# haampie/Homogenization.jl

Hardware: AMD Instinct MI355X
Metric: fine-DOF updates/sec per V-cycle (3D Tet64) (higher is better)
Workload: dtype f64; 1 GPU; 3D Tet64 checkerboard, 32^3 unit cubes x 6 tets, refinements=5 (BASELINE config 3); cells=196608, nf=6545, levels=6, smoothing_steps=3, smoothing_steps_coarse=2, coarse_solver=device CG, Chebyshev(4)-of-Jacobi preconditioner, rtol 1e-13, spare_vector_bytes=10294394880, lazy_top_form=2

## Files before the change

homogenization.jl_amd/csrc/hmg_context.cpp:

```cpp
#include "../../include/hmg.h"
#include "hmg_objects.hpp"

#include <algorithm>

namespace hmg {

std::recursive_mutex &lifetime_mutex()
{
    static std::recursive_mutex m;
    return m;
}

std::atomic<int64_t> &device_allocs()
{
    static std::atomic<int64_t> n{0};
    return n;
}

namespace {

void vec_pool_trim(hmg_ctx *c)
{
    LifetimeLock lock(lifetime_mutex());
    if (c->vec_pool.empty()) return;
    (void)hipStreamSynchronize(c->stream);
    for (auto &b : c->vec_pool) (void)hipFree(b.second);
    c->vec_pool.clear();
}

std::vector<hmg_ctx *> &live_contexts()
{
    static std::vector<hmg_ctx *> v;
    return v;
}

void release_pooled_memory()
{
    LifetimeLock lock(lifetime_mutex());
    for (hmg_ctx *c : live_contexts()) vec_pool_trim(c);
}

}

hipError_t device_malloc(void **p, size_t bytes)
{
    *p = nullptr;
    hipError_t e = hipMalloc(p, bytes);
    if (e != hipSuccess) {
        (void)hipGetLastError();
        release_pooled_memory();
        e = hipMalloc(p, bytes);
    }
    if (e == hipSuccess) device_allocs() += 1;
    return e;
}

double *vec_alloc(hmg_ctx *c, size_t bytes)
{
    LifetimeLock lock(lifetime_mutex());
    void *p = nullptr;
    for (size_t i = 0; i < c->vec_pool.size(); ++i)
        if (c->vec_pool[i].first == bytes) {
            p = c->vec_pool[i].second;
            c->vec_pool[i] = c->vec_pool.back();
            c->vec_pool.pop_back();
            break;
        }
    const bool pooled = p != nullptr;
    if (!pooled) {
        hipError_t e = device_malloc(&p, bytes);
        if (e != hipSuccess)
            throw std::runtime_error(std::string("hipMalloc of a level vector (") + std::to_string(bytes >> 20) +
                                     " MiB) failed: " + hipGetErrorString(e));
    }
    hipError_t e = hipMemsetAsync(p, 0, bytes, c->stream);
    if (e != hipSuccess) {
        (void)hipFree(p);
        throw std::runtime_error(std::string("HIP error: ") + hipGetErrorString(e));
    }
    return (double *)p;
}

void vec_release(hmg_ctx *c, void *p, size_t bytes)
{
    LifetimeLock lock(lifetime_mutex());
    if (c->vec_pool_on && bytes > 0) {
        c->vec_pool.emplace_back(bytes, p);
        return;
    }
    (void)hipStreamSynchronize(c->stream);
    (void)hipFree(p);
}

namespace {

void ensure_reduce_scratch(hmg_ctx *c, int64_t nentries)
{
    const int64_t need_blocks = nentries / 512 + 2;
    if (need_blocks <= 2048 || need_blocks <= c->L.rpart_cap) return;
    HIPCHK(hipStreamSynchronize(c->stream));
    c->rpart.alloc((size_t)need_blocks);
    c->L.rpart = c->rpart.p;
    c->L.rpart_cap = need_blocks;
}

void ctx_unref(hmg_ctx *ctx)
{
    LifetimeLock lock(lifetime_mutex());
    if (!ctx || --ctx->refs > 0) return;
    auto &lc = live_contexts();
    lc.erase(std::remove(lc.begin(), lc.end(), ctx), lc.end());
    (void)hipSetDevice(ctx->device);
    (void)hipStreamSynchronize(ctx->stream);
    for (auto &ev : ctx->timer.pool) {
        (void)hipEventDestroy(ev.first);
        (void)hipEventDestroy(ev.second);
    }
    vec_pool_trim(ctx);
    comm_drop(ctx);
    if (ctx->own_stream) (void)hipStreamDestroy(ctx->stream);
    delete ctx;
}

}

void grid_unref(hmg_grid *grid)
{
    LifetimeLock lock(lifetime_mutex());
    if (!grid || --grid->refs > 0) return;
    hmg_ctx *c = grid->ctx;
    if (c) {
        (void)hipSetDevice(c->device);
        (void)hipStreamSynchronize(c->stream);
    }
    probe_unlist(grid);
    release_top_spare(grid);
    release_weight_cache(grid);
    release_smoother_diag(grid);
    if (grid->probe && grid->probe->h) (void)hipHostFree(grid->probe->h);
    if (grid->probe && grid->probe->ev) (void)hipEventDestroy(grid->probe->ev);
    delete grid;
    ctx_unref(c);
}

double read_scalar(hmg_ctx *c, int slot)
{
    double h = 0.0;
    HIPCHK(hipMemcpyAsync(&h, c->L.scal + slot, sizeof(double), hipMemcpyDeviceToHost, c->stream));
    HIPCHK(hipStreamSynchronize(c->stream));
    judge_probes(c);
    return h;
}

}

extern "C" {

const char *hmg_last_error(void) { return last_error().c_str(); }
int hmg_version(void) { return 1; }

static int ctx_create(int device, void *stream, bool use_given, hmg_ctx **out)
{
    HMG_TRY
    need(out != nullptr, "null out pointer");
    int ndev = 0;
    hipError_t e = hipGetDeviceCount(&ndev);
    if (e != hipSuccess || ndev == 0)
        throw std::runtime_error("no HIP device available: libhmg_hip needs an MI355X (gfx950); there is no CPU fallback");
    need(device >= 0 && device < ndev, "device index out of range");
    HIPCHK(hipSetDevice(device));
    std::unique_ptr<hmg_ctx> c(new hmg_ctx);
    c->device = device;
    if (use_given) {
        c->stream = (hipStream_t)stream;
    } else {
        HIPCHK(hipStreamCreateWithFlags(&c->stream, hipStreamNonBlocking));
        c->own_stream = true;
    }
    hipDeviceProp_t prop;
    HIPCHK(hipGetDeviceProperties(&prop, device));
    c->partials.alloc(4096);
    c->scal.alloc(S_COUNT);
    HIPCHK(hipMemsetAsync(c->scal.p, 0, S_COUNT * sizeof(double), c->stream));
    c->L.stream = c->stream;
    c->L.partials = c->partials.p;
    c->L.rpart = nullptr;
    c->L.rpart_cap = 0;
    c->L.scal = c->scal.p;
    c->L.num_cu = prop.multiProcessorCount > 0 ? prop.multiProcessorCount : 256;
    c->L.apply_threads = 0;
    c->L.apply_mass_only = 0;
    c->L.cell_order = 1;
    c->L.weight_cache = 1;
    c->L.apply_wave = 1;
    c->L.wave_grid = 16 * (int64_t)c->L.num_cu;
    c->L.n_wave_launches = &c->wave_launches;
    c->L.apply_slab2 = 1;
    c->L.n_slab2_launches = &c->slab2_launches;
    c->L.n_rows_launches = &c->rows_launches;
    c->L.slab2_grid = 0;
    c->L.slab2_force = 0;
    c->L.restrict_slab2 = 1;
    c->L.apply_pack = 1;
    c->L.apply_small = 1;
    c->L.n_small_launches = &c->small_launches;
    c->L.n_wc_launches = &c->wc_launches;
    c->L.apply_wg512 = 1;
    {
        LifetimeLock lock(lifetime_mutex());
        live_contexts().push_back(c.get());
    }
    *out = c.release();
    HMG_END
}

int hmg_ctx_create(int device, void *stream, hmg_ctx **out) { return ctx_create(device, stream, stream != nullptr, out); }

int hmg_ctx_create_on_stream(int device, void *stream, hmg_ctx **out) { return ctx_create(device, stream, true, out); }

int hmg_ctx_destroy(hmg_ctx *ctx)
{
    HMG_TRY
    ctx_unref(ctx);
    HMG_END
}

int hmg_ctx_sync(hmg_ctx *ctx)
{
    HMG_TRY
    need(ctx != nullptr, "null ctx");
    HIPCHK(hipStreamSynchronize(ctx->stream));
    judge_probes(ctx);
    HMG_END
}

int64_t hmg_ctx_counter(hmg_ctx *ctx, const char *name)
{
    if (!ctx || !name) return -1;
    const std::string n(name);
    if (n == "wave_launches") return ctx->wave_launches;
    if (n == "slab2_launches") return ctx->slab2_launches;
    if (n == "rows_launches") return ctx->rows_launches;
    if (n == "small_launches") return ctx->small_launches;
    if (n == "weight_cache_launches") return ctx->wc_launches;
    if (n == "comm_calls") return ctx->comm_calls;
    if (n == "device_allocs") return device_allocs().load();
    if (n == "spare_bytes") return ctx->spare_bytes;
    if (n == "weight_cache_classes") return ctx->wc_classes;
    if (n == "weight_cache_bytes") return ctx->wc_bytes;
    if (n == "weight_cache_refusals") return ctx->wc_refusals;
    if (n == "fcg_bytes") return ctx->fcg_bytes;
    if (n == "smoother_diag_bytes") return ctx->smoother_diag_bytes;
    if (n == "smoother_diag_builds") return ctx->smoother_diag_builds;
    if (n == "lazy_top_form") return ctx->last_top_form;
    if (n == "lazy_pre_form") return ctx->last_pre_form;
    if (n == "coarse_x_folds") return ctx->coarse_x_folds;
    if (n == "cell_moments_kernel_ns") return ctx->moments_kernel_ns;
    if (n == "cell_moments_download_ns") return ctx->moments_download_ns;
    if (n == "comm_nranks") return ctx->comm ? ctx->comm_nranks : 0;
    return -1;
}

int hmg_ctx_release_memory(hmg_ctx *ctx)
{
    HMG_TRY
    need(ctx != nullptr, "null ctx");
    vec_pool_trim(ctx);
    HMG_END
}

int hmg_ctx_set_option(hmg_ctx *ctx, const char *name, int64_t value)
{
    HMG_TRY
    need(ctx && name, "null argument");
    std::string n(name);
    static const std::pair<const char *, bool hmg_ctx::*> flags[] = {
        {"coarse_probe", &hmg_ctx::coarse_probe}, {"fuse_cg", &hmg_ctx::fuse_cg_default}, {"fold_x", &hmg_ctx::fold_x},
        {"swap_rp", &hmg_ctx::swap_rp}, {"fold_prolong", &hmg_ctx::fold_prolong}, {"zero_entry", &hmg_ctx::zero_entry},
        {"fold_restrict", &hmg_ctx::fold_restrict}, {"lazy_dead", &hmg_ctx::lazy_dead}, {"lazy_pre", &hmg_ctx::lazy_pre}, {"fold_coarse_x", &hmg_ctx::fold_coarse_x}, {"fold_faces", &hmg_ctx::fold_faces},
        {"lean_post", &hmg_ctx::lean_post}, {"lazy_post", &hmg_ctx::lazy_post}, {"prolong_in_image", &hmg_ctx::prolong_in_image},
        {"comm_rehearsal", &hmg_ctx::comm_rehearsal}};
    for (const auto &f : flags)
        if (n == f.first) {
            ctx->*f.second = value != 0;
            return 0;
        }
    if (n == "apply_threads")
        ctx->L.apply_threads = (int)value;
    else if (n == "apply_wg512")
        ctx->L.apply_wg512 = value != 0;
    else if (n == "apply_pack")
        ctx->L.apply_pack = value != 0;
    else if (n == "apply_small")
        ctx->L.apply_small = value != 0;
    else if (n == "weight_cache")
        ctx->L.weight_cache = value != 0;
    else if (n == "weight_cache_classes")
        ctx->wc_max_classes = std::max<int64_t>(0, value);
    else if (n == "apply_slab2")
        ctx->L.apply_slab2 = value != 0;
    else if (n == "restrict_slab2")
        ctx->L.restrict_slab2 = value != 0;
    else if (n == "slab2_force")
        ctx->L.slab2_force = value != 0;
    else if (n == "slab2_grid")
        ctx->L.slab2_grid = std::max<int64_t>(0, value);
    else if (n == "apply_wave")
        ctx->L.apply_wave = value != 0;
    else if (n == "wave_grid")
        ctx->L.wave_grid = std::max<int64_t>(1, value) * (int64_t)ctx->L.num_cu;
    else if (n == "wave_grid_total")
        ctx->L.wave_grid = std::max<int64_t>(1, value);
    else if (n == "cell_order")
        ctx->L.cell_order = value != 0;
    else if (n == "coarse_poly")
        ctx->coarse_poly = std::max<int>(1, std::min<int>(16, (int)value));
    else if (n == "coarse_maxit")
        ctx->coarse_maxit = (int)value;
    else if (n == "coarse_check")
        ctx->coarse_check = std::max<int>(1, (int)value);
    else if (n == "lazy_top")
        ctx->lazy_top = (int)value;
    else if (n == "overlap_min_doubles")
        ctx->overlap_min_doubles = value;
    else if (n == "vec_pool") {
        ctx->vec_pool_on = value != 0;
        if (!ctx->vec_pool_on) vec_pool_trim(ctx);
    }
    else if (n == "time_apply") {
        ctx->timer.on = value > 0;
        ctx->timer.min_level = (int)value;
        ctx->timer.used = 0;
        ctx->timer.ev_level.clear();
        ctx->timer.ev_bytes.clear();
    }
    else
        throw std::runtime_error("unknown option: " + n);
    HMG_END
}

int hmg_ctx_set_option_f64(hmg_ctx *ctx, const char *name, double value)
{
    HMG_TRY
    need(ctx && name, "null argument");
    std::string n(name);
    if (n == "coarse_rtol")
        ctx->coarse_rtol = value;
    else if (n == "coarse_poly_ratio")
        ctx->coarse_poly_ratio = value;
    else
        throw std::runtime_error("unknown option: " + n);
    HMG_END
}

void *hmg_ctx_scalar_bank(hmg_ctx *ctx) { return ctx ? (void *)ctx->L.scal : nullptr; }

int hmg_ctx_set_scalar_bank(hmg_ctx *ctx, void *device_doubles16)
{
    HMG_TRY
    need(ctx != nullptr, "null argument");
    HIPCHK(hipStreamSynchronize(ctx->stream));
    double *to = device_doubles16 ? (double *)device_doubles16 : ctx->scal.p;
    if (to != ctx->L.scal) HIPCHK(hipMemcpy(to, ctx->L.scal, S_COUNT * sizeof(double), hipMemcpyDeviceToDevice));
    ctx->L.scal = to;
    HMG_END
}

static int apply_timing(hmg_ctx *ctx, bool every, int level, int64_t *launches, double *total_ms, double *total_bytes)
{
    HMG_TRY
    need(ctx && launches && total_ms && total_bytes, "null argument");
    HIPCHK(hipStreamSynchronize(ctx->stream));
    const ApplyTimer &tm = ctx->timer;
    double ms = 0.0, by = 0.0;
    int64_t n = 0;
    for (size_t i = 0; i < tm.used; ++i) {
        if (!every && tm.ev_level[i] != level) continue;
        float t = 0.f;
        HIPCHK(hipEventElapsedTime(&t, tm.pool[i].first, tm.pool[i].second));
        ms += t;
        by += tm.ev_bytes[i];
        n += 1;
    }
    *launches = n;
    *total_ms = ms;
    *total_bytes = by;
    HMG_END
}

int hmg_ctx_apply_timing(hmg_ctx *ctx, int64_t *launches, double *total_ms, double *total_bytes)
{
    return apply_timing(ctx, true, 0, launches, total_ms, total_bytes);
}

int hmg_ctx_apply_timing_level(hmg_ctx *ctx, int level, int64_t *launches, double *total_ms, double *total_bytes)
{
    return apply_timing(ctx, false, level, launches, total_ms, total_bytes);
}

void *hmg_ctx_stream(hmg_ctx *ctx) { return ctx ? (void *)ctx->stream : nullptr; }

int hmg_grid_destroy(hmg_grid *grid)
{
    HMG_TRY
    grid_unref(grid);
    HMG_END
}

int hmg_vec_create(hmg_grid *g, int level, hmg_vec **out)
{
    HMG_TRY
    need(g && out, "null argument");
    const LevelDev &lv = lev(g, level);
    HIPCHK(hipSetDevice(g->ctx->device));
    std::unique_ptr<hmg_vec> v(new hmg_vec);
    v->g = g;
    v->level = level;
    v->own = true;
    v->alloc_cells = g->md.ncells;
    size_t bytes = sizeof(double) * (size_t)lv.ld * (size_t)g->md.ncells;
    ensure_reduce_scratch(g->ctx, (int64_t)lv.ld * g->md.ncells);
    v->d = vec_alloc(g->ctx, bytes);
    v->bytes = bytes;
    if (wants_top_spare(g, level)) (void)reserve_top_spare(g, false);
    {
        LifetimeLock lock(lifetime_mutex());
        g->refs += 1;
    }
    *out = v.release();
    HMG_END
}

int hmg_vec_wrap(hmg_grid *g, int level, void *device_ptr, hmg_vec **out)
{
    HMG_TRY
    need(g && out && device_ptr, "null argument");
    ensure_reduce_scratch(g->ctx, (int64_t)lev(g, level).ld * g->md.ncells);
    std::unique_ptr<hmg_vec> v(new hmg_vec);
    v->g = g;
    v->level = level;
    v->own = false;
    v->alloc_cells = g->md.ncells;
    v->d = (double *)device_ptr;
    if (wants_top_spare(g, level)) (void)reserve_top_spare(g, false);
    {
        LifetimeLock lock(lifetime_mutex());
        g->refs += 1;
    }
    *out = v.release();
    HMG_END
}

int hmg_vec_destroy(hmg_vec *v)
{
    HMG_TRY
    if (v) {
        if (v->own && v->d) vec_release(v->g->ctx, v->d, v->bytes);
        hmg_grid *g = v->g;
        delete v;
        grid_unref(g);
    }
    HMG_END
}

void *hmg_vec_device_ptr(hmg_vec *v) { return v ? (void *)v->d : nullptr; }

}
```

homogenization.jl_amd/csrc/hmg_device.hpp:

```cpp
#pragma once
#include <hip/hip_runtime.h>

#include <cstdint>

namespace hmg {

constexpr int TABLE_PAD = 3 * 1024;

__host__ __device__ inline int rows_slot(int m, int i, int j, int nei, int off_int, int &cls)
{
    if (j == 0) {
        cls = i == 0 ? 4 : i == m ? 5 : 1;
        return i == 0 ? 0 : i == m ? 1 : 3 + i - 1;
    }
    if (i == 0) {
        cls = j == m ? 6 : 2;
        return j == m ? 2 : 3 + nei + j - 1;
    }
    if (i + j == m) {
        cls = 3;
        return 3 + 2 * nei + j - 1;
    }
    cls = 0;
    return off_int + (j - 1) * (m - 1) - (((j - 1) * j) >> 1) + i - 1;
}

struct LevelDev {
    int dim, level, m;
    int nf, ld;
    int ncorner, nedge, nface;
    int nei, nfi, nint;
    int off_edge, off_face, off_int;
    int ncls, ndir, nterm;
    int lds_g0, lds_g1;
    int nf_coarse;
    const uint64_t *meta;
    const uint16_t *lpos;
    const uint16_t *sweep_slot;
    int nsweep;
    const uint32_t *pos32;
    const uint32_t *pos32w;
    const uint32_t *sweep32;
    const uint32_t *blk_word;
    const uint16_t *blk_slot;
    int nblk, blk_R;
    const double *ctab;
    const int32_t *hier2slot;
    const int32_t *par_a, *par_b;
    const uint32_t *par32;
    const uint64_t *par64;
    const uint16_t *clpos;
    const uint32_t *rs_word;
    const double *rs_w;
    const uint16_t *rs_lp;
    const int32_t *rptr, *ridx;
    const double *dphi;
    const uint32_t *wave_tab;
    const uint32_t *wave_lpos;
    const uint32_t *wave_par;
    const uint32_t *wave_cl;
    const uint32_t *wave_rs;
    const double *wcache;
};

constexpr int WM = 16, WNF = 969, WNFI = 105, WNEI = 15, WNCORNER = 4, WNBLK = 152, WNFC = 165, WR = 4;
constexpr int WOFF_EDGE = 4, WOFF_FACE = 94, WNEC = 94;
constexpr int WNQ = 16;
constexpr int WVZ = 168;
constexpr int WAVE_TAB_ROWS = 15;
constexpr int WAVE_ROW = 16;
constexpr int WAVE_WSTRIDE = 15 * WAVE_ROW;

struct SlabTables {
    const int *head;
    const uint32_t *ld_word;
    const uint32_t *cp_word;
    const uint16_t *cp_slot;
    int nslab, lds_nodes;
    int max_surf;
    int max_int;
};

struct MeshDev {
    int dim;
    int64_t ncells, nnodes;
    const int32_t *cells;
    const int32_t *face_pairs;
    int64_t nfacepairs;
    const int32_t *face_partner;
    const int32_t *edge_ptr, *edge_ent;
    int64_t nsharededges;
    const int32_t *node_ptr, *node_ent;
    int64_t nsharednodes;
    const int32_t *node_first;
    const uint16_t *dmask, *dupmask;
    const double *coef;
    int64_t ncut_edge_groups, ncut_node_groups;
    int64_t ncut_face_pairs;
    const int32_t *cells_cut, *cells_inner;
    const int32_t *cell_perm;
    int64_t ncells_cut, ncells_inner;
    const uint8_t *mult;
    const int32_t *cell_class;
    int nclasses;
    double wc_lambda;
    double *blockpart;
    SlabTables slab;
};

struct ApplyArgs {
    double alpha, lambda;
    const double *x;
    const double *x2;
    double *xout;
    double *xacc;
    int a_num, a_den;
    const double *x3;
    int c_num, c_den;
    const double *x4;
    int d_num, d_den;
    const double *xcoarse;
    int64_t ldc;
    const double *xc_p, *xc_r;
    const double *src;
    double *out;
    double *rcoarse;
    int64_t ldrc;
    const double *scal;
    int s_num, s_den;
    double *blockpart;
    const uint8_t *mult;
    int flags;
    int64_t ncells_prefix;
    int64_t out_ld;
    const int32_t *cell_list;
    int64_t ncell_list;
    int64_t nwork;
    const int32_t *cell_class;
};

struct CoarseDev {
    int64_t n;
    const int32_t *rowptr, *colidx;
    const double *val, *diag;
    const int32_t *interior;
};

enum { S_RS = 0, S_PAP = 1, S_RS2 = 2, S_TMP = 3, S_C0 = 4, S_C1 = 5, S_C2 = 6, S_C3 = 7, S_PAP2 = 8, S_DONE = 9, S_ITER = 10,
       S_CRR = 11, S_HOST = 12, S_COUNT = 16,
       S_RS3 = S_C1, S_PAP3 = S_TMP };

struct Launch {
    hipStream_t stream;
    double *partials;
    double *rpart;
    int64_t rpart_cap;
    double *scal;
    int num_cu;
    int apply_threads;
    int apply_mass_only;
    int apply_wg512;
    int cell_order;
    int weight_cache;
    int apply_pack;
    int apply_small;
    int64_t *n_small_launches;
    int64_t *n_wc_launches;
    int apply_wave;
    int64_t wave_grid;
    int64_t *n_wave_launches;
    int apply_slab2;
    int64_t *n_slab2_launches;
    int64_t slab2_grid;
    int restrict_slab2;
    int slab2_force;
    int64_t *n_rows_launches;
};

void launch_apply(const Launch &L, const LevelDev &lv, const MeshDev &mesh, double alpha, double lambda,
                  const double *x, const double *src, double *out, int use_mask);
size_t apply_lds_bytes(const LevelDev &lv);
bool apply_restricts(const Launch &L, const LevelDev &lv);
bool apply_folds_coarse_x(const Launch &L, const LevelDev &lv);
bool apply_defers3(const Launch &L, const LevelDev &lv);
void launch_apply_fused_kernel(const Launch &L, const LevelDev &lv, const MeshDev &mesh, ApplyArgs a);
void launch_apply_fused_reduce(const Launch &L, const MeshDev &mesh, int slot_pap, int slot_rr);
void launch_apply_args(const Launch &L, const LevelDev &lv, const MeshDev &mesh, ApplyArgs a);
bool apply_wave_ok(const Launch &L, const LevelDev &lv, const MeshDev &mesh, const ApplyArgs &a, bool fused);
void launch_apply_wave(const Launch &L, const LevelDev &lv, const MeshDev &mesh, const ApplyArgs &a, bool fused);
bool apply_slab2_ok(const Launch &L, const LevelDev &lv, const MeshDev &mesh, const ApplyArgs &a);
void launch_apply_slab2(const Launch &L, const LevelDev &lv, const MeshDev &mesh, const ApplyArgs &a, bool fused);
void launch_apply_rows(const Launch &L, const LevelDev &lv, const MeshDev &mesh, const ApplyArgs &a, bool fused, bool wd);
void launch_prolong_add_wide(const Launch &L, const LevelDev &fine, const LevelDev &coarse, int64_t ncells, const double *xc,
                             double *xf);
int64_t launch_norm2_unique_wide(const Launch &L, const LevelDev &lv, const MeshDev &mesh, const double *x);
bool apply_small_ok(const Launch &L, const LevelDev &lv, const MeshDev &mesh, const ApplyArgs &a, bool fused);
void launch_apply_small(const Launch &L, const LevelDev &lv, const MeshDev &mesh, const ApplyArgs &a, bool fused);
void launch_weight_cache(const Launch &L, const LevelDev &lv, const double *coef_rep, int nclasses, double lambda, double *wcache);

void launch_interface_sum(const Launch &L, const LevelDev &lv, const MeshDev &mesh, double *x, int which = 0,
                          bool faces = true);
void launch_mask(const Launch &L, const LevelDev &lv, const MeshDev &mesh, double *x, int which );
void launch_restrict_slab(const Launch &L, const LevelDev &fine_rtab, const MeshDev &mesh, const SlabTables &st, int ldc,
                          const double *rf, double *bc);
void launch_restrict(const Launch &L, const LevelDev &fine, const LevelDev &coarse, int64_t ncells,
                     const double *rf, double *bc);
void launch_prolong_add(const Launch &L, const LevelDev &fine, const LevelDev &coarse, int64_t ncells,
                        const double *xc, double *xf);

void launch_fill(const Launch &L, double *x, int64_t n, double v);
void launch_copy(const Launch &L, double *dst, const double *src, int64_t n);
void launch_axpy(const Launch &L, double a, const double *x, double *y, int64_t n);
void launch_xpby(const Launch &L, const double *r, double b, double *p, int64_t n);
void launch_dot(const Launch &L, const double *x, const double *y, int64_t n, int slot);
void launch_norm2_unique(const Launch &L, const LevelDev &lv, const MeshDev &mesh, const double *x, int slot);
void launch_copy_dot(const Launch &L, double *p, const double *r, int64_t n, int slot);
void launch_cg_update(const Launch &L, double *x, double *r, const double *p, const double *q, int64_t n,
                      int s_num, int s_den, int s_out);
void launch_cg_rupdate(const Launch &L, const double *r, double *rout, const double *q, int64_t n, int s_num, int s_den,
                       int s_out);
void launch_cg_rupdate_faces(const Launch &L, const LevelDev &lv, const MeshDev &mesh, const double *r, double *rout,
                             const double *q, int64_t n, int s_num, int s_den, int s_out);
void launch_cg_rupdate_faces_x(const Launch &L, const LevelDev &lv, const MeshDev &mesh, const double *r, double *rout,
                               const double *q, int64_t n, int s_num, int s_den, int s_out, double *x, const double *p, int a_num,
                               int a_den, int b_num, int b_den, const double *p0, int z_num, int z_den);
void launch_cg_xp_update(const Launch &L, double *x, double *p, const double *r, int64_t n, int a_num, int a_den,
                         int s_num, int s_den, int with_p);
void launch_cg_x2_update(const Launch &L, double *x, const double *p, const double *r, int64_t n, int a_num, int a_den, int b_num,
                         int b_den, int c_num, int c_den);
void launch_cg_pupdate(const Launch &L, double *p, const double *r, int64_t n, int s_num, int s_den);

void launch_gather_base(const Launch &L, const MeshDev &mesh, int ld1, const double *v1, double *u);
void launch_scatter_base(const Launch &L, const MeshDev &mesh, int ld1, const double *u, double *v1);

void launch_gather_owned(const Launch &L, const MeshDev &mesh, const int32_t *nodes_g, const int32_t *owned, int ld1,
                         const double *v1, double *ug);
void launch_scatter_cells(const Launch &L, const int32_t *cell_nodes, int64_t ncells, int npc, int ld1, const double *u,
                          double *v1);

void launch_permute(const Launch &L, const LevelDev &lv, int64_t ncells, const double *src, double *dst,
                    int to_storage);
void launch_fill_random(const Launch &L, const LevelDev &lv, int64_t ncells, double *x, uint64_t seed,
                        int64_t cell_offset);

void launch_coarse_gather_rhs(const Launch &L, const CoarseDev &A, const double *u, double *b);
void launch_coarse_scatter_sol(const Launch &L, const CoarseDev &A, int64_t nnodes, const double *x, double *u);
void launch_coarse_init(const Launch &L, const CoarseDev &A, const double *b, double *x, double *r, double *z,
                        double *p, double zscale = 1.0, double *dcheb = nullptr);
void launch_coarse_cheb(const Launch &L, const CoarseDev &A, const double *r, const double *zin, double *zout, double *d, double c1,
                        double c2, int last);
void launch_coarse_rz_from_cheb(const Launch &L, const CoarseDev &A);
void launch_coarse_update(const Launch &L, const CoarseDev &A, double *x, double *r, double *z, const double *p,
                          const double *q, int slot_old, double zscale = 1.0, double *dcheb = nullptr);
void launch_coarse_residual_norm(const Launch &L, const CoarseDev &A);
void launch_coarse_direction(const Launch &L, const CoarseDev &A, double *p, double *q, const double *z, int slot_old, int slot_new,
                             double rtol2, int mode, int count_it, int rz_from_cheb = 0);

void launch_rhs_dphi(const Launch &L, const LevelDev &lv, int64_t ncells, const double *pvec, double *b);

void launch_integrate(const Launch &L, const LevelDev &lv, const MeshDev &mesh, int mode, int64_t nsub, const double *v,
                      const double *second, int slot);
void launch_integrate_load(const Launch &L, const LevelDev &lv, const MeshDev &mesh, int64_t nsub, const double *v,
                           const double *load, int slot);

struct CutPackArgs {
    int64_t n[3];
    const int64_t *pos[3];
    const int32_t *cell_lid[3];
    const uint8_t *first[3];
};
void launch_cut_pack(const Launch &L, const LevelDev &lv, const CutPackArgs &c, double *buf, double *x, int unpack);
void launch_seg_sum(const Launch &L, const int64_t *plan, int64_t ndoubles, double *buf, const double *stage);

}
```

homogenization.jl_amd/csrc/hmg_kernels.hip:

```cpp
#include "hmg_device.hpp"
#include "hmg_stencil.hpp"

#include <cstdio>
#include <stdexcept>
#include <string>

namespace hmg {

__global__ void __launch_bounds__(256) k_finalize(const double *__restrict__ partials, int n, double *scal, int slot)
{
    __shared__ double red[4];
    double v = 0.0;
    for (int i = threadIdx.x; i < n; i += 256) v += partials[i];
    double s = block_sum(v, red);
    if (threadIdx.x == 0) scal[slot] = s;
}

#ifdef HMG_PHASE_TIMING
#define HMG_STAMP(i)                                                                     \
    do {    \
        if (a.blockpart && !a.cell_list && tid == 0)                                     \
            a.blockpart[2 * (size_t)a.nwork + 8 * cell + (i)] = (double)wall_clock64(); \
    } while (0)
#define HMG_SLAB_T0() const long long _t0 = wall_clock64(); long long _tl = _t0; double _ph[5] = {0, 0, 0, 0, 0}
#define HMG_SLAB_PHASE(i)                              \
    do {                                               \
        const long long _n = wall_clock64();           \
        _ph[i] += (double)(_n - _tl);                  \
        _tl = _n;                                      \
    } while (0)
#define HMG_SLAB_STORE()                                                                      \
    do {                                                                                      \
        if (a.blockpart && tid == 0) {                                                        \
            double *_o = a.blockpart + 2 * (size_t)a.nwork + 8 * cell;                        \
            _o[0] = (double)_t0;                                                              \
            for (int _q = 0; _q < 5; ++_q) _o[1 + _q] = _ph[_q];                              \
            _o[6] = (double)wall_clock64();                                                   \
        }                                                                                     \
    } while (0)
#else
#define HMG_STAMP(i)
#define HMG_SLAB_T0()
#define HMG_SLAB_PHASE(i)
#define HMG_SLAB_STORE()
#endif

template <int DIM, int NT, int SPT, bool FUSED, int RB, bool WD = false, bool CG = false, bool RS = false, bool WC = false, int LF = 0>
__global__ void __launch_bounds__(NT, NT >= 640 ? 8 : RB && NT == 512 ? 6 : 1)
k_apply(LevelDev lv, const double *__restrict__ coef, const uint16_t *__restrict__ dmask, ApplyArgs a)
{
    constexpr int NDIR = DIM == 3 ? 15 : 7;
    constexpr int NTERM = DIM == 3 ? 7 : 4;
    constexpr int WS = RB ? WSZ_RB : WSZ;
    extern __shared__ double smem[];
    double *W = smem;
    double *xs = smem + WS + lv.lds_g0;
    const int tid = threadIdx.x;
    constexpr bool LOOP = NT == 64;
    int64_t blk = blockIdx.x;
    do {
    const int64_t cell = a.cell_list ? (int64_t)a.cell_list[blk] : blk;
    const int nf = lv.nf;
    HMG_STAMP(0);

    size_t wbase16 = 0;
    if constexpr (WC) wbase16 = (size_t)(2 * HMG_KP(int32_t, a.cell_class)[cell] + (a.alpha < 0.0 ? 1 : 0)) * WAVE_WSTRIDE;
    const double cv = RB && !WC ? coef[cell * 8 + (tid & 7)] : 0.0;
    if (!RB && (tid >= NT - 256 || NT <= 256)) {
        const int first = NT <= 256 ? tid : tid - (NT - 256);
        const int step = NT <= 256 ? NT : 256;
        if constexpr (WC) {
            for (int idx = first; idx < lv.ncls * NDIR; idx += step)
                W[idx] = lv.wcache[wbase16 + (size_t)((idx / NDIR) * WAVE_ROW + idx % NDIR)];
        } else {
        double s[NTERM];
        cell_scales<DIM>(coef + cell * 8, a.alpha, a.lambda, s, a.flags);
        for (int idx = first; idx < lv.ncls * NDIR; idx += step) {
            const double *c = lv.ctab + (size_t)idx * NTERM;
            double w = 0.0;
#pragma unroll
            for (int t = 0; t < NTERM; ++t) w += c[t] * s[t];
            W[idx] = w;
        }
        }
    }
    for (int q = tid; q < lv.lds_g0; q += NT) smem[WS + q] = 0.0;
    for (int q = tid; q < lv.lds_g1; q += NT) xs[nf + q] = 0.0;
    const int m = lv.m;
    constexpr int NW = NT / 64, WPF = NW / 4 > 0 ? NW / 4 : 1, NE = NW >= 6 ? 1 : 2;
    constexpr int FI = RB && NT == 512 ? 4 : 2;
    constexpr int NPASS = RB && NT == 512 ? 2 : 1;
    constexpr bool EARLY = RB && (NT <= 256 || WC);
    const int wave = tid >> 6, lane = tid & 63;
    const int face = wave / WPF, ft0 = (wave % WPF) * (FI * 64);
    int edge[NE], ebase[NE];
#pragma unroll
    for (int q = 0; q < NE; ++q) {
        edge[q] = NW - 1 - wave + q * NW;
        if (edge[q] >= lv.nedge) edge[q] = -1;
        ebase[q] = lv.off_edge + (edge[q] < 0 ? 0 : edge[q]) * lv.nei;
    }
    uint32_t fw[FI], ew[NE][1], cw = 0u;
#pragma unroll
    for (int q = 0; q < FI; ++q) fw[q] = 0u;
    uint32_t p0 = 0u, p1 = 0u;
    double wv = 0.0;
    double c7[NTERM];
    uint32_t q0 = 0u, q1 = 0u;
    int s0 = 0, s1 = 0;
    uint32_t mq[4] = {0, 0, 0, 0};
    uint32_t mqr[4] = {0, 0, 0, 0};
    uint32_t dm = 0u;
    const uint32_t *iw = RB ? lv.blk_word : lv.sweep32;
    const uint16_t *is = RB ? lv.blk_slot : lv.sweep_slot;
    double cwl = 0.0;
    auto issue_rows = [&]() {
        if constexpr (WC) {
            if (a.flags & 1) {
                const uint32_t w2 = HMG_KP(uint32_t, dmask)[cell >> 1];
                dm = (cell & 1) ? w2 >> 16 : w2 & 0xffffu;
            }
            if (RB) {
                int row = 0;
                if (lane < 15)
                    row = lane;
                else if (lane >= 16 && lane < 31)
                    row = (1 + face) * WAVE_ROW + lane - 16;
                else if (lane >= 32 && lane < 47 && edge[0] >= 0)
                    row = (1 + lv.nface + edge[0]) * WAVE_ROW + lane - 32;
                else if (NE > 1 && lane >= 48 && lane < 63 && edge[NE - 1] >= 0)
                    row = (1 + lv.nface + edge[NE - 1]) * WAVE_ROW + lane - 48;
                wv = lv.wcache[wbase16 + row];
                if (wave == NW - 1) {
                    const int cl = lane < 60 ? lane : 59;
                    cwl = lv.wcache[wbase16 + (1 + lv.nface + lv.nedge + cl / 15) * WAVE_ROW + cl % 15];
                }
            }
            if (FUSED && a.mult) {
#pragma unroll
                for (int q = 0; q < 4; ++q) mqr[q] = HMG_KP(uint32_t, a.mult)[cell * 4 + q];
            }
            return;
        }
        dm = (a.flags & 1) ? dmask[cell] : 0u;
        if (RB) {
            int row = 0;
            if (lane < 15)
                row = lane;
            else if (lane >= 16 && lane < 31)
                row = (1 + face) * NDIR + lane - 16;
            else if (lane >= 32 && lane < 47 && edge[0] >= 0)
                row = (1 + lv.nface + edge[0]) * NDIR + lane - 32;
            else if (NE > 1 && lane >= 48 && lane < 63 && edge[NE - 1] >= 0)
                row = (1 + lv.nface + edge[NE - 1]) * NDIR + lane - 48;
#pragma unroll
            for (int t = 0; t < NTERM; ++t) c7[t] = lv.ctab[(size_t)row * NTERM + t];
        }
        if (FUSED && a.mult) {
            const uint32_t *mp = reinterpret_cast<const uint32_t *>(a.mult + cell * 16);
#pragma unroll
            for (int q = 0; q < 4; ++q) mqr[q] = mp[q];
        }
    };
    auto issue_words = [&]() {
        if (RB) {
#pragma unroll
            for (int q = 0; q < FI; ++q) {
                const int ti = ft0 + q * 64 + lane;
                if (ti < lv.nfi) fw[q] = lv.pos32[lv.off_face + face * lv.nfi + ti];
            }
#pragma unroll
            for (int q = 0; q < NE; ++q) ew[q][0] = edge[q] >= 0 && lane < lv.nei ? lv.pos32[ebase[q] + lane] : 0u;
            if (wave == NW - 1 && lane < lv.ncorner) cw = lv.pos32[lane];
        } else {
            p0 = lv.pos32[tid];
            p1 = lv.pos32[tid + NT];
        }
        q0 = iw[tid];
        q1 = RB && NPASS < 2 ? 0u : iw[tid + NT];
        s0 = (int)is[tid];
        s1 = RB && NPASS < 2 ? 0 : (int)is[tid + NT];
    };
    auto finish_tables = [&]() {
        if constexpr (WC) {
            if (RB && wave == NW - 1 && lane < 60) W[lane] = cwl;
            if (FUSED) {
#pragma unroll
                for (int q = 0; q < 4; ++q) mq[q] = a.mult ? mqr[q] : 0x01010101u;
            }
            return;
        }
        if (RB) {
            double sc7[NTERM];
#pragma unroll
            for (int t = 0; t < NTERM - 1; ++t) sc7[t] = (a.flags & 2) ? 0.0 : a.alpha * readlane_f64(cv, t);
            sc7[NTERM - 1] = a.alpha * a.lambda * ((a.flags & 16) ? 1.0 : readlane_f64(cv, NTERM - 1));
#pragma unroll
            for (int t = 0; t < NTERM; ++t) wv += c7[t] * sc7[t];
            if (wave == NW - 1) {
                const int cbase = (1 + lv.nface + lv.nedge) * NDIR;
                for (int idx = cbase + lane; idx < lv.ncls * NDIR; idx += 64) {
                    double w = 0.0;
#pragma unroll
                    for (int t = 0; t < NTERM; ++t) w += lv.ctab[(size_t)idx * NTERM + t] * sc7[t];
                    W[idx - cbase] = w;
                }
            }
        }
        if (FUSED) {
#pragma unroll
            for (int q = 0; q < 4; ++q) mq[q] = a.mult ? __builtin_amdgcn_readfirstlane(mqr[q]) : 0x01010101u;
        }
    };
    constexpr bool rows_late = WC && (LF == 2 || LF == 5);
    constexpr bool WEARLY = false;
    if (EARLY && !rows_late) issue_rows();
    if (WEARLY) issue_words();
    const double *xc = a.x + cell * lv.ld;
    double rr = 0.0, pap = 0.0;
    {
        const double *x2c = FUSED && a.x2 ? a.x2 + cell * lv.ld : nullptr;
        double *xoc = FUSED && a.xout ? a.xout + cell * lv.ld : nullptr;
        double *xac = FUSED && a.xacc ? a.xacc + cell * lv.ld : nullptr;
        const double *x3c = FUSED && a.x3 ? a.x3 + cell * lv.ld : nullptr;
        const double beta = x2c ? a.scal[a.s_num] / a.scal[a.s_den] : 0.0;
        const double ax = xac || x3c ? a.scal[a.a_num] / a.scal[a.a_den] : 0.0;
        const double c2 = x3c ? a.scal[a.c_num] / a.scal[a.c_den] : 0.0;
        constexpr bool X4 = FUSED && RS && LF == 4;
        const double *x4c = X4 && a.x4 ? a.x4 + cell * lv.ld : nullptr;
        const double dx4 = x4c ? a.scal[a.d_num] / a.scal[a.d_den] : 0.0;
        const double *ccol = FUSED && !RS && a.xcoarse ? a.xcoarse + cell * a.ldc : nullptr;
        constexpr bool cgather = FUSED && CG;
        double *cs = xs + nf + lv.lds_g1;
        double cval = 0.0;
        if (ccol && !cgather) {
            if (tid < lv.nf_coarse) cval = ccol[tid];
            for (int q = tid + NT; q < lv.nf_coarse; q += NT) cs[q] = ccol[q];
        }
        auto prolong = [&](double v, uint32_t w) {
            const uint32_t pa = w & 0xffffu, pb = w >> 16;
            if (pa == pb) return v + cs[pa];
            v += 0.5 * cs[pa];
            return v + 0.5 * cs[pb];
        };
        if (cgather && ccol) {
            constexpr int NC = 2;
            constexpr bool CX = cgather && LF == 5;
            const double *cpc = CX ? a.xc_p + cell * a.ldc : nullptr, *crc = CX ? a.xc_r + cell * a.ldc : nullptr;
            const double cxa = CX ? to_sgpr(a.scal[a.a_num] / a.scal[a.a_den]) : 0.0;
            const double cxb = CX ? to_sgpr(a.scal[a.s_num] / a.scal[a.s_den]) : 0.0;
            const double cxc = CX ? to_sgpr(a.scal[a.c_num] / a.scal[a.c_den]) : 0.0;
            double cv2[NC], cp2[CX ? NC : 1], cr2[CX ? NC : 1];
            int cl2[NC];
#pragma unroll
            for (int q = 0; q < NC; ++q) {
                const int c = tid + q * NT;
                if (c < lv.nf_coarse) {
                    cv2[q] = ccol[c];
                    if (CX) {
                        cp2[q] = cpc[c];
                        cr2[q] = crc[c];
                    }
                    cl2[q] = lv.clpos[c];
                }
            }
            if (CX) {
#pragma unroll
                for (int q = 0; q < NC; ++q)
                    if (tid + q * NT < lv.nf_coarse) cv2[q] = axpy1(cxc, axpy1(cxb, cp2[q], cr2[q]), axpy1(cxa, cp2[q], cv2[q]));
                __builtin_amdgcn_sched_barrier(0);
                if (EARLY && rows_late) issue_rows();
            }
            double xv[SPT];
            uint64_t pw[SPT];
#pragma unroll
            for (int q = 0; q < SPT; ++q) {
                const int t = tid + q * NT;
                if (t < nf) {
                    xv[q] = xc[t];
                    pw[q] = lv.par64[t];
                }
            }
            if (EARLY) finish_tables();
#pragma unroll
            for (int q = 0; q < NC; ++q)
                if (tid + q * NT < lv.nf_coarse) xs[cl2[q]] = cv2[q];
            __syncthreads();
#pragma unroll
            for (int q = 0; q < SPT; ++q) {
                const int t = tid + q * NT;
                if (t < nf) {
                    const uint32_t pa = (uint32_t)pw[q] & 0xffffu, pb = ((uint32_t)pw[q] >> 16) & 0xffffu;
                    double v = xv[q];
                    if (pa == pb)
                        v = v + lds_ld(xs + pa);
                    else {
                        v += 0.5 * lds_ld(xs + pa);
                        v = v + 0.5 * lds_ld(xs + pb);
                    }
                    xv[q] = v;
                }
            }
            __syncthreads();
#pragma unroll
            for (int q = 0; q < SPT; ++q) {
                const int t = tid + q * NT;
                if (t < nf) {
                    const double v = xv[q];
                    if (xoc) xoc[t] = v;
                    rr += v * v;
                    xs[(int)(pw[q] >> 32)] = v;
                }
            }
        }
        const bool light = LF == 1 || (LF == 0 && !RS && FUSED && NT >= 512 && !x2c && !xac && !x3c && !ccol);
        if (FUSED && light) {
            double xv[SPT];
            int lp[SPT];
#pragma unroll
            for (int q = 0; q < SPT; ++q) {
                const int t = tid + q * NT;
                if (t < nf) {
                    xv[q] = xc[t];
                    lp[q] = lv.lpos[t];
                }
            }
            if (EARLY) finish_tables();
#pragma unroll
            for (int q = 0; q < SPT; ++q) {
                const int t = tid + q * NT;
                if (t < nf) {
                    const double v = xv[q];
                    if (xoc) xoc[t] = v;
                    rr += v * v;
                    xs[lp[q]] = v;
                }
            }
        }
        const bool light2 = LF == 2 || (LF == 0 && !RS && FUSED && NT >= 512 && x2c && !xoc && !xac && !x3c && !ccol);
        if (FUSED && light2) {
            double xv[SPT], x2v[SPT];
            int lp[SPT];
#pragma unroll
            for (int q = 0; q < SPT; ++q) {
                const int t = tid + q * NT;
                if (t < nf) {
                    xv[q] = xc[t];
                    x2v[q] = x2c[t];
                    lp[q] = lv.lpos[t];
                }
            }
            if (EARLY && rows_late) issue_rows();
            if (EARLY) finish_tables();
#pragma unroll
            for (int q = 0; q < SPT; ++q) {
                const int t = tid + q * NT;
                if (t < nf) {
                    const double v = axpy1(beta, x2v[q], xv[q]);
                    if (LF == 2 && xoc) xoc[t] = v;
                    rr += v * v;
                    xs[lp[q]] = v;
                }
            }
        }
        constexpr int HB = X4 ? (SPT + 2) / 3 : FUSED ? (SPT + 1) / 2 : SPT;
        const bool xzero = FUSED && (RS || RB == 0) && (a.flags & 128);
        if (!light && !light2 && !(cgather && ccol)) {
#pragma unroll
        for (int q0 = 0; q0 < SPT; q0 += HB) {
            double xv[HB], x2v[HB], xav[HB], x4v[X4 ? HB : 1];
            int lp[HB];
            uint32_t pw[HB];
#pragma unroll
            for (int q = 0; q < HB; ++q) {
                const int t = tid + (q0 + q) * NT;
                if (q0 + q < SPT && t < nf) {
                    xv[q] = xzero ? 0.0 : xc[t];
                    if (X4) x4v[q] = x4c ? x4c[t] : 0.0;
                    x2v[q] = x2c ? x2c[t] : 0.0;
                    xav[q] = xac ? xac[t] : x3c ? x3c[t] : 0.0;
                    lp[q] = lv.lpos[t];
                    if (FUSED && !cgather) pw[q] = ccol ? lv.par32[t] : 0u;
                }
            }
            if (EARLY && q0 == 0) finish_tables();
            if (FUSED && q0 == 0 && ccol && !cgather) {
                if (tid < lv.nf_coarse) cs[tid] = cval;
                __syncthreads();
            }
#pragma unroll
            for (int q = 0; q < HB; ++q) {
                const int t = tid + (q0 + q) * NT;
                if (q0 + q < SPT && t < nf) {
                    double v = xv[q];
                    if (FUSED) {
                        if (!cgather && ccol) v = prolong(v, pw[q]);
                        if (xac) xac[t] = axpy1(ax, x2v[q], xav[q]);
                        if (x3c) {
                            if (X4 && x4c) v = axpy1(dx4, x4v[q], v);
                            const double t1 = axpy1(ax, x2v[q], v);
                            const double p2 = axpy1(beta, x2v[q], xav[q]);
                            v = axpy1(c2, p2, t1);
                        } else if (x2c)
                            v = axpy1(beta, x2v[q], v);
                        if (xoc) xoc[t] = v;
                        if (!RS) rr += v * v;
                    }
                    xs[lp[q]] = v;
                }
            }
        }
        }
        for (int t = tid + SPT * NT; t < nf; t += NT) {
            double v = xzero ? 0.0 : xc[t];
            if (FUSED) {
                const double pv = x2c ? x2c[t] : 0.0;
                if (!cgather && ccol) v = prolong(v, lv.par32[t]);
                if (xac) xac[t] = axpy1(ax, pv, xac[t]);
                if (x3c) {
                    if (X4 && x4c) v = axpy1(dx4, x4c[t], v);
                    const double t1 = axpy1(ax, pv, v);
                    const double p2 = axpy1(beta, pv, x3c[t]);
                    v = axpy1(c2, p2, t1);
                } else if (x2c)
                    v = axpy1(beta, pv, v);
                if (xoc) xoc[t] = v;
                rr += v * v;
            }
            xs[lv.lpos[t]] = v;
        }
    }

    HMG_STAMP(1);
    __builtin_amdgcn_sched_barrier(0);
    if (!WEARLY) issue_words();
    if (!EARLY) {
        issue_rows();
        finish_tables();
    }
    const double *sc = a.src ? a.src + cell * lv.ld : nullptr;
    double *oc = a.out ? a.out + cell * lv.ld : nullptr;
    const int nsurf = lv.off_int;
    const int nsw = RB ? lv.nblk : lv.nsweep;
    const bool wdot = WD && FUSED && (a.flags & 8);
    const double wself = (wdot && (a.flags & 256)) ? 0.0 : 1.0;
    HMG_STAMP(2);
    __syncthreads();
    HMG_STAMP(3);

    const int wbase = RB ? (1 + lv.nface + lv.nedge) * NDIR : 0;
    auto surface_node = [&](int t, uint32_t pw) -> double {
        const double sv = sc ? sc[t] : 0.0;
        int L, len, A, B, cls;
        decode32<DIM>(pw, m, L, len, A, B, cls);
        double ctr;
        double o = stencil_eval_c<DIM>(W + cls * NDIR - wbase, xs, L, len, A, B, ctr);
        if (!wdot) o = sv + o;
        if ((dm >> (cls - 1)) & 1u) o = 0.0;
        if (!FUSED || oc) oc[t] = o;
        if (FUSED && !RS) {
            const int e = cls - 1;
            const uint32_t word = e < 4 ? mq[0] : e < 8 ? mq[1] : e < 12 ? mq[2] : mq[3];
            const uint32_t mu = (word >> (8 * (e & 3))) & 0xffu;
            pap += (double)mu * ((wdot ? fma(wself, ctr, sv) : ctr) * o);
        }
        return o;
    };
    double kf[FI], ke[NE], kc = 0.0, ki[NPASS][RB ? RB : 1];
    if constexpr (RS && RB != 0 && DIM == 3) {
        double w0e[15];
#pragma unroll
        for (int d = 0; d < NDIR; ++d) w0e[d] = readlane_f64(wv, d);
        if (tid < nsw) interior_block_keep<RB ? RB : 1, FUSED>(w0e, xs, m, nf >> 1, q0, s0, sc, oc, ki[0]);
        if (NPASS > 1 && tid + NT < nsw) interior_block_keep<RB ? RB : 1, FUSED>(w0e, xs, m, nf >> 1, q1, s1, sc, oc, ki[NPASS - 1]);
    }
    if (RB) {
        if (DIM == 3) {
            const bool fdir = (dm >> face) & 1u;
            const double fmult = (double)((mq[0] >> (8 * (face & 3))) & 0xffu);
            const int fbase = lv.off_face + face * lv.nfi;
            double nopre[FI];
#pragma unroll
            for (int q = 0; q < FI; ++q) nopre[q] = 0.0;
            if (face >= 4)
                ;
            else if (face == 0)
                face_items<0, FI, FUSED, FUSED && !RS>(wv, 16, xs, m, lv.nfi, fbase, ft0, fw, fdir, fmult, sc, oc, pap, lane, nopre, false, wdot, RS ? kf : nullptr, wself);
            else if (face == 1)
                face_items<1, FI, FUSED, FUSED && !RS>(wv, 16, xs, m, lv.nfi, fbase, ft0, fw, fdir, fmult, sc, oc, pap, lane, nopre, false, wdot, RS ? kf : nullptr, wself);
            else if (face == 2)
                face_items<2, FI, FUSED, FUSED && !RS>(wv, 16, xs, m, lv.nfi, fbase, ft0, fw, fdir, fmult, sc, oc, pap, lane, nopre, false, wdot, RS ? kf : nullptr, wself);
            else
                face_items<3, FI, FUSED, FUSED && !RS>(wv, 16, xs, m, lv.nfi, fbase, ft0, fw, fdir, fmult, sc, oc, pap, lane, nopre, false, wdot, RS ? kf : nullptr, wself);
#pragma unroll
            for (int q = 0; q < NE; ++q) {
                if (edge[q] < 0) continue;
                const int eb = lv.nface + edge[q];
                const bool edir = (dm >> eb) & 1u;
                const double emult = (double)(((eb < 4 ? mq[0] : eb < 8 ? mq[1] : mq[2]) >> (8 * (eb & 3))) & 0xffu);
                const double nop1[1] = {0.0};
                const int wl = 32 + 16 * q;
                switch (edge[q]) {
                case 0: class_items<edge_tap_mask(0), 1, FUSED, FUSED && !RS>(wv, wl, xs, m, lv.nei, ebase[q], 0, ew[q], edir, emult, sc, oc, pap, lane, nop1, false, wdot, RS ? &ke[q] : nullptr, wself); break;
                case 1: class_items<edge_tap_mask(1), 1, FUSED, FUSED && !RS>(wv, wl, xs, m, lv.nei, ebase[q], 0, ew[q], edir, emult, sc, oc, pap, lane, nop1, false, wdot, RS ? &ke[q] : nullptr, wself); break;
                case 2: class_items<edge_tap_mask(2), 1, FUSED, FUSED && !RS>(wv, wl, xs, m, lv.nei, ebase[q], 0, ew[q], edir, emult, sc, oc, pap, lane, nop1, false, wdot, RS ? &ke[q] : nullptr, wself); break;
                case 3: class_items<edge_tap_mask(3), 1, FUSED, FUSED && !RS>(wv, wl, xs, m, lv.nei, ebase[q], 0, ew[q], edir, emult, sc, oc, pap, lane, nop1, false, wdot, RS ? &ke[q] : nullptr, wself); break;
                case 4: class_items<edge_tap_mask(4), 1, FUSED, FUSED && !RS>(wv, wl, xs, m, lv.nei, ebase[q], 0, ew[q], edir, emult, sc, oc, pap, lane, nop1, false, wdot, RS ? &ke[q] : nullptr, wself); break;
                default: class_items<edge_tap_mask(5), 1, FUSED, FUSED && !RS>(wv, wl, xs, m, lv.nei, ebase[q], 0, ew[q], edir, emult, sc, oc, pap, lane, nop1, false, wdot, RS ? &ke[q] : nullptr, wself); break;
                }
            }
            if (wave == NW - 1 && lane < lv.ncorner) kc = surface_node(lane, cw);
        }
    } else {
        const int nit_surf = (nsurf + NT - 1) / NT;
        for (int it = 0; it < nit_surf; ++it) {
            const int t = tid + it * NT;
            const uint32_t pw = p0;
            p0 = p1;
            p1 = lv.pos32[t + 2 * NT];
            if (t < nsurf) surface_node(t, pw);
        }
    }
    HMG_STAMP(4);
    double w0[15];
#pragma unroll
    for (int d = 0; d < NDIR; ++d) w0[d] = RB ? readlane_f64(wv, d) : to_sgpr(W[d]);
    if (RB) {
        if constexpr (!RS) {
        if (DIM == 3 && tid < nsw) {
            if (sc)
                interior_block<RB ? RB : 1, FUSED, true>(w0, xs, m, nf >> 1, q0, s0, sc, oc, pap, wdot, wself);
            else
                interior_block<RB ? RB : 1, FUSED, false>(w0, xs, m, nf >> 1, q0, s0, sc, oc, pap);
        }
        if (DIM == 3 && NPASS > 1 && tid + NT < nsw) {
            if (sc)
                interior_block<RB ? RB : 1, FUSED, true>(w0, xs, m, nf >> 1, q1, s1, sc, oc, pap, wdot, wself);
            else
                interior_block<RB ? RB : 1, FUSED, false>(w0, xs, m, nf >> 1, q1, s1, sc, oc, pap);
        }
        }
    } else {
        const int nit_sweep = (nsw + NT - 1) / NT;
        for (int it = 0; it < nit_sweep; ++it) {
            const int u = tid + it * NT;
            const uint32_t pw = q0;
            const int t = s0;
            q0 = q1;
            s0 = s1;
            q1 = iw[u + 2 * NT];
            s1 = (int)is[u + 2 * NT];
            if (t != 0xffff) {
                const double sv = sc ? sc[t] : 0.0;
                int L, len, A, B, cls;
                decode32<DIM>(pw, m, L, len, A, B, cls);
                double ctr;
                double o = stencil_eval_v<DIM>(w0, xs + L, len, A, B, ctr);
                if (!wdot) o = sv + o;
                if (!FUSED || oc) oc[t] = o;
                if (FUSED) pap += (wdot ? fma(wself, ctr, sv) : ctr) * o;
            }
        }
    }
    HMG_STAMP(5);
    if constexpr (RS && RB != 0 && DIM == 3) {
        int fl[FI], el[NE], cl = 0;
        uint32_t b0 = 0u, b1 = 0u;
        if (face < 4) {
#pragma unroll
            for (int q = 0; q < FI; ++q) {
                const int ti = ft0 + q * 64 + lane;
                fl[q] = ti < lv.nfi ? (int)lv.lpos[lv.off_face + face * lv.nfi + ti] : 0;
            }
        }
#pragma unroll
        for (int q = 0; q < NE; ++q) el[q] = edge[q] >= 0 && lane < lv.nei ? (int)lv.lpos[ebase[q] + lane] : 0;
        if (wave == NW - 1 && lane < lv.ncorner) cl = (int)lv.lpos[lane];
        if (tid < nsw) b0 = lv.blk_word[tid];
        if (NPASS > 1 && tid + NT < nsw) b1 = lv.blk_word[tid + NT];
        __syncthreads();
        if (face < 4) {
#pragma unroll
            for (int q = 0; q < FI; ++q)
                if (ft0 + q * 64 + lane < lv.nfi) xs[fl[q]] = kf[q];
        }
#pragma unroll
        for (int q = 0; q < NE; ++q)
            if (edge[q] >= 0 && lane < lv.nei) xs[el[q]] = ke[q];
        if (wave == NW - 1 && lane < lv.ncorner) xs[cl] = kc;
        {
            int pos[RB ? RB : 1];
            if (tid < nsw) {
                block_positions<RB ? RB : 1>(m, b0, pos);
                const int nv = (int)(b0 >> 28);
#pragma unroll
                for (int r = 0; r < (RB ? RB : 1); ++r)
                    if (r < nv) xs[pos[r]] = ki[0][r];
            }
            if (NPASS > 1 && tid + NT < nsw) {
                block_positions<RB ? RB : 1>(m, b1, pos);
                const int nv = (int)(b1 >> 28);
#pragma unroll
                for (int r = 0; r < (RB ? RB : 1); ++r)
                    if (r < nv) xs[pos[r]] = ki[NPASS - 1][r];
            }
        }
        __syncthreads();
        double *rc = a.rcoarse + cell * a.ldrc;
        if (lv.rs_lp) {
            for (int c = tid; c < lv.nf_coarse; c += NT) {
                const int b = lv.rptr[c], n = lv.rptr[c + 1] - b;
                int lp[15];
#pragma unroll
                for (int q = 0; q < 15; ++q) lp[q] = lv.rs_lp[b + (q < n ? q : 0)];
                double tmp = 0.0;
                tmp += 1.0 * lds_ld(xs + lp[0]);
#pragma unroll
                for (int q = 1; q < 15; ++q)
                    if (q < n) tmp += 0.5 * lds_ld(xs + lp[q]);
                rc[c] = tmp;
            }
        } else
        for (int c = tid; c < lv.nf_coarse; c += NT) {
            int L, len, A, B, cls, k;
            decode32w(lv.rs_word[c], m, L, len, A, B, cls, k);
            const double *w = lv.rs_w + cls * NDIR;
            auto at = [&](int off) { return lds_ld(xs + max(L + off, 0)); };
            double acc = w[0] * lds_ld(xs + L);
            acc += w[1] * lds_ld(xs + L + 1);
            acc += w[2] * at(-1);
            acc += w[3] * lds_ld(xs + L + len - 1);
            acc += w[4] * at(-len);
            acc += w[5] * lds_ld(xs + L + len);
            acc += w[6] * at(-len - 1);
            acc += w[7] * lds_ld(xs + L + A - len);
            acc += w[8] * at(len + 1 - B);
            acc += w[9] * lds_ld(xs + L + A - 1);
            acc += w[10] * at(1 - B);
            acc += w[11] * lds_ld(xs + L + A);
            acc += w[12] * at(-B);
            acc += w[13] * lds_ld(xs + L + A + 1 - len);
            acc += w[14] * at(len - B);
            rc[c] = 0.0 + acc;
        }
    }
    if (FUSED && !RS) {
        __syncthreads();
        const double s_pap = block_sum(pap, smem);
        const double s_rr = block_sum(rr, smem);
        if (tid == 0) {
            a.blockpart[2 * cell] = s_pap;
            a.blockpart[2 * cell + 1] = s_rr;
        }
    }
    HMG_STAMP(6);
    if (LOOP) {
        blk += gridDim.x;
        if (blk >= a.nwork) break;
        __syncthreads();
    }
    } while (LOOP);
}

template <int DIM, int NT, bool FUSED, bool WD = false>
__global__ void __launch_bounds__(NT, 8)
k_apply_slab(LevelDev lv, const double *__restrict__ coef, const uint16_t *__restrict__ dmask, ApplyArgs a, SlabTables st)
{
    constexpr int NDIR = DIM == 3 ? 15 : 7;
    constexpr int NTERM = DIM == 3 ? 7 : 4;
    constexpr int HB = FUSED ? 3 : 4;
    constexpr int MV = 5;
    extern __shared__ double smem[];
    double *W = smem;
    double *img = smem + WSZ;
    const int tid = threadIdx.x;
    const int64_t cell = a.cell_list ? (int64_t)a.cell_list[blockIdx.x] : (int64_t)blockIdx.x;
    const int m = lv.m;

    if (a.flags & 4) {
        for (int idx = tid; idx < lv.ncls * NDIR; idx += NT) W[idx] = lv.ctab[(size_t)idx * NTERM + NTERM - 1];
    } else {
        double s[NTERM];
        cell_scales<DIM>(coef + cell * 8, a.alpha, a.lambda, s, a.flags);
        for (int idx = tid; idx < lv.ncls * NDIR; idx += NT) {
            const double *c = lv.ctab + (size_t)idx * NTERM;
            double w = 0.0;
#pragma unroll
            for (int t = 0; t < NTERM; ++t) w += c[t] * s[t];
            W[idx] = w;
        }
    }
    const double *xc = a.x + cell * lv.ld;
    const double *x2c = FUSED && a.x2 ? a.x2 + cell * lv.ld : nullptr;
    double *xoc = FUSED && a.xout ? a.xout + cell * lv.ld : nullptr;
    double *xac = FUSED && a.xacc ? a.xacc + cell * lv.ld : nullptr;
    const double *x3c = FUSED && a.x3 ? a.x3 + cell * lv.ld : nullptr;
    const double beta = to_sgpr(x2c ? a.scal[a.s_num] / a.scal[a.s_den] : 0.0);
    const double ax = to_sgpr(xac || x3c ? a.scal[a.a_num] / a.scal[a.a_den] : 0.0);
    const double c2 = to_sgpr(x3c ? a.scal[a.c_num] / a.scal[a.c_den] : 0.0);
    const uint32_t dm = (a.flags & 1) ? dmask[cell] : 0u;
    const double *sc = a.src ? a.src + cell * lv.ld : nullptr;
    double *oc = a.out ? a.out + cell * (a.out_ld ? a.out_ld : (int64_t)lv.ld) : nullptr;
    uint32_t mq[4] = {0, 0, 0, 0};
    if (FUSED) {
        const uint32_t *mp = reinterpret_cast<const uint32_t *>(a.mult + cell * 16);
#pragma unroll
        for (int q = 0; q < 4; ++q) mq[q] = a.mult ? __builtin_amdgcn_readfirstlane(mp[q]) : 0x01010101u;
    }
    const bool wdot = WD && FUSED && (a.flags & 8);
    const double wself = (wdot && (a.flags & 256)) ? 0.0 : 1.0;
    double rr = 0.0, pap = 0.0;
    auto plane_off = [&](int k) {
        if (k <= 0) return 0;
        if (k > m + 1) k = m + 1;
        const long long n1 = m + 1, n2 = m + 1 - k;
        return (int)((n1 * (n1 + 1) * (n1 + 2) - n2 * (n2 + 1) * (n2 + 2)) / 6);
    };
    HMG_SLAB_T0();
    __syncthreads();
    HMG_SLAB_PHASE(0);
    double w0[NDIR];
#pragma unroll
    for (int d = 0; d < NDIR; ++d) w0[d] = to_sgpr(W[d]);
    int lo_prev = 0;
    for (int sl = 0; sl < st.nslab; ++sl) {
        const int *hd = st.head + 8 * sl;
        const int k0 = hd[0], ld_off = hd[1], ld_cnt = hd[2], cp_off = hd[3], cp_cnt = hd[4], cp_surf = hd[5];
        const int lo = plane_off(k0 - 1);
        double *xs = img - lo;
        uint32_t wd0[HB];
#pragma unroll
        for (int q = 0; q < HB; ++q) wd0[q] = st.ld_word[ld_off + q * NT + tid];
        if (sl > 0) {
            __syncthreads();
            const int cnt = plane_off(k0 + 1) - lo, src = lo - lo_prev;
            if (cnt <= MV * NT) {
                double mv[MV];
#pragma unroll
                for (int c = 0; c < MV; ++c) {
                    const int q = c * NT + tid;
                    mv[c] = q < cnt ? img[src + q] : 0.0;
                }
                __syncthreads();
#pragma unroll
                for (int c = 0; c < MV; ++c) {
                    const int q = c * NT + tid;
                    if (q < cnt) img[q] = mv[c];
                }
            } else {
            const int nchunk = (cnt + NT - 1) / NT;
            for (int c = 0; c < nchunk; ++c) {
                const int q = c * NT + tid;
                const double v = q < cnt ? img[src + q] : 0.0;
                __syncthreads();
                if (q < cnt) img[q] = v;
            }
            }
        }
        for (int q = (sl > 0 ? plane_off(k0 + 1) - lo : 0) + tid; q < st.lds_nodes; q += NT) img[q] = 0.0;
        __syncthreads();
        HMG_SLAB_PHASE(1);
        for (int q0 = 0; q0 < ld_cnt; q0 += HB * NT) {
            uint32_t wd[HB];
            double xv[HB], x2v[HB], xav[HB];
#pragma unroll
            for (int q = 0; q < HB; ++q) {
                const int v = q0 + q * NT + tid;
                wd[q] = q0 == 0 ? wd0[q] : st.ld_word[ld_off + v];
            }
#pragma unroll
            for (int q = 0; q < HB; ++q) {
                const int v = q0 + q * NT + tid;
                if (v < ld_cnt) {
                    const int t = (int)(wd[q] >> 16);
                    xv[q] = xc[t];
                    x2v[q] = x2c ? x2c[t] : 0.0;
                    xav[q] = xac ? xac[t] : x3c ? x3c[t] : 0.0;
                }
            }
#pragma unroll
            for (int q = 0; q < HB; ++q) {
                const int v = q0 + q * NT + tid;
                if (v < ld_cnt) {
                    const int t = (int)(wd[q] >> 16);
                    double val = xv[q];
                    if (FUSED) {
                        if (xac) xac[t] = axpy1(ax, x2v[q], xav[q]);
                        if (x3c) {
                            const double t1 = axpy1(ax, x2v[q], val);
                            const double p2 = axpy1(beta, x2v[q], xav[q]);
                            val = axpy1(c2, p2, t1);
                        } else if (x2c)
                            val = axpy1(beta, x2v[q], val);
                        if (xoc) xoc[t] = val;
                        rr += val * val;
                    }
                    xs[wd[q] & 0xffffu] = val;
                }
            }
        }
        const int ib = cp_off + cp_surf;
        uint32_t p0 = st.cp_word[cp_off + tid], p1 = st.cp_word[cp_off + tid + NT];
        int s0 = (int)st.cp_slot[cp_off + tid], s1 = (int)st.cp_slot[cp_off + tid + NT];
        uint32_t q0 = st.cp_word[ib + tid], q1 = st.cp_word[ib + tid + NT];
        int t0 = (int)st.cp_slot[ib + tid], t1 = (int)st.cp_slot[ib + tid + NT];
        __syncthreads();
        HMG_SLAB_PHASE(2);
        const int nit_s = (cp_surf + NT - 1) / NT;
        for (int it = 0; it < nit_s; ++it) {
            const int v = it * NT + tid;
            const uint32_t pw = p0;
            const int t = s0;
            p0 = p1;
            s0 = s1;
            p1 = st.cp_word[cp_off + v + 2 * NT];
            s1 = (int)st.cp_slot[cp_off + v + 2 * NT];
            if (v < cp_surf) {
                const double sv = sc ? sc[t] : 0.0;
                int L, len, A, B, cls, k;
                decode32w(pw, m, L, len, A, B, cls, k);
                double ctr;
                double o = stencil_eval_c<DIM>(W + cls * NDIR, xs, L, len, A, B, ctr);
                if (!wdot) o = sv + o;
                if ((dm >> (cls - 1)) & 1u) o = 0.0;
                if (!FUSED || oc) oc[t] = o;
                if (FUSED) {
                    const int en = cls - 1;
                    const uint32_t word = en < 4 ? mq[0] : en < 8 ? mq[1] : en < 12 ? mq[2] : mq[3];
                    const uint32_t mu = (word >> (8 * (en & 3))) & 0xffu;
                    pap += (double)mu * ((wdot ? fma(wself, ctr, sv) : ctr) * o);
                }
            }
        }
        HMG_SLAB_PHASE(3);
        const int n_int = cp_cnt - cp_surf;
        const int nit_i = (n_int + NT - 1) / NT;
        for (int it = 0; it < nit_i; ++it) {
            const int v = it * NT + tid;
            const uint32_t pw = q0;
            const int t = t0;
            q0 = q1;
            t0 = t1;
            q1 = st.cp_word[ib + v + 2 * NT];
            t1 = (int)st.cp_slot[ib + v + 2 * NT];
            if (v < n_int) {
                const double sv = sc ? sc[t] : 0.0;
                int L, len, A, B;
                decode_lattice(pw, m, L, len, A, B);
                double ctr;
                double o = stencil_eval_v<DIM>(w0, xs + L, len, A, B, ctr);
                if (!wdot) o = sv + o;
                if (!FUSED || oc) oc[t] = o;
                if (FUSED) pap += (wdot ? fma(wself, ctr, sv) : ctr) * o;
            }
        }
        lo_prev = lo;
        HMG_SLAB_PHASE(4);
    }
    HMG_SLAB_STORE();
    if (FUSED) {
        __syncthreads();
        const double s_pap = block_sum(pap, smem);
        const double s_rr = block_sum(rr, smem);
        if (tid == 0) {
            a.blockpart[2 * cell] = s_pap;
            a.blockpart[2 * cell + 1] = s_rr;
        }
    }
}

__global__ void __launch_bounds__(256)
k_reduce_pairs(const double *__restrict__ blockpart, int64_t n, double *partials)
{
    __shared__ double red[4];
    double s0 = 0.0, s1 = 0.0;
    for (int64_t c = (int64_t)blockIdx.x * 256 + threadIdx.x; c < n; c += (int64_t)gridDim.x * 256) {
        s0 += blockpart[2 * c];
        s1 += blockpart[2 * c + 1];
    }
    const double r0 = block_sum(s0, red);
    const double r1 = block_sum(s1, red);
    if (threadIdx.x == 0) {
        partials[blockIdx.x] = r0;
        partials[2048 + blockIdx.x] = r1;
    }
}

__global__ void __launch_bounds__(256)
k_reduce_weighted(const double *__restrict__ blockpart, const double *__restrict__ coef, int jterm, int64_t n, double *partials)
{
    __shared__ double red[4];
    double s0 = 0.0;
    for (int64_t c = (int64_t)blockIdx.x * 256 + threadIdx.x; c < n; c += (int64_t)gridDim.x * 256)
        s0 += blockpart[2 * c] * coef[c * 8 + jterm];
    const double r0 = block_sum(s0, red);
    if (threadIdx.x == 0) partials[blockIdx.x] = r0;
}

size_t apply_lds_bytes(const LevelDev &lv)
{
    return sizeof(double) * (size_t)(WSZ + lv.lds_g0 + lv.nf + lv.lds_g1);
}

bool apply_restricts(const Launch &L, const LevelDev &lv)
{
    if (!(lv.dim == 3 && apply_lds_bytes(lv) <= 160 * 1024 && L.apply_threads == 0 && lv.rs_word &&
          lv.rs_w && lv.nf_coarse > 0 && lv.nei <= 64 && lv.nedge == 6 && lv.ncorner == 4))
        return false;
    if (lv.nf > 2048)
        return lv.blk_R == 6 && lv.nblk <= 960 && L.apply_wg512 && lv.nfi <= 512;
    return lv.nf > 192 && lv.nf <= 1024 && lv.blk_R == 4 && lv.nblk <= 192 && lv.nfi <= 128 && lv.rs_lp != nullptr;
}

bool apply_defers3(const Launch &L, const LevelDev &lv)
{
    return apply_restricts(L, lv) && lv.nf > 2048 && lv.nf <= 13 * 512;
}

bool apply_folds_coarse_x(const Launch &L, const LevelDev &lv)
{
    return lv.dim == 3 && apply_lds_bytes(lv) <= 160 * 1024 && L.apply_threads == 0 && L.apply_wg512 && lv.blk_R == 6 && lv.nblk <= 960 &&
           lv.nei <= 64 && lv.nedge == 6 && lv.ncorner == 4 && lv.nfi <= 512 && lv.par64 && lv.clpos && lv.nf > 2048 &&
           lv.nf <= 13 * 512 && lv.nf_coarse > 0 && lv.nf_coarse <= 2 * 512;
}

static size_t apply_lds_bytes_rb(const LevelDev &lv)
{
    return sizeof(double) * (size_t)(WSZ_RB + lv.lds_g0 + lv.nf + lv.lds_g1);
}

template <bool FUSED>
static void check_apply_bases(const ApplyArgs &a, const MeshDev &mesh)
{
    if (!a.x) throw std::runtime_error("operator apply: null input vector");
    if (!FUSED && !a.out) throw std::runtime_error("operator apply: a plain launch needs an output vector");
    if (a.rcoarse && a.ldrc <= 0) throw std::runtime_error("operator apply: epilogue restriction without the coarse column stride");
    if (FUSED && (!a.blockpart || !a.scal)) throw std::runtime_error("operator apply: fused launch without its reduction scratch");
    if (!mesh.coef) throw std::runtime_error("operator apply: no operator coefficients on the device (hmg_grid_set_operator)");
    if ((a.flags & 1) && !mesh.dmask) throw std::runtime_error("operator apply: constraint requested without a Dirichlet mask");
    if (a.xcoarse && !a.xout) throw std::runtime_error("operator apply: folded prolongation without xout");
    if ((a.flags & 128) && !(FUSED && a.x3 && a.x2 && a.xout && !a.xcoarse))
        throw std::runtime_error("operator apply: the zero-input form exists for the residual with two pending x-updates only");
}

static bool weight_cache_ok(const Launch &L, const LevelDev &lv, const MeshDev &mesh, const ApplyArgs &a)
{
    return L.weight_cache && lv.wcache && mesh.cell_class && lv.dim == 3 && lv.ncls == 15 && !(a.flags & (2 | 8 | 16)) &&
           (a.alpha == 1.0 || a.alpha == -1.0) && a.lambda == mesh.wc_lambda;
}

template <int DIM, int NT, int SPT, bool FUSED, int RB = 0, bool WD = false, bool CG = false, bool RS = false, bool WC = false, int LF = 0>
static void launch_apply_generic(const Launch &L, const LevelDev &lv, const MeshDev &mesh, const ApplyArgs &a, size_t lds)
{
    auto kern = k_apply<DIM, NT, SPT, FUSED, RB, WD, CG, RS, WC, LF>;
    if (a.rcoarse && !RS) throw std::runtime_error("operator apply: this instantiation cannot restrict in its epilogue");
    if (a.xc_p && !(CG && LF == 5)) throw std::runtime_error("operator apply: this instantiation cannot finish the coarse x");
    if (a.x4 && LF != 4) throw std::runtime_error("operator apply: this instantiation cannot carry a third pending x-update");
    if ((a.flags & 128) && !(FUSED && (RS || RB == 0)))
        throw std::runtime_error("operator apply: this instantiation cannot take a zero input that is not in memory");
    if (FUSED && a.xcoarse && !CG) lds += sizeof(double) * (size_t)lv.nf_coarse;
    if (lds > 48 * 1024)
        HMG_HIP_CHECK(hipFuncSetAttribute((const void *)kern, hipFuncAttributeMaxDynamicSharedMemorySize, (int)lds));
    const int64_t nblocks = a.cell_list ? a.ncell_list : a.ncells_prefix ? a.ncells_prefix : mesh.ncells;
    if (nblocks == 0) return;
    check_apply_bases<FUSED>(a, mesh);
    ApplyArgs b = a;
    b.nwork = nblocks;
    b.cell_class = WC ? mesh.cell_class : nullptr;
    if (WC && !weight_cache_ok(L, lv, mesh, a)) throw std::runtime_error("operator apply: class-weight cache not usable for this launch");
    if (L.cell_order && RB && !a.cell_list && !a.ncells_prefix && mesh.cell_perm) {
        b.cell_list = mesh.cell_perm;
        b.ncell_list = nblocks;
    }
    const int64_t grid = NT == 64 ? std::min<int64_t>(nblocks, 32 * (int64_t)L.num_cu) : nblocks;
    hipLaunchKernelGGL(kern, dim3((unsigned)grid), dim3(NT), lds, L.stream, lv, mesh.coef, mesh.dmask, b);
    check_launch();
    if (WC && L.n_wc_launches) *L.n_wc_launches += 1;
}

template <int DIM, bool FUSED, bool WD = false>
static void launch_apply_dim(const Launch &L, const LevelDev &lv, const MeshDev &mesh, const ApplyArgs &a)
{
    const size_t lds = apply_lds_bytes(lv);
    if (a.x4 && !(FUSED && DIM == 3 && !WD && a.x3 && a.x2 && a.xout && a.rcoarse && !a.xcoarse && !a.xacc && !(a.flags & 128) &&
                  apply_defers3(L, lv)))
        throw std::runtime_error("operator apply: a third pending x-update (x4) where no kernel carries it");
    if ((a.xc_p || a.xc_r) && !(FUSED && DIM == 3 && !WD && a.xc_p && a.xc_r && a.xcoarse && (a.flags & 64) && !a.x2 && !a.xacc && !a.x3 &&
                                !a.rcoarse && apply_folds_coarse_x(L, lv)))
        throw std::runtime_error("operator apply: pending coarse x-updates (xc_p, xc_r) where no kernel carries them");
    if constexpr (DIM == 3 && !WD) {
        if (apply_wave_ok(L, lv, mesh, a, FUSED)) {
            launch_apply_wave(L, lv, mesh, a, FUSED);
            return;
        }
        if (apply_small_ok(L, lv, mesh, a, FUSED)) {
            launch_apply_small(L, lv, mesh, a, FUSED);
            return;
        }
    }
    const bool force_slab2 = DIM == 3 && !WD && L.slab2_force && mesh.slab.head && mesh.slab.nslab >= 2 && lv.nf > 2048 &&
                             !a.xcoarse && !a.rcoarse && !(a.flags & (4 | 8));
    if (DIM == 2 && lds > 160 * 1024) {
        launch_apply_rows(L, lv, mesh, a, FUSED, WD);
        return;
    }
    if (lds > 160 * 1024 || force_slab2) {
        if (DIM != 3 || !mesh.slab.head) throw std::runtime_error("operator apply: cell does not fit the LDS");
        if constexpr (DIM == 3 && !WD) {
            if (apply_slab2_ok(L, lv, mesh, a)) {
                launch_apply_slab2(L, lv, mesh, a, FUSED);
                return;
            }
        }
        auto kern = k_apply_slab<3, 1024, FUSED, WD>;
        const size_t bytes = sizeof(double) * (size_t)(WSZ + mesh.slab.lds_nodes);
        HMG_HIP_CHECK(hipFuncSetAttribute((const void *)kern, hipFuncAttributeMaxDynamicSharedMemorySize, (int)bytes));
        const int64_t nblocks = a.cell_list ? a.ncell_list : a.ncells_prefix ? a.ncells_prefix : mesh.ncells;
        if (nblocks == 0) return;
        check_apply_bases<FUSED>(a, mesh);
        ApplyArgs b = a;
        b.nwork = nblocks;
        if (L.cell_order && !a.cell_list && !a.ncells_prefix && mesh.cell_perm) {
            b.cell_list = mesh.cell_perm;
            b.ncell_list = nblocks;
        }
        hipLaunchKernelGGL(kern, dim3((unsigned)nblocks), dim3(1024), bytes, L.stream, lv, mesh.coef, mesh.dmask, b,
                           mesh.slab);
        check_launch();
        return;
    }
    const int nf = lv.nf;
    int nt = WD ? 0 : L.apply_threads;
    if (nt == 0) nt = nf <= 192 ? 64 : nf <= 2048 ? 256 : 1024;
    if (nt <= 64) {
        if constexpr (DIM == 3 && !WD) {
            if (weight_cache_ok(L, lv, mesh, a)) {
                if (nf > 64)
                    launch_apply_generic<DIM, 64, 3, FUSED, 0, false, false, false, DIM == 3>(L, lv, mesh, a, lds);
                else
                    launch_apply_generic<DIM, 64, 1, FUSED, 0, false, false, false, DIM == 3>(L, lv, mesh, a, lds);
                return;
            }
        }
        if (nf > 64)
            launch_apply_generic<DIM, 64, 3, FUSED, 0, WD>(L, lv, mesh, a, lds);
        else
            launch_apply_generic<DIM, 64, 1, FUSED, 0, WD>(L, lv, mesh, a, lds);
    }
    else if (nt <= 192 && nf <= 192)
        launch_apply_generic<DIM, 192, 1, FUSED, 0, WD>(L, lv, mesh, a, lds);
    else if (nt <= 256 && nf <= 1024) {
        if (DIM == 3 && lv.blk_R == 4 && lv.nblk <= 192 && lv.nfi <= 128 && lv.nei <= 64 && lv.nedge == 6 && lv.ncorner == 4) {
            if constexpr (!WD) {
                if (FUSED && DIM == 3 && a.rcoarse && lv.rs_word && lv.rs_w && !a.xcoarse) {
                    launch_apply_generic<DIM, 256, 4, FUSED, DIM == 3 ? 4 : 0, false, false, FUSED && DIM == 3>(
                        L, lv, mesh, a, apply_lds_bytes_rb(lv));
                    return;
                }
            }
            launch_apply_generic<DIM, 256, 4, FUSED, DIM == 3 ? 4 : 0, WD>(L, lv, mesh, a, apply_lds_bytes_rb(lv));
        }
        else
            launch_apply_generic<DIM, 256, 4, FUSED, 0, WD>(L, lv, mesh, a, lds);
    }
    else if (nt <= 256)
        launch_apply_generic<DIM, 256, 8, FUSED, 0, WD>(L, lv, mesh, a, lds);
    else if (nt <= 640) {
        if constexpr (!WD) {
            if (nt <= 512) {
                if (DIM == 3 && lv.blk_R == 6 && lv.nblk <= 1024 && lv.nfi <= 512 && lv.nei <= 64 && lv.nedge == 6 &&
                    lv.ncorner == 4)
                    launch_apply_generic<DIM, 512, 13, FUSED, DIM == 3 ? 6 : 0>(L, lv, mesh, a, apply_lds_bytes_rb(lv));
                else
                    launch_apply_generic<DIM, 512, 13, FUSED>(L, lv, mesh, a, lds);
            } else
                launch_apply_generic<DIM, 640, 11, FUSED>(L, lv, mesh, a, lds);
        }
    } else if (DIM == 3 && lv.blk_R == 6 && lv.nblk <= 960 && lv.nei <= 64 && lv.nedge == 6 && lv.ncorner == 4) {
        if constexpr (!WD) {
            if (L.apply_wg512 && lv.nfi <= 512) {
                const bool cg = FUSED && DIM == 3 && a.xcoarse && (a.flags & 64) && lv.par64 && lv.clpos && !a.x2 && !a.xacc && !a.x3 &&
                                lv.nf <= 13 * 512 && lv.nf_coarse <= 2 * 512;
                const bool rs = !cg && FUSED && DIM == 3 && a.rcoarse && lv.rs_word && lv.rs_w && !a.xcoarse;
                constexpr int R6 = DIM == 3 ? 6 : 0;
                constexpr bool F3 = FUSED && DIM == 3;
                if (DIM == 3 && weight_cache_ok(L, lv, mesh, a)) {
                    if (cg && a.xc_p)
                        launch_apply_generic<DIM, 512, 13, FUSED, R6, false, F3, false, DIM == 3, F3 ? 5 : 0>(L, lv, mesh, a, apply_lds_bytes_rb(lv));
                    else if (cg)
                        launch_apply_generic<DIM, 512, 13, FUSED, R6, false, F3, false, DIM == 3>(L, lv, mesh, a, apply_lds_bytes_rb(lv));
                    else if (rs && a.x4)
                        launch_apply_generic<DIM, 512, 13, FUSED, R6, false, false, F3, DIM == 3, F3 ? 4 : 0>(L, lv, mesh, a, apply_lds_bytes_rb(lv));
                    else if (rs)
                        launch_apply_generic<DIM, 512, 13, FUSED, R6, false, false, F3, DIM == 3>(L, lv, mesh, a, apply_lds_bytes_rb(lv));
                    else if (FUSED && !a.x2 && !a.xacc && !a.x3 && !a.xcoarse && !a.rcoarse)
                        launch_apply_generic<DIM, 512, 13, FUSED, R6, false, false, false, DIM == 3, F3 ? 1 : 0>(L, lv, mesh, a, apply_lds_bytes_rb(lv));
                    else if (FUSED && a.x2 && (!a.xout || a.xout != a.x2) && !a.xacc && !a.x3 && !a.xcoarse && !a.rcoarse)
                        launch_apply_generic<DIM, 512, 13, FUSED, R6, false, false, false, DIM == 3, F3 ? 2 : 0>(L, lv, mesh, a, apply_lds_bytes_rb(lv));
                    else
                        launch_apply_generic<DIM, 512, 13, FUSED, R6, false, false, false, DIM == 3>(L, lv, mesh, a, apply_lds_bytes_rb(lv));
                    return;
                }
                if (cg && a.xc_p)
                    launch_apply_generic<DIM, 512, 13, FUSED, R6, false, F3, false, false, F3 ? 5 : 0>(L, lv, mesh, a, apply_lds_bytes_rb(lv));
                else if (cg)
                    launch_apply_generic<DIM, 512, 13, FUSED, R6, false, F3>(L, lv, mesh, a, apply_lds_bytes_rb(lv));
                else if (rs && a.x4)
                    launch_apply_generic<DIM, 512, 13, FUSED, R6, false, false, F3, false, F3 ? 4 : 0>(L, lv, mesh, a, apply_lds_bytes_rb(lv));
                else if (rs)
                    launch_apply_generic<DIM, 512, 13, FUSED, R6, false, false, F3>(L, lv, mesh, a, apply_lds_bytes_rb(lv));
                else
                    launch_apply_generic<DIM, 512, 13, FUSED, R6>(L, lv, mesh, a, apply_lds_bytes_rb(lv));
                return;
            }
        }
        launch_apply_generic<DIM, 1024, 7, FUSED, DIM == 3 ? 6 : 0, WD>(L, lv, mesh, a, apply_lds_bytes_rb(lv));
    }
    else
        launch_apply_generic<DIM, 1024, 7, FUSED, 0, WD>(L, lv, mesh, a, lds);
}

void launch_apply(const Launch &L, const LevelDev &lv, const MeshDev &mesh, double alpha, double lambda,
                  const double *x, const double *src, double *out, int use_mask)
{
    ApplyArgs a{};
    a.alpha = alpha;
    a.lambda = lambda;
    a.x = x;
    a.src = src;
    a.out = out;
    a.flags = (use_mask ? 1 : 0) | (L.apply_mass_only ? 2 : 0);
#ifdef HMG_PHASE_TIMING
    a.blockpart = mesh.blockpart;
#endif
    if (lv.dim == 3)
        launch_apply_dim<3, false>(L, lv, mesh, a);
    else
        launch_apply_dim<2, false>(L, lv, mesh, a);
}

void launch_apply_args(const Launch &L, const LevelDev &lv, const MeshDev &mesh, ApplyArgs a)
{
    a.flags = (a.flags & 1) | (L.apply_mass_only ? 2 : 0);
    if (lv.dim == 3)
        launch_apply_dim<3, false>(L, lv, mesh, a);
    else
        launch_apply_dim<2, false>(L, lv, mesh, a);
}

void launch_apply_fused_kernel(const Launch &L, const LevelDev &lv, const MeshDev &mesh, ApplyArgs a)
{
    a.scal = L.scal;
    if (!(a.flags & 32)) a.mult = mesh.mult;
    a.blockpart = mesh.blockpart;
    if (a.flags & 8) {
        if (lv.dim == 3)
            launch_apply_dim<3, true, true>(L, lv, mesh, a);
        else
            launch_apply_dim<2, true, true>(L, lv, mesh, a);
        return;
    }
    if (lv.dim == 3)
        launch_apply_dim<3, true>(L, lv, mesh, a);
    else
        launch_apply_dim<2, true>(L, lv, mesh, a);
}

void launch_apply_fused_reduce(const Launch &L, const MeshDev &mesh, int slot_pap, int slot_rr)
{
    hipLaunchKernelGGL(k_reduce_pairs, dim3(256), dim3(256), 0, L.stream, mesh.blockpart, mesh.ncells, L.partials);
    check_launch();
    hipLaunchKernelGGL(k_finalize, dim3(1), dim3(256), 0, L.stream, L.partials, 256, L.scal, slot_pap);
    if (slot_rr >= 0)
        hipLaunchKernelGGL(k_finalize, dim3(1), dim3(256), 0, L.stream, L.partials + 2048, 256, L.scal, slot_rr);
    check_launch();
}

__global__ void __launch_bounds__(256)
k_iface_faces(const int32_t *__restrict__ pairs, int64_t npairs, int nfi, int off_face, int ld, double *x)
{
    constexpr int U = 8;
    const int lane = threadIdx.x & 63;
    const int64_t nw = ((int64_t)gridDim.x * blockDim.x) >> 6;
    for (int64_t p = ((int64_t)blockIdx.x * blockDim.x + threadIdx.x) >> 6; p < npairs; p += nw) {
        const int32_t ca = pairs[3 * p], cb = pairs[3 * p + 1], lf = pairs[3 * p + 2];
        double *a = x + (int64_t)ca * ld + off_face + (lf & 15) * nfi;
        double *b = x + (int64_t)cb * ld + off_face + (lf >> 4) * nfi;
        for (int k0 = 0; k0 < nfi; k0 += U * 64) {
            double va[U], vb[U];
#pragma unroll
            for (int u = 0; u < U; ++u) {
                const int k = k0 + u * 64 + lane;
                if (k < nfi) {
                    va[u] = a[k];
                    vb[u] = b[k];
                }
            }
#pragma unroll
            for (int u = 0; u < U; ++u) {
                const int k = k0 + u * 64 + lane;
                if (k < nfi) {
                    const double s = va[u] + vb[u];
                    a[k] = s;
                    b[k] = s;
                }
            }
        }
    }
}

__global__ void __launch_bounds__(256)
k_iface_csr(const int32_t *__restrict__ eptr, const int32_t *__restrict__ eent, int64_t nedge, int nei, int off_edge,
            const int32_t *__restrict__ nptr, const int32_t *__restrict__ nent, int64_t nnode, int ld, double *x)
{
    constexpr int U = 8;
    const int64_t tedge = nedge * nei, total = tedge + nnode;
    for (int64_t idx = (int64_t)blockIdx.x * blockDim.x + threadIdx.x; idx < total;
         idx += (int64_t)gridDim.x * blockDim.x) {
        const bool is_edge = idx < tedge;
        const int64_t e = is_edge ? idx / nei : idx - tedge;
        const int k = is_edge ? (int)(idx - e * nei) : 0;
        const int per = is_edge ? nei : 1, off = is_edge ? off_edge : 0;
        const int32_t *ptr = is_edge ? eptr : nptr, *ent = is_edge ? eent : nent;
        const int b = ptr[e], end = ptr[e + 1];
        double s = 0.0;
        if (end - b <= U) {
            int32_t v[U];
            double xv[U];
#pragma unroll
            for (int u = 0; u < U; ++u) v[u] = b + u < end ? ent[b + u] : -1;
#pragma unroll
            for (int u = 0; u < U; ++u) xv[u] = v[u] >= 0 ? x[(int64_t)(v[u] >> 3) * ld + off + (v[u] & 7) * per + k] : 0.0;
#pragma unroll
            for (int u = 0; u < U; ++u)
                if (v[u] >= 0) s += xv[u];
#pragma unroll
            for (int u = 0; u < U; ++u)
                if (v[u] >= 0) x[(int64_t)(v[u] >> 3) * ld + off + (v[u] & 7) * per + k] = s;
            continue;
        }
        for (int q0 = b; q0 < end; q0 += U) {
            int32_t v[U];
            double xv[U];
#pragma unroll
            for (int u = 0; u < U; ++u) v[u] = q0 + u < end ? ent[q0 + u] : -1;
#pragma unroll
            for (int u = 0; u < U; ++u) xv[u] = v[u] >= 0 ? x[(int64_t)(v[u] >> 3) * ld + off + (v[u] & 7) * per + k] : 0.0;
#pragma unroll
            for (int u = 0; u < U; ++u)
                if (v[u] >= 0) s += xv[u];
        }
        for (int q0 = b; q0 < end; q0 += U) {
            int32_t v[U];
#pragma unroll
            for (int u = 0; u < U; ++u) v[u] = q0 + u < end ? ent[q0 + u] : -1;
#pragma unroll
            for (int u = 0; u < U; ++u)
                if (v[u] >= 0) x[(int64_t)(v[u] >> 3) * ld + off + (v[u] & 7) * per + k] = s;
        }
    }
}

void launch_interface_sum(const Launch &L, const LevelDev &lv, const MeshDev &mesh, double *x, int which, bool faces)
{
    const int cap = L.num_cu * 8;
    if (lv.dim == 3 && lv.nfi > 0 && mesh.nfacepairs > 0) {
        const int64_t ncut = mesh.ncut_face_pairs;
        const int64_t first = which == 2 ? ncut : 0;
        const int64_t last = which == 1 || !faces ? ncut : mesh.nfacepairs;
        const int64_t np = last - first;
        if (np > 0) {
            const int64_t blocks = (np + 3) / 4;
            hipLaunchKernelGGL(k_iface_faces, dim3((unsigned)blocks), dim3(256), 0, L.stream, mesh.face_pairs + 3 * first, np,
                               lv.nfi, lv.off_face, lv.ld, x);
            check_launch();
        }
    }
    auto range = [&](int64_t n, int64_t ncut, int64_t &first, int64_t &count) {
        first = which == 2 ? ncut : 0;
        count = which == 1 ? ncut : which == 2 ? n - ncut : n;
    };
    int64_t efirst, ecount, nfirst, ncount;
    range(mesh.nsharededges, mesh.ncut_edge_groups, efirst, ecount);
    range(mesh.nsharednodes, mesh.ncut_node_groups, nfirst, ncount);
    if (lv.nei == 0) ecount = 0;
    const int64_t total = ecount * lv.nei + ncount;
    if (total > 0) {
        int64_t blocks = (total + 255) / 256;
        if (blocks > cap * 4) blocks = cap * 4;
        hipLaunchKernelGGL(k_iface_csr, dim3((unsigned)blocks), dim3(256), 0, L.stream, mesh.edge_ptr + efirst,
                           mesh.edge_ent, ecount, lv.nei, lv.off_edge, mesh.node_ptr + nfirst, mesh.node_ent, ncount,
                           lv.ld, x);
        check_launch();
    }
}

__device__ __forceinline__ void entity_range(const LevelDev &lv, int bit, int &off, int &len)
{
    if (bit < lv.nface) {
        off = lv.off_face + bit * lv.nfi;
        len = lv.nfi;
    } else if (bit < lv.nface + lv.nedge) {
        off = lv.off_edge + (bit - lv.nface) * lv.nei;
        len = lv.nei;
    } else {
        off = bit - lv.nface - lv.nedge;
        len = 1;
    }
}

__global__ void __launch_bounds__(64) k_mask(LevelDev lv, int64_t ncells, const uint16_t *__restrict__ mask, double *x)
{
    const int64_t cell = blockIdx.x;
    if (cell >= ncells) return;
    uint32_t m = mask[cell];
    double *xc = x + cell * lv.ld;
    while (m) {
        const int bit = __ffs((int)m) - 1;
        m &= m - 1;
        int off, len;
        entity_range(lv, bit, off, len);
        for (int k = threadIdx.x; k < len; k += 64) xc[off + k] = 0.0;
    }
}

void launch_mask(const Launch &L, const LevelDev &lv, const MeshDev &mesh, double *x, int which)
{
    hipLaunchKernelGGL(k_mask, dim3((unsigned)mesh.ncells), dim3(64), 0, L.stream, lv, mesh.ncells,
                       which == 0 ? mesh.dmask : mesh.dupmask, x);
    check_launch();
}

template <int NT>
__global__ void __launch_bounds__(NT)
k_prolong_add(LevelDev fine, int nfc, int ldc, const double *__restrict__ xc, double *xf)
{
    extern __shared__ double smem[];
    const int64_t cell = blockIdx.x;
    const double *c = xc + cell * ldc;
    for (int t = threadIdx.x; t < nfc; t += NT) smem[t] = c[t];
    __syncthreads();
    double *f = xf + cell * fine.ld;
    for (int t = threadIdx.x; t < fine.nf; t += NT) {
        const int a = fine.par_a[t], b = fine.par_b[t];
        double y = f[t];
        if (a == b)
            y += 1.0 * smem[a];
        else {
            y += 0.5 * smem[a];
            y += 0.5 * smem[b];
        }
        f[t] = y;
    }
}

template <int NT, int SPT>
__global__ void __launch_bounds__(NT)
k_prolong_add_big(LevelDev fine, int nfc, int ldc, const double *__restrict__ xc, double *xf)
{
    extern __shared__ double smem[];
    const int64_t cell = blockIdx.x;
    const double *c = xc + cell * ldc;
    for (int t0 = threadIdx.x; t0 < nfc; t0 += NT * SPT) {
        double v[SPT];
#pragma unroll
        for (int q = 0; q < SPT; ++q) {
            const int t = t0 + q * NT;
            v[q] = t < nfc ? c[t] : 0.0;
        }
#pragma unroll
        for (int q = 0; q < SPT; ++q) {
            const int t = t0 + q * NT;
            if (t < nfc) smem[t] = v[q];
        }
    }
    __syncthreads();
    double *f = xf + cell * fine.ld;
    for (int t0 = threadIdx.x; t0 < fine.nf; t0 += NT * SPT) {
        double y[SPT];
        uint32_t w[SPT];
#pragma unroll
        for (int q = 0; q < SPT; ++q) {
            const int t = t0 + q * NT;
            if (t < fine.nf) {
                y[q] = f[t];
                w[q] = fine.par32[t];
            }
        }
#pragma unroll
        for (int q = 0; q < SPT; ++q) {
            const int t = t0 + q * NT;
            if (t < fine.nf) {
                const uint32_t a = w[q] & 0xffffu, b = w[q] >> 16;
                double r = y[q];
                if (a == b)
                    r += 1.0 * smem[a];
                else {
                    r += 0.5 * smem[a];
                    r += 0.5 * smem[b];
                }
                f[t] = r;
            }
        }
    }
}

template <int NT, bool USE_LDS>
__global__ void __launch_bounds__(NT)
k_restrict(LevelDev fine, int nfc, int ldc, const double *__restrict__ rf, double *bc)
{
    extern __shared__ double smem[];
    const int64_t cell = blockIdx.x;
    const double *f = rf + cell * fine.ld;
// ... 1122 lines not shown
```

homogenization.jl_amd/csrc/hmg_objects.hpp:

```cpp
#pragma once

#include "../../include/hmg.h"
#include "hmg_device.hpp"
#include "hmg_host.hpp"

#include <atomic>
#include <memory>
#include <mutex>
#include <stdexcept>
#include <string>
#include <vector>

struct ncclComm;

using namespace hmg;

#define HIPCHK(expr)                                                                            \
    do {                                                                                        \
        hipError_t _e = (expr);                                                                 \
        if (_e != hipSuccess)                                                                   \
            throw std::runtime_error(std::string("HIP error: ") + hipGetErrorString(_e) + " (" #expr ")"); \
    } while (0)

namespace hmg {

std::recursive_mutex &lifetime_mutex();
using LifetimeLock = std::lock_guard<std::recursive_mutex>;

std::atomic<int64_t> &device_allocs();

hipError_t device_malloc(void **p, size_t bytes);

struct DryUploads {
    static DryUploads *&current()
    {
        static thread_local DryUploads *c = nullptr;
        return c;
    }
    bool dry;
    uint64_t *hash;
    DryUploads *prev;
    DryUploads(bool dry_, uint64_t *hash_) : dry(dry_), hash(hash_), prev(current()) { current() = this; }
    ~DryUploads() { current() = prev; }
    DryUploads(const DryUploads &) = delete;
    DryUploads &operator=(const DryUploads &) = delete;
    static bool active() { return current() && current()->dry; }
    static void note(const void *data, size_t bytes)
    {
        uint64_t h = *current()->hash ^ (bytes * 0x9e3779b97f4a7c15ull);
        const unsigned char *b = (const unsigned char *)data;
        for (size_t i = 0; i < bytes; ++i) h = (h ^ b[i]) * 1099511628211ull;
        *current()->hash = h;
    }
};

template <class T>
struct DevBuf {
    T *p = nullptr;
    size_t n = 0;
    DevBuf() = default;
    DevBuf(const DevBuf &) = delete;
    DevBuf &operator=(const DevBuf &) = delete;
    ~DevBuf() { release(); }
    void release()
    {
        if (p) (void)hipFree(p);
        p = nullptr;
        n = 0;
    }
    void alloc(size_t count)
    {
        release();
        n = count;
        if (!count || DryUploads::active()) return;
        HIPCHK(device_malloc((void **)&p, count * sizeof(T)));
    }
    void upload(const std::vector<T> &h, hipStream_t s)
    {
        alloc(h.size());
        if (DryUploads::active()) {
            DryUploads::note(h.data(), h.size() * sizeof(T));
            return;
        }
        if (!h.empty()) {
            HIPCHK(hipMemcpyAsync(p, h.data(), h.size() * sizeof(T), hipMemcpyHostToDevice, s));
            HIPCHK(hipStreamSynchronize(s));
        }
    }
};

struct LevelBufs {
    DevBuf<uint64_t> meta;
    DevBuf<uint16_t> lpos, sweep_slot;
    DevBuf<int> slab_head, slab_rs_head;
    DevBuf<uint32_t> slab_ld_word, slab_cp_word, slab_rs_word;
    DevBuf<uint16_t> slab_cp_slot, slab_rs_slot;
    DevBuf<double> rtab;
    int nslab = 0, slab_lds_nodes = 0, slab_max_surf = 0, slab_rs_max_surf = 0, slab_max_int = 0, slab_rs_max_int = 0;
    DevBuf<uint32_t> pos32, pos32w, sweep32, par32, blk_word;
    DevBuf<uint64_t> par64;
    DevBuf<uint16_t> clpos;
    DevBuf<uint32_t> rs_word;
    DevBuf<double> rs_w;
    DevBuf<uint16_t> rs_lp;
    DevBuf<uint16_t> blk_slot;
    DevBuf<uint32_t> wave_tab, wave_lpos, wave_par, wave_cl, wave_rs;
    DevBuf<double> wcache;
    DevBuf<double> ctab;
    DevBuf<int32_t> hier2slot, par_a, par_b, rptr, ridx;
    DevBuf<double> dphi;
};

struct CutKind {
    int64_t nglobal = 0;
    int64_t nentries = 0;
    std::vector<int64_t> gid;
    std::vector<int32_t> seg;
    std::vector<int64_t> sidx;
    DevBuf<int32_t> cell_lid;
    DevBuf<uint8_t> first;
};

struct CutLevel {
    bool ready = false;
    DevBuf<int64_t> pos[3];
    int64_t ndoubles = 0;
    std::vector<int64_t> ops;
    int64_t nstage = 0;
    DevBuf<int64_t> plan;
};

struct ApplyTimer {
    bool on = false;
    int min_level = 0;
    std::vector<std::pair<hipEvent_t, hipEvent_t>> pool;
    std::vector<int> ev_level;
    std::vector<double> ev_bytes;
    size_t used = 0;
};

struct CoarseProbe {
    double *h = nullptr;
    hipEvent_t ev = nullptr;
    bool pending = false;
    int budget = 0;
    int generation = 0;
};

}

struct hmg_ctx {
    int refs = 1;
    ApplyTimer timer;
    bool fuse_cg_default = true;
    bool fold_x = true;
    bool swap_rp = true;
    bool fold_prolong = true;
    bool lazy_dead = true;
    bool lazy_pre = true;
    bool fold_faces = true;
    bool lean_post = true;
    bool lazy_post = true;
    bool fold_coarse_x = true;
    int lazy_top = 2;
    bool zero_entry = true;
    bool fold_restrict = true;
    bool prolong_in_image = true;
    int device = 0;
    hipStream_t stream = nullptr;
    bool own_stream = false;
    DevBuf<double> partials, scal, rpart;
    Launch L{};
    int coarse_maxit = 5000;
    int coarse_check = 25;
    bool coarse_probe = true;
    double coarse_rtol = 1e-13;
    int coarse_poly = 4;
    double coarse_poly_ratio = 20.0;
    ncclComm *comm = nullptr;
    int comm_nranks = 1, comm_rank = 0;
    hipStream_t comm_stream = nullptr;
    hipEvent_t ev_packed = nullptr, ev_summed = nullptr;
    int64_t comm_calls = 0, comm_doubles = 0;
    int64_t small_launches = 0;
    int64_t wc_launches = 0;
    int64_t wave_launches = 0;
    int64_t slab2_launches = 0;
    int64_t rows_launches = 0;
    int64_t wc_max_classes = 0;
    int64_t wc_classes = 0, wc_bytes = 0;
    int64_t wc_refusals = 0;
    int64_t spare_bytes = 0;
    int64_t fcg_bytes = 0;
    int64_t smoother_diag_bytes = 0;
    int64_t smoother_diag_builds = 0;
    int64_t moments_kernel_ns = 0, moments_download_ns = 0;
    int64_t coarse_x_folds = 0;
    int last_pre_form = 0;
    int last_top_form = 0;
    bool vec_pool_on = true;
    std::vector<std::pair<size_t, void *>> vec_pool;
    bool comm_rehearsal = false;
    int64_t overlap_min_doubles = 524288;
    std::vector<struct hmg_grid *> probe_grids;
};

struct hmg_grid {
    int refs = 1;
    hmg_ctx *ctx = nullptr;
    int dim = 0, nlevels = 0;
    std::vector<LevelTables> lt;
    std::vector<std::unique_ptr<LevelBufs>> lb;
    std::vector<LevelDev> ld;
    MeshTables mesh_full, mesh;
    bool shrunk = false;
    MeshDev md{};
    DevBuf<int32_t> d_cells, d_face_pairs, d_face_partner, d_edge_ptr, d_edge_ent, d_node_ptr, d_node_ent, d_node_first;
    DevBuf<uint16_t> d_dmask, d_dupmask;
    DevBuf<uint8_t> d_mult;
    DevBuf<double> d_blockpart;
    bool fuse_cg = true;
    DevBuf<double> d_coef;
    std::vector<double> sigma, coef;
    int sig_n = 0;
    DevBuf<int32_t> d_cell_class;
    DevBuf<double> d_coef_rep;
    int nclasses = 0;
    std::vector<int32_t> cell_class;
    int64_t wc_limit = 0;
    bool wc_trim = false;
    int64_t wc_counted_classes = 0, wc_counted_bytes = 0;
    double wc_lambda = 0.0;
    bool wc_ready = false;
    double lambda = 0.0;
    bool has_op = false;
    uint64_t op_epoch = 0;
    CoarseMatrix cm;
    CoarseDev cd{};
    bool coarse_ready = false;
    DevBuf<int32_t> c_rowptr, c_colidx, c_interior;
    DevBuf<double> c_val, c_diag, c_b, c_x, c_r, c_z, c_p, c_q, c_u, c_z2, c_d;
    DevBuf<double> top_spare;
    bool top_spare_refused = false;
    int smoother = 0;
    std::vector<std::unique_ptr<DevBuf<double>>> dinv;
    bool dinv_ready = false;
    std::vector<char> dinv_level_ready;
    bool dinv_build_counted = false;
    double c_lmax = 2.0;
    int coarse_last_it = 0;
    int coarse_budget = 0;
    int coarse_generation = 0;
    int64_t coarse_misses = 0;
    std::unique_ptr<CoarseProbe> probe{new CoarseProbe};
    std::unique_ptr<Partition> part;
    std::vector<double> sigma_global;
    std::vector<double> part_coords;
    std::vector<int64_t> part_cells;
    std::vector<int32_t> part_owner, part_cut_owner;
    bool part_halo = true;
    int64_t part_nnodes = 0, part_ncells = 0;
    DevBuf<int32_t> d_nodes_g, d_owned, d_cells_gnode;
    CutKind cut[3];
    int64_t cut_agreed[3] = {0, 0, 0};
    bool cut_agreed_ready = false;
    std::vector<std::unique_ptr<CutLevel>> cutlv;
    bool sharers = false;
    hmg_exchange_fn exchange = nullptr, scalar_sum = nullptr;
    hmg_exchange_fn ex_begin = nullptr;
    int (*ex_end)(void *) = nullptr;
    hmg_p2p_fn p2p = nullptr, p2p_begin = nullptr;
    double *stage = nullptr;
    int64_t stage_cap = 0;
    DevBuf<double> own_stage;
    bool overlap = true;
    DevBuf<int32_t> d_cells_cut, d_cells_inner, d_cell_perm;
    void *ex_user = nullptr;
    double *ex_buf = nullptr;
    int64_t ex_cap = 0;
    DevBuf<double> own_exbuf;

    uint64_t upload_hash = 1469598103934665603ull;

    const MeshTables &cur() const { return shrunk ? mesh : mesh_full; }
};

struct hmg_vec {
    hmg_grid *g = nullptr;
    int level = 0;
    double *d = nullptr;
    bool own = false;
    int64_t alloc_cells = 0;
    size_t bytes = 0;
};

namespace hmg {

inline int fail(const std::exception &e)
{
    last_error() = e.what();
    return 1;
}

#define HMG_TRY try {
#define HMG_END                      \
    }                                \
    catch (const std::exception &e)  \
    {                                \
        return fail(e);              \
    }                                \
    catch (...)                      \
    {                                \
        last_error() = "unknown error"; \
        return 1;                    \
    }                                \
    return 0;

inline void need(bool c, const char *msg)
{
    if (!c) throw std::runtime_error(msg);
}

inline const LevelDev &lev(const hmg_grid *g, int level)
{
    need(g != nullptr, "null grid");
    need(g->ctx != nullptr, "this grid was created without a device context (host tables only): no compute path exists on the CPU");
    need(level >= 1 && level <= g->nlevels, "level out of range");
    return g->ld[level - 1];
}

inline void check_vec(const hmg_grid *g, int level, const hmg_vec *v, const char *name)
{
    if (!v) throw std::runtime_error(std::string("null vector: ") + name);
    if (v->g != g) throw std::runtime_error(std::string("vector belongs to another grid: ") + name);
    if (v->level != level) throw std::runtime_error(std::string("vector has the wrong level: ") + name);
    if (v->alloc_cells < g->md.ncells) throw std::runtime_error(std::string("vector too small: ") + name);
}

inline int64_t vec_len(const hmg_vec *v) { return (int64_t)v->g->ld[v->level - 1].ld * v->g->md.ncells; }

inline bool has_exchange(const hmg_grid *g) { return g->exchange || g->ex_begin || g->p2p || g->p2p_begin; }

double *vec_alloc(hmg_ctx *c, size_t bytes);
void vec_release(hmg_ctx *c, void *p, size_t bytes);
void grid_unref(hmg_grid *grid);
double read_scalar(hmg_ctx *c, int slot);

void ensure_weight_cache(hmg_grid *g);
void release_weight_cache(hmg_grid *g);

void set_slab(hmg_grid *g, const LevelDev &lv);
void apply(hmg_grid *g, const LevelDev &lv, double alpha, const double *x, const double *src, double *out, int mask);
void restrict_level(hmg_grid *g, int level_fine, const double *rf, double *bc);
void interface_sum(hmg_grid *g, const LevelDev &lv, double *x, bool faces = true);
void scalar_sum(hmg_grid *g, int slot, int count);
bool reserve_top_spare(hmg_grid *g, bool must);
void release_top_spare(hmg_grid *g);
bool wants_top_spare(const hmg_grid *g, int level);
void ensure_smoother_diag(hmg_grid *g, int level, double *scratch);
void ensure_smoother_diag(hmg_grid *g, int top, hmg_vec **states);
void release_smoother_diag(hmg_grid *g);
void vcycle(hmg_grid *g, int k, int steps, int steps_coarse, hmg_vec **st, bool top = true, bool zero_guess = false);

void coarse_solve(hmg_grid *g, hmg_vec *b1, hmg_vec *x1);
void probe_unlist(hmg_grid *g);
void judge_probes(hmg_ctx *c);

void exchange_cut(hmg_grid *g, const LevelDev &lv, double *x);
void cut_pack(hmg_grid *g, const LevelDev &lv, double *x, int unpack);
void exchange_prepare(hmg_grid *g, const LevelDev &lv);
void exchange_run(hmg_grid *g, const LevelDev &lv, bool async);
void exchange_finish(hmg_grid *g, const LevelDev &lv, bool async);
void comm_drop(hmg_ctx *c);

}
```

homogenization.jl_amd/csrc/hmg_smooth.cpp:

```cpp
#include "../../include/hmg.h"
#include "hmg_objects.hpp"
#include "hmg_pcg.hpp"

#include <algorithm>
#include <cmath>

namespace hmg {

void set_slab(hmg_grid *g, const LevelDev &lv)
{
    const LevelBufs &B = *g->lb[lv.level - 1];
    g->md.slab.head = B.slab_head.p;
    g->md.slab.ld_word = B.slab_ld_word.p;
    g->md.slab.cp_word = B.slab_cp_word.p;
    g->md.slab.cp_slot = B.slab_cp_slot.p;
    g->md.slab.nslab = B.nslab;
    g->md.slab.lds_nodes = B.slab_lds_nodes;
    g->md.slab.max_surf = B.slab_max_surf;
    g->md.slab.max_int = B.slab_max_int;
}

namespace {

struct TimedRegion {
    hmg_ctx *c;
    bool timed;
    int level;
    double bytes;
    TimedRegion(hmg_grid *g, const LevelDev &lv, double bytes_) : c(g->ctx), level(lv.level), bytes(bytes_)
    {
        ApplyTimer &t = c->timer;
        timed = t.on && lv.level >= t.min_level;
        if (!timed) return;
        if (t.used == t.pool.size()) {
            hipEvent_t a, b;
            HIPCHK(hipEventCreate(&a));
            HIPCHK(hipEventCreate(&b));
            t.pool.emplace_back(a, b);
        }
        HIPCHK(hipEventRecord(t.pool[t.used].first, c->stream));
    }
    void stop()
    {
        if (!timed) return;
        ApplyTimer &t = c->timer;
        HIPCHK(hipEventRecord(t.pool[t.used].second, c->stream));
        t.used += 1;
        t.ev_level.push_back(level);
        t.ev_bytes.push_back(bytes);
        timed = false;
    }
};

}

void apply(hmg_grid *g, const LevelDev &lv, double alpha, const double *x, const double *src, double *out, int mask)
{
    TimedRegion tr(g, lv, 8.0 * (double)lv.nf * (double)g->md.ncells * (src ? 3.0 : 2.0));
    set_slab(g, lv);
    ensure_weight_cache(g);
    launch_apply(g->ctx->L, lv, g->md, alpha, g->lambda, x, src, out, mask);
    tr.stop();
}

void restrict_level(hmg_grid *g, int level_fine, const double *rf, double *bc)
{
    const LevelDev &fine = lev(g, level_fine), &coarse = lev(g, level_fine - 1);
    const LevelBufs &B = *g->lb[level_fine - 1];
    if (B.slab_rs_head.p) {
        LevelDev fr = fine;
        fr.ctab = B.rtab.p;
        SlabTables st{};
        st.head = B.slab_rs_head.p;
        st.ld_word = B.slab_ld_word.p;
        st.cp_word = B.slab_rs_word.p;
        st.cp_slot = B.slab_rs_slot.p;
        st.nslab = B.nslab;
        st.lds_nodes = B.slab_lds_nodes;
        st.max_surf = B.slab_rs_max_surf;
        st.max_int = B.slab_rs_max_int;
        launch_restrict_slab(g->ctx->L, fr, g->md, st, coarse.ld, rf, bc);
        return;
    }
    launch_restrict(g->ctx->L, fine, coarse, g->md.ncells, rf, bc);
}

void interface_sum(hmg_grid *g, const LevelDev &lv, double *x, bool faces)
{
    launch_interface_sum(g->ctx->L, lv, g->md, x, 0, faces);
    if (has_exchange(g)) exchange_cut(g, lv, x);
}

void scalar_sum(hmg_grid *g, int slot, int count)
{
    if (g->scalar_sum) {
        if (g->scalar_sum(g->ex_user, g->ctx->L.scal + slot, count) != 0)
            throw std::runtime_error("scalar_sum callback failed");
    }
}

namespace {

void agree_on_cut(hmg_grid *g)
{
    if (g->cut_agreed_ready) return;
    const Partition &P = *g->part;
    hmg_ctx *c = g->ctx;
    if (P.global_ids) {
        for (int k = 0; k < 3; ++k) g->cut_agreed[k] = g->cut[k].nglobal;
    } else if (!g->scalar_sum) {
        for (int k = 0; k < 3; ++k) g->cut_agreed[k] = -1;
    } else {
        double lead[3] = {0.0, 0.0, 0.0};
        for (const Partition::Segment &S : P.segs)
            if (!S.members.empty() && S.members.front() == P.rank)
                for (int k = 0; k < 3; ++k) lead[k] += (double)S.count[k];
        double *d = c->L.scal + S_HOST;
        HIPCHK(hipMemcpyAsync(d, lead, sizeof(lead), hipMemcpyHostToDevice, c->stream));
        scalar_sum(g, S_HOST, 3);
        HIPCHK(hipMemcpyAsync(lead, d, sizeof(lead), hipMemcpyDeviceToHost, c->stream));
        HIPCHK(hipStreamSynchronize(c->stream));
        for (int k = 0; k < 3; ++k) g->cut_agreed[k] = (int64_t)std::llround(lead[k]);
    }
    g->cut_agreed_ready = true;
}

void apply_then_sum(hmg_grid *g, const LevelDev &lv, ApplyArgs a, bool fused, int slot_pap, int slot_rr,
                    bool sum_out = true, bool faces = true)
{
    hmg_ctx *c = g->ctx;
    const Launch &L = c->L;
    set_slab(g, lv);
    ensure_weight_cache(g);
    const double streams = ((a.flags & 128) ? 0.0 : 1.0) + (a.out ? 1.0 : 0.0) + (a.src ? 1.0 : 0.0) + (a.x2 ? 1.0 : 0.0) + (a.xout ? 1.0 : 0.0) +
                           (a.xacc ? 2.0 : 0.0) + (a.x3 ? 1.0 : 0.0) + (a.x4 ? 1.0 : 0.0) + (a.xcoarse ? (double)lv.nf_coarse / (double)lv.nf : 0.0) +
                           (a.rcoarse ? (double)lv.nf_coarse / (double)lv.nf : 0.0) + (a.xc_p ? 2.0 * (double)lv.nf_coarse / (double)lv.nf : 0.0);
    TimedRegion tr(g, lv, 8.0 * (double)lv.nf * (double)g->md.ncells * streams);
    if (has_exchange(g) && g->part) agree_on_cut(g);
    const bool has_cut = has_exchange(g) && g->part && g->cut_agreed[0] >= 0 &&
                         g->cut_agreed[0] + g->cut_agreed[1] + g->cut_agreed[2] > 0;
    const int64_t global_cut = has_cut ? g->cut_agreed[0] * lv.nfi + g->cut_agreed[1] * lv.nei + g->cut_agreed[2] : 0;
    const bool overlap = has_cut && (g->sharers ? g->p2p_begin != nullptr : g->ex_begin != nullptr) && g->ex_end && g->overlap &&
                         global_cut >= std::max<int64_t>(1, c->overlap_min_doubles);
    auto launch = [&](const int32_t *list, int64_t n) {
        ApplyArgs b = a;
        b.cell_list = list;
        b.ncell_list = n;
        if (fused)
            launch_apply_fused_kernel(L, lv, g->md, b);
        else
            launch_apply_args(L, lv, g->md, b);
    };
    auto sums = [&]() {
        if (!fused || slot_pap < 0) return;
        launch_apply_fused_reduce(L, g->md, slot_pap, slot_rr);
        if (slot_rr >= 0 && (slot_rr == slot_pap + 1 || slot_rr + 1 == slot_pap))
            scalar_sum(g, std::min(slot_rr, slot_pap), 2);
        else {
            if (slot_rr >= 0) scalar_sum(g, slot_rr, 1);
            scalar_sum(g, slot_pap, 1);
        }
    };
    if (!a.out && a.rcoarse) {
        need(fused && !sum_out, "epilogue restriction belongs to the cell-local residual");
        launch(nullptr, 0);
        tr.stop();
        return;
    }
    if (!a.out) {
        need(fused, "apply without an output vector");
        launch(nullptr, 0);
        tr.stop();
        sums();
        return;
    }
    if (!sum_out) {
        launch(nullptr, 0);
        tr.stop();
        return;
    }
    if (!overlap) {
        launch(nullptr, 0);
        tr.stop();
        sums();
        interface_sum(g, lv, a.out, faces);
        return;
    }
    if (g->md.ncells_cut > 0) launch(g->md.cells_cut, g->md.ncells_cut);
    launch_interface_sum(L, lv, g->md, a.out, 1);
    exchange_prepare(g, lv);
    cut_pack(g, lv, a.out, 0);
    exchange_run(g, lv, true);
    if (g->md.ncells_inner > 0)
        launch(g->md.cells_inner, g->md.ncells_inner);
    tr.stop();
    launch_interface_sum(L, lv, g->md, a.out, 2, faces);
    sums();
    exchange_finish(g, lv, true);
    cut_pack(g, lv, a.out, 1);
}

enum class Role {
    Plain,
    Pre,
    PostTop,
    PostBelow,
};

enum class Tail {
    Full,
    ScratchP,
    Top2,
    Top3,
    DeadXp,
    DeadDefer,
    DeadDefer2,
    DeadDefer3,
    DeadX2,
};

struct SmoothForm {
    bool swap_rp = false;
    bool ride = false;
    Tail tail = Tail::Full;
    bool hand_up = false;
    bool x_zero = false;
};

struct DeferredX {
    int rs = -1;
    int pap = S_PAP;
    bool two_updates = false;
    int a_num = -1, a_den = -1, b_num = -1, b_den = -1;
    bool three_updates = false;
    int d_num = -1, d_den = -1;
    const double *p = nullptr, *r = nullptr;
};

SmoothForm smooth_form(const hmg_grid *g, int level, int steps, Role role)
{
    const LevelDev &lv = lev(g, level);
    const hmg_ctx *c = g->ctx;
    const bool lean = c->lean_post && (role == Role::PostTop || role == Role::PostBelow);
    const bool dead = role == Role::Pre || (lean && role == Role::PostBelow);
    SmoothForm f;
    if (!g->fuse_cg || g->smoother == 1) {
        f.tail = dead ? Tail::DeadXp : lean ? Tail::ScratchP : Tail::Full;
        return f;
    }
    const bool faces = c->fold_faces && lv.dim == 3 && lv.nfi > 0;
    f.swap_rp = role != Role::Plain && c->swap_rp && steps > 0;
    f.ride = faces;
    if (role == Role::Pre && c->fold_x) {
        f.tail = steps >= 2 && c->lazy_dead ? Tail::DeadDefer2 : Tail::DeadDefer;
        if (f.tail == Tail::DeadDefer2 && steps >= 3 && c->lazy_pre && faces && c->fold_restrict && apply_defers3(c->L, lv) &&
            g->top_spare.n >= (size_t)lv.ld * (size_t)g->md.ncells)
            f.tail = Tail::DeadDefer3;
    }
    else if (dead)
        f.tail = steps >= 2 && c->lazy_post ? Tail::DeadX2 : Tail::DeadXp;
    else if (lean && steps >= 2 && c->lazy_top > 0 && faces)
        f.tail = steps >= 3 && c->lazy_top > 1 && g->top_spare.n >= (size_t)lv.ld * (size_t)g->md.ncells ? Tail::Top3 : Tail::Top2;
    else if (lean)
        f.tail = Tail::ScratchP;
    return f;
}

}

bool reserve_top_spare(hmg_grid *g, bool must)
{
    hmg_ctx *c = g->ctx;
    const LevelDev &lv = g->ld[(size_t)g->nlevels - 1];
    const size_t n = (size_t)lv.ld * (size_t)g->mesh_full.ncells;
    if (g->top_spare.n >= n && n > 0) return true;
    if (g->top_spare_refused && !must) return false;
    HIPCHK(hipSetDevice(c->device));
    void *q = nullptr;
    if (device_malloc(&q, n * sizeof(double)) != hipSuccess) {
        (void)hipGetLastError();
        g->top_spare_refused = true;
        if (must)
            throw std::runtime_error("the spare direction vector of the finest level (" + std::to_string((n * sizeof(double)) >> 20) +
                                     " MiB, option lazy_top = 2) does not fit the device memory; V-cycles take the two-update form");
        return false;
    }
    c->spare_bytes -= (int64_t)(g->top_spare.n * sizeof(double));
    g->top_spare.release();
    g->top_spare.p = (double *)q;
    g->top_spare.n = n;
    g->top_spare_refused = false;
    c->spare_bytes += (int64_t)(n * sizeof(double));
    return true;
}

void release_top_spare(hmg_grid *g)
{
    if (g->ctx) {
        if (g->top_spare.p) (void)hipStreamSynchronize(g->ctx->stream);
        g->ctx->spare_bytes -= (int64_t)(g->top_spare.n * sizeof(double));
    }
    g->top_spare.release();
}

bool wants_top_spare(const hmg_grid *g, int level)
{
    return g->ctx && g->smoother == 0 && g->ctx->lazy_top > 1 && level == g->nlevels && g->dim == 3 && g->ld[(size_t)level - 1].nfi > 0;
}

void ensure_smoother_diag(hmg_grid *g, int level, double *scratch)
{
    if (g->smoother != 1 || level < 2) return;
    need(g->has_op, "operator not set");
    need(g->dinv.size() == (size_t)g->nlevels && level <= g->nlevels, "Jacobi-preconditioned smoother: the inverse diagonals were not reserved");
    if (!g->dinv_ready) {
        g->dinv_level_ready.assign((size_t)g->nlevels, 0);
        g->dinv_build_counted = false;
        g->dinv_ready = true;
    }
    if (g->dinv_level_ready[(size_t)level - 1]) return;
    const LevelDev &lv = lev(g, level);
    double *d = g->dinv[(size_t)level - 1]->p;
    need(scratch != nullptr && scratch != d, "Jacobi-preconditioned smoother: no scratch vector to form the diagonal with");
    for (int limb = diag_limbs() - 1; limb >= 0; --limb) {
        launch_operator_diag(g->ctx->L, lv, g->md, g->lambda, limb, scratch);
        interface_sum(g, lv, scratch);
        launch_diag_accum(g->ctx->L, lv, g->md, scratch, d, limb);
    }
    launch_dinv_finish(g->ctx->L, lv, g->md, d);
    g->dinv_level_ready[(size_t)level - 1] = 1;
    if (!g->dinv_build_counted) {
        g->ctx->smoother_diag_builds += 1;
        g->dinv_build_counted = true;
    }
}

void ensure_smoother_diag(hmg_grid *g, int top, hmg_vec **states)
{
    if (g->smoother != 1) return;
    for (int level = 2; level <= top; ++level) ensure_smoother_diag(g, level, states[5 * (level - 1) + 4]->d);
}

void release_smoother_diag(hmg_grid *g)
{
    int64_t bytes = 0;
    for (const auto &d : g->dinv)
        if (d) bytes += (int64_t)(d->n * sizeof(double));
    if (g->ctx) {
        if (bytes > 0) (void)hipStreamSynchronize(g->ctx->stream);
        g->ctx->smoother_diag_bytes -= bytes;
    }
    g->dinv.clear();
    g->dinv_level_ready.clear();
    g->dinv_ready = false;
}

namespace {

void first_residual(hmg_grid *g, int level, hmg_vec *x, hmg_vec *b, hmg_vec *r, const SmoothForm &f, const hmg_vec *xcoarse,
                    const DeferredX *cx)
{
    const LevelDev &lv = lev(g, level);
    const Launch &L = g->ctx->L;
    const int64_t n = vec_len(x);
    {
        ApplyArgs a{};
        a.alpha = -1.0;
        a.lambda = g->lambda;
        a.x = x->d;
        a.src = b->d;
        a.out = r->d;
        a.flags = 1;
        if (f.x_zero) {
            need(!xcoarse, "zero initial guess with a coarse-grid correction");
            launch_copy(L, r->d, b->d, n);
            launch_mask(L, lv, g->md, r->d, 0);
            interface_sum(g, lv, r->d);
        } else if (xcoarse) {
            a.xcoarse = xcoarse->d;
            a.ldc = lev(g, level - 1).ld;
            a.xout = x->d;
            if (g->ctx->prolong_in_image && apply_lds_bytes(lv) > 48 * 1024) a.flags |= 64;
            if (cx && cx->rs >= 0) {
                need(cx->two_updates && cx->p && cx->r && (a.flags & 64), "pending coarse x-updates where the residual cannot carry them");
                a.xc_p = cx->p;
                a.xc_r = cx->r;
                a.a_num = cx->a_num;
                a.a_den = cx->a_den;
                a.s_num = cx->b_num;
                a.s_den = cx->b_den;
                a.c_num = cx->rs;
                a.c_den = cx->pap;
                g->ctx->coarse_x_folds += 1;
            }
            apply_then_sum(g, lv, a, true, -1, -1);
        } else {
            apply_then_sum(g, lv, a, false, -1, -1);
        }
    }
}

void smooth_pcg(hmg_grid *g, int level, int steps, hmg_vec *x, hmg_vec *r, hmg_vec *p, hmg_vec *Ap, const SmoothForm &f)
{
    const LevelDev &lv = lev(g, level);
    const Launch &L = g->ctx->L;
    const int64_t n = vec_len(x);
    need(g->dinv_ready && g->dinv.size() == (size_t)g->nlevels && g->dinv_level_ready[(size_t)level - 1] && g->dinv[(size_t)level - 1] &&
             (g->dinv[(size_t)level - 1]->p || n == 0),
         "Jacobi-preconditioned smoother: no inverse diagonal for this level");
    need(f.tail == Tail::Full || f.tail == Tail::ScratchP || f.tail == Tail::DeadXp, "Jacobi-preconditioned smoother: unknown tail");
    const double *dinv = g->dinv[(size_t)level - 1]->p;
    int cur = S_RS, other = S_RS2;
    launch_pcg_start(L, p->d, r->d, dinv, n, cur);
    scalar_sum(g, cur, 1);
    for (int i = 0; i < steps; ++i) {
        if (g->fuse_cg) {
            ApplyArgs a{};
            a.alpha = 1.0;
            a.lambda = g->lambda;
            a.x = p->d;
            a.out = Ap->d;
            a.flags = 1;
            apply_then_sum(g, lv, a, true, S_PAP, -1);
        } else {
            apply(g, lv, 1.0, p->d, nullptr, Ap->d, 1);
            interface_sum(g, lv, Ap->d);
            launch_dot(L, p->d, Ap->d, n, S_PAP);
            scalar_sum(g, S_PAP, 1);
        }
        const bool last = i == steps - 1;
        if (last && f.tail != Tail::Full) {
            if (f.tail == Tail::ScratchP) {
                launch_pcg_rupdate(L, r->d, Ap->d, dinv, n, cur, S_PAP, other);
                scalar_sum(g, other, 1);
            }
            launch_cg_xp_update(L, x->d, p->d, r->d, n, cur, S_PAP, cur, other, 0);
            return;
        }
        launch_pcg_rupdate(L, r->d, Ap->d, dinv, n, cur, S_PAP, other);
        scalar_sum(g, other, 1);
        launch_pcg_xp(L, x->d, p->d, r->d, dinv, n, cur, S_PAP, other, cur);
        std::swap(cur, other);
    }
}

DeferredX smooth(hmg_grid *g, int level, int steps, hmg_vec *x, hmg_vec *b, hmg_vec *r, hmg_vec *p, hmg_vec *Ap,
                 const SmoothForm &f, const hmg_vec *xcoarse = nullptr, const DeferredX *cx = nullptr)
{
    const LevelDev &lv = lev(g, level);
    const Launch &L = g->ctx->L;
    const int64_t n = vec_len(x);
    first_residual(g, level, x, b, r, f, xcoarse, cx);
    if (g->smoother == 1) {
        smooth_pcg(g, level, steps, x, r, p, Ap, f);
        return {};
    }
    int cur = S_RS, other = S_RS2;
    if (!g->fuse_cg || steps <= 0) {
        launch_copy_dot(L, p->d, r->d, n, cur);
        scalar_sum(g, cur, 1);
        for (int i = 0; i < steps; ++i) {
            apply(g, lv, 1.0, p->d, nullptr, Ap->d, 1);
            interface_sum(g, lv, Ap->d);
            launch_dot(L, p->d, Ap->d, n, S_PAP);
            scalar_sum(g, S_PAP, 1);
            const bool last = i == steps - 1;
            if (last && f.tail == Tail::DeadXp) {
                launch_cg_xp_update(L, x->d, p->d, r->d, n, cur, S_PAP, cur, other, 0);
                return {};
            }
            launch_cg_update(L, x->d, r->d, p->d, Ap->d, n, cur, S_PAP, other);
            scalar_sum(g, other, 1);
            if (last && f.tail == Tail::ScratchP) return {};
            launch_cg_pupdate(L, p->d, r->d, n, other, cur);
            std::swap(cur, other);
        }
        return {};
    }
    auto args = [&](int i) {
        ApplyArgs a{};
        a.alpha = 1.0;
        a.lambda = g->lambda;
        a.x = r->d;
        a.x2 = i == 0 ? nullptr : p->d;
        a.xout = i == 0 && f.swap_rp ? nullptr : p->d;
        a.xacc = i == 0 ? nullptr : x->d;
        a.a_num = other;
        a.a_den = S_PAP;
        a.out = Ap->d;
        a.s_num = cur;
        a.s_den = other;
        a.flags = 1;
        return a;
    };
    auto exchange_rp = [&]() {
        std::swap(r->d, p->d);
        std::swap(r->own, p->own);
        std::swap(r->alloc_cells, p->alloc_cells);
        std::swap(r->bytes, p->bytes);
    };
    auto step = [&](int i, bool ride) {
        apply_then_sum(g, lv, args(i), true, S_PAP, i == 0 ? cur : -1, true, !ride);
        const double *r_in = r->d;
        if (i == 0 && f.swap_rp) {
            exchange_rp();
            r_in = p->d;
        }
        if (ride)
            launch_cg_rupdate_faces(L, lv, g->md, r_in, r->d, Ap->d, n, cur, S_PAP, other);
        else
            launch_cg_rupdate(L, r_in, r->d, Ap->d, n, cur, S_PAP, other);
        scalar_sum(g, other, 1);
        std::swap(cur, other);
    };
    const int last = steps - 1;
    for (int i = 0; i < last; ++i) {
        if ((f.tail == Tail::Top3 || f.tail == Tail::DeadDefer3) && i == last - 1) {
            ApplyArgs a = args(i);
            a.xout = g->top_spare.p;
            a.xacc = nullptr;
            apply_then_sum(g, lv, a, true, S_PAP2, -1, true, false);
            launch_cg_rupdate_faces(L, lv, g->md, r->d, r->d, Ap->d, n, cur, S_PAP2, S_RS3);
            scalar_sum(g, S_RS3, 1);
            continue;
        }
        step(i, f.ride);
    }
    if (f.tail == Tail::Top2 || f.tail == Tail::Top3) g->ctx->last_top_form = f.tail == Tail::Top3 ? 2 : 1;
    ApplyArgs a = args(last);
    switch (f.tail) {
    case Tail::Full:
    case Tail::ScratchP:
        step(last, f.ride && f.tail == Tail::ScratchP);
        launch_cg_xp_update(L, x->d, p->d, r->d, n, other, S_PAP, cur, other, f.tail == Tail::Full ? 1 : 0);
        return {};
    case Tail::DeadXp:
    case Tail::DeadDefer:
        a.out = nullptr;
        apply_then_sum(g, lv, a, true, S_PAP, last == 0 ? cur : -1, true, true);
        if (last == 0 && f.swap_rp) exchange_rp();
        if (f.tail == Tail::DeadDefer) return DeferredX{cur};
        launch_cg_xp_update(L, x->d, p->d, r->d, n, cur, S_PAP, cur, other, 0);
        return {};
    case Tail::DeadDefer2:
    case Tail::DeadX2:
        a.out = a.xout = a.xacc = nullptr;
        apply_then_sum(g, lv, a, true, S_PAP2, -1);
        if (f.tail == Tail::DeadX2 && f.hand_up) {
            DeferredX d{cur, S_PAP2, true, other, S_PAP, cur, other};
            d.p = p->d;
            d.r = r->d;
            return d;
        }
        if (f.tail == Tail::DeadX2) {
            launch_cg_x2_update(L, x->d, p->d, r->d, n, other, S_PAP, cur, other, cur, S_PAP2);
            return {};
        }
        return DeferredX{cur, S_PAP2, true, other, S_PAP, cur, other};
    case Tail::DeadDefer3:
        a.x2 = g->top_spare.p;
        a.out = a.xout = a.xacc = nullptr;
        a.s_num = S_RS3;
        a.s_den = cur;
        apply_then_sum(g, lv, a, true, S_PAP3, -1);
        {
            DeferredX d{S_RS3, S_PAP3, true, cur, S_PAP2, S_RS3, cur};
            d.three_updates = true;
            d.d_num = other;
            d.d_den = S_PAP;
            return d;
        }
    case Tail::Top2:
        a.xout = a.xacc = nullptr;
        apply_then_sum(g, lv, a, true, S_PAP2, -1, true, false);
        launch_cg_rupdate_faces_x(L, lv, g->md, r->d, r->d, Ap->d, n, cur, S_PAP2, other, x->d, p->d, other, S_PAP, cur, other,
                                  nullptr, 0, 0);
        scalar_sum(g, other, 1);
        return {};
    case Tail::Top3:
        a.x2 = g->top_spare.p;
        a.xout = a.xacc = nullptr;
        a.s_num = S_RS3;
        a.s_den = cur;
        apply_then_sum(g, lv, a, true, S_PAP3, -1, true, false);
        launch_cg_rupdate_faces_x(L, lv, g->md, r->d, r->d, Ap->d, n, S_RS3, S_PAP3, other, x->d, g->top_spare.p, cur, S_PAP2,
                                  S_RS3, cur, p->d, other, S_PAP);
        scalar_sum(g, other, 1);
        return {};
    }
    return {};
}

bool zero_entry_ok(const hmg_grid *g, int k, int steps)
{
    if (!g->ctx->zero_entry) return false;
    if (k == 1) return true;
    if (g->smoother == 1) return false;
    if (steps != 2 || smooth_form(g, k, steps, Role::Pre).tail != Tail::DeadDefer2) return false;
    const LevelDev &lv = g->ld[k - 1];
    if (lv.blk_R > 0) return g->ctx->fold_restrict && apply_restricts(g->ctx->L, lv);
    return true;
}

int vcycle_down(hmg_grid *g, int k, int steps, hmg_vec **st, bool inside = false, bool x_zero = false, int steps_next = -1)
{
    hmg_vec **cur = st + 5 * (k - 1);
    hmg_vec **nxt = st + 5 * (k - 2);
    const Launch &L = g->ctx->L;
    SmoothForm form = smooth_form(g, k, steps, Role::Pre);
    need(!x_zero || form.tail == Tail::DeadDefer2, "zero initial guess: the pre-smoother does not defer both x-updates");
    form.x_zero = x_zero;
    const DeferredX dx = smooth(g, k, steps, cur[0], cur[1], cur[2], cur[3], cur[4], form);
    const int deferred = dx.rs < 0 ? 0 : dx.three_updates ? 3 : dx.two_updates ? 2 : 1;
    const bool skip_fill = inside && steps_next >= 0 && zero_entry_ok(g, k - 1, steps_next);
    if (dx.rs >= 0) {
        ApplyArgs a{};
        a.alpha = -1.0;
        a.lambda = g->lambda;
        a.x = cur[0]->d;
        a.x2 = dx.three_updates ? g->top_spare.p : cur[3]->d;
        a.xout = cur[0]->d;
        if (dx.three_updates) {
            need(g->ctx->fold_restrict && apply_defers3(L, lev(g, k)), "three pending x-updates where the local residual cannot carry them");
            a.x4 = cur[3]->d;
            a.d_num = dx.d_num;
            a.d_den = dx.d_den;
        }
        if (dx.two_updates) {
            a.x3 = cur[2]->d;
            a.a_num = dx.a_num;
            a.a_den = dx.a_den;
            a.s_num = dx.b_num;
            a.s_den = dx.b_den;
            a.c_num = dx.rs;
            a.c_den = dx.pap;
        } else {
            a.s_num = dx.rs;
            a.s_den = dx.pap;
        }
        a.src = cur[1]->d;
        a.out = cur[2]->d;
        a.flags = 1 | (x_zero ? 128 : 0);
        if (g->ctx->fold_restrict && apply_restricts(L, lev(g, k))) {
            if (inside) a.out = nullptr;
            a.rcoarse = nxt[1]->d;
            a.ldrc = lev(g, k - 1).ld;
            apply_then_sum(g, lev(g, k), a, true, -1, -1, false);
            if (!skip_fill) launch_fill(L, nxt[0]->d, vec_len(nxt[0]), 0.0);
            return deferred;
        }
        apply_then_sum(g, lev(g, k), a, true, -1, -1, false);
    } else {
        apply(g, lev(g, k), -1.0, cur[0]->d, cur[1]->d, cur[2]->d, 1);
    }
    restrict_level(g, k, cur[2]->d, nxt[1]->d);
    if (!skip_fill) launch_fill(L, nxt[0]->d, vec_len(nxt[0]), 0.0);
    return deferred;
}

DeferredX vcycle_up(hmg_grid *g, int k, int steps, hmg_vec **st, Role role, const DeferredX *cx = nullptr, bool hand_up = false)
{
    hmg_vec **cur = st + 5 * (k - 1);
    hmg_vec **nxt = st + 5 * (k - 2);
    const Launch &L = g->ctx->L;
    const bool fold_p = g->ctx->fold_prolong && g->fuse_cg && apply_lds_bytes(lev(g, k)) <= 160 * 1024 &&
                        apply_lds_bytes(lev(g, k)) + sizeof(double) * (size_t)lev(g, k - 1).nf <= 80 * 1024;
    need(!(cx && cx->rs >= 0) || fold_p, "pending coarse x-updates without the folded prolongation");
    if (!fold_p) launch_prolong_add(L, lev(g, k), lev(g, k - 1), g->md.ncells, nxt[0]->d, cur[0]->d);
    SmoothForm form = smooth_form(g, k, steps, role);
    form.hand_up = hand_up && form.tail == Tail::DeadX2;
    return smooth(g, k, steps, cur[0], cur[1], cur[2], cur[3], cur[4], form, fold_p ? nxt[0] : nullptr, cx);
}

bool coarse_x_folds(const hmg_grid *g, int k, int steps_below)
{
    const hmg_ctx *c = g->ctx;
    if (k < 3 || g->smoother == 1 || !c->fold_coarse_x || !c->lazy_post || !c->fold_prolong || !c->lean_post || !g->fuse_cg || !c->prolong_in_image) return false;
    const LevelDev &lv = g->ld[(size_t)k - 1];
    if (!(apply_lds_bytes(lv) > 48 * 1024 && apply_lds_bytes(lv) <= 160 * 1024 &&
          apply_lds_bytes(lv) + sizeof(double) * (size_t)g->ld[(size_t)k - 2].nf <= 80 * 1024))
        return false;
    return apply_folds_coarse_x(c->L, lv) && smooth_form(g, k - 1, steps_below, Role::PostBelow).tail == Tail::DeadX2;
}

DeferredX vcycle_level(hmg_grid *g, int k, int steps, int steps_coarse, hmg_vec **st, bool top, bool zero_guess, bool hand_up)
{
    if (k == 1) {
        hmg_vec **cur = st;
        coarse_solve(g, cur[1], cur[0]);
        return {};
    }
    const bool x_zero = (zero_guess || !top) && zero_entry_ok(g, k, steps);
    if (top && zero_guess && !x_zero) launch_fill(g->ctx->L, st[5 * (k - 1)]->d, vec_len(st[5 * (k - 1)]), 0.0);
    const int deferred = vcycle_down(g, k, steps, st, true, x_zero, steps_coarse);
    if (top) g->ctx->last_pre_form = deferred;
    const DeferredX cx = vcycle_level(g, k - 1, steps_coarse, steps_coarse, st, false, false, coarse_x_folds(g, k, steps_coarse));
    if (top) g->ctx->last_top_form = 0;
    return vcycle_up(g, k, steps, st, top ? Role::PostTop : Role::PostBelow, &cx, hand_up);
}

}

void vcycle(hmg_grid *g, int k, int steps, int steps_coarse, hmg_vec **st, bool top, bool zero_guess)
{
    (void)vcycle_level(g, k, steps, steps_coarse, st, top, zero_guess, false);
}

}

extern "C" {

int hmg_grid_reserve_spare(hmg_grid *g, int enable)
{
    HMG_TRY
    need(g != nullptr, "null grid");
    need(g->ctx != nullptr, "this grid was created without a device context (host tables only)");
    if (enable) {
        (void)reserve_top_spare(g, true);
    } else {
        release_top_spare(g);
        g->top_spare_refused = true;
    }
    HMG_END
}

int hmg_grid_set_smoother(hmg_grid *g, int kind)
{
    HMG_TRY
    need(g != nullptr, "null grid");
    need(g->ctx != nullptr, "this grid was created without a device context (host tables only)");
    need(kind == 0 || kind == 1, "smoother kind must be 0 (CG) or 1 (Jacobi-preconditioned CG)");
    HIPCHK(hipSetDevice(g->ctx->device));
    if (kind == 1 && g->dinv.size() != (size_t)g->nlevels) {
        release_smoother_diag(g);
        std::vector<std::unique_ptr<DevBuf<double>>> bufs((size_t)g->nlevels);
        int64_t bytes = 0;
        for (int level = 2; level <= g->nlevels; ++level) {
            const size_t n = (size_t)g->ld[(size_t)level - 1].ld * (size_t)g->mesh_full.ncells;
            bufs[(size_t)level - 1].reset(new DevBuf<double>);
            try {
                bufs[(size_t)level - 1]->alloc(n);
            } catch (const std::exception &) {
                (void)hipGetLastError();
                throw std::runtime_error("hmg_grid_set_smoother: the inverse diagonal of level " + std::to_string(level) + " (" +
                                         std::to_string((n * sizeof(double)) >> 20) + " MiB) does not fit the device memory; the smoother is unchanged");
            }
            bytes += (int64_t)(n * sizeof(double));
        }
        g->dinv = std::move(bufs);
        g->ctx->smoother_diag_bytes += bytes;
    }
    if (kind == 0) {
        release_smoother_diag(g);
    }
    g->smoother = kind;
    g->dinv_ready = false;
    g->op_epoch += 1;
    HMG_END
}

int hmg_grid_smoother(const hmg_grid *g) { return g ? g->smoother : -1; }

int hmg_grid_smoother_diag(hmg_grid *g, int level, hmg_vec *out)
{
    HMG_TRY
    need(g != nullptr, "null grid");
    need(g->smoother == 1, "hmg_grid_smoother_diag: the grid's smoother has no diagonal (hmg_grid_set_smoother(grid, 1))");
    need(level >= 2 && level <= g->nlevels, "level out of range (2..nlevels: level 1 has no smoother)");
    check_vec(g, level, out, "out");
    ensure_smoother_diag(g, level, out->d);
    launch_copy(g->ctx->L, out->d, g->dinv[(size_t)level - 1]->p, vec_len(out));
    HMG_END
}

int hmg_smooth(hmg_grid *g, int level, int steps, hmg_vec *x, hmg_vec *b, hmg_vec *r, hmg_vec *p, hmg_vec *Ap)
{
    HMG_TRY
    need(g && g->has_op, "operator not set");
    check_vec(g, level, x, "x");
    check_vec(g, level, b, "b");
    check_vec(g, level, r, "r");
    check_vec(g, level, p, "p");
    check_vec(g, level, Ap, "Ap");
    ensure_smoother_diag(g, level, Ap->d);
    smooth(g, level, steps, x, b, r, p, Ap, smooth_form(g, level, steps, Role::Plain));
    HMG_END
}

int hmg_level_tune_placement(hmg_grid *g, int level, int steps, hmg_vec **states, int extra, int trials, double *ms_out)
{
    HMG_TRY
    need(g && g->has_op && states, "null argument or operator not set");
    need(level >= 2 && level <= g->nlevels, "level must be 2..nlevels (level 1 has no smoother)");
    need(steps >= 1, "steps must be positive");
    need(extra >= 0 && extra <= 8, "extra must be 0..8");
    need(trials >= 1 && trials <= 512, "trials must be 1..512");
    hmg_vec **state = states + 5 * (level - 1);
    hmg_vec **below = states + 5 * (level - 2);
    for (int q = 0; q < 5; ++q) {
        check_vec(g, level, state[q], "states[] (level)");
        check_vec(g, level - 1, below[q], "states[] (level - 1)");
        need(state[q]->own && state[q]->bytes == state[0]->bytes && state[q]->alloc_cells == state[0]->alloc_cells,
             "the five vectors of the level must be hmg_vec_create'd vectors");
        for (int p = 0; p < q; ++p) need(state[p] != state[q] && state[p]->d != state[q]->d, "the five vectors must be distinct");
    }
    hmg_ctx *c = g->ctx;
    HIPCHK(hipSetDevice(c->device));
    ensure_smoother_diag(g, level, state[4]->d);
    const size_t bytes = state[0]->bytes;
    const int64_t n = vec_len(state[0]);
    std::vector<double *> blk;
    for (int q = 0; q < 5; ++q) blk.push_back(state[q]->d);
    hipEvent_t e0 = nullptr, e1 = nullptr;
    std::vector<int> first = {0, 1, 2, 3, 4}, best = first;
    auto assign = [&](const std::vector<int> &a) {
        for (int q = 0; q < 5; ++q) state[q]->d = blk[(size_t)a[q]];
    };
    auto cleanup = [&](const std::vector<int> &keep) {
        assign(keep);
        (void)hipStreamSynchronize(c->stream);
        for (size_t i = 0; i < blk.size(); ++i)
            if (std::find(keep.begin(), keep.end(), (int)i) == keep.end()) (void)hipFree(blk[i]);
        if (e0) (void)hipEventDestroy(e0);
        if (e1) (void)hipEventDestroy(e1);
    };
    double t_first = 0.0, t_best = 0.0;
    try {
        std::string local_failure;
        try {
            for (int e = 0; e < extra; ++e) blk.push_back(vec_alloc(c, bytes));
            HIPCHK(hipEventCreate(&e0));
            HIPCHK(hipEventCreate(&e1));
        } catch (const std::exception &ex) {
            local_failure = ex.what();
        }
        if (has_exchange(g) && g->part && g->scalar_sum) {
            double failed = local_failure.empty() ? 0.0 : 1.0;
            double *d = c->L.scal + S_HOST;
            HIPCHK(hipMemcpyAsync(d, &failed, sizeof(double), hipMemcpyHostToDevice, c->stream));
            scalar_sum(g, S_HOST, 1);
            HIPCHK(hipMemcpyAsync(&failed, d, sizeof(double), hipMemcpyDeviceToHost, c->stream));
            HIPCHK(hipStreamSynchronize(c->stream));
            if (failed > 0.0 && local_failure.empty())
                local_failure = "placement tuning: another rank could not set it up (nothing was changed on this rank)";
        }
        if (!local_failure.empty()) throw std::runtime_error(local_failure);
        const int nb = (int)blk.size();
        auto run = [&](const std::vector<int> &a) {
            assign(a);
            launch_fill(c->L, state[0]->d, n, 0.5);
            launch_fill(c->L, state[1]->d, n, 1.0);
            HIPCHK(hipEventRecord(e0, c->stream));
            (void)vcycle_down(g, level, steps, states, true, false, 2);
            (void)vcycle_up(g, level, steps, states, Role::PostTop);
            HIPCHK(hipEventRecord(e1, c->stream));
            HIPCHK(hipEventSynchronize(e1));
            float ms = 0.f;
            HIPCHK(hipEventElapsedTime(&ms, e0, e1));
            return (double)ms;
        };
        (void)run(first);
        uint64_t rng = 0x9E3779B97F4A7C15ull;
        auto next = [&]() {
            rng ^= rng << 13;
            rng ^= rng >> 7;
            rng ^= rng << 17;
            return rng;
        };
        t_best = 1e300;
        for (int t = 0; t < trials; ++t) {
            std::vector<int> a(nb);
            for (int i = 0; i < nb; ++i) a[i] = i;
            if (t > 0)
                for (int i = 0; i < 5; ++i) std::swap(a[i], a[i + (int)(next() % (uint64_t)(nb - i))]);
            a.resize(5);
            const double ms = run(a);
            if (t == 0) t_first = ms;
            if (ms < t_best) {
                t_best = ms;
                best = a;
            }
        }
        {
            const double again_first = run(first), again_best = run(best);
            t_first = std::min(t_first, again_first);
            t_best = std::max(t_best, again_best);
            if (!(t_best < 0.995 * t_first)) {
                best = first;
                t_best = t_first;
            }
        }
    } catch (...) {
        cleanup(first);
        throw;
    }
    cleanup(best);
    for (int q = 0; q < 5; ++q) {
        HIPCHK(hipMemsetAsync(state[q]->d, 0, bytes, c->stream));
        HIPCHK(hipMemsetAsync(below[q]->d, 0, sizeof(double) * (size_t)vec_len(below[q]), c->stream));
    }
    if (ms_out) {
        ms_out[0] = t_first;
        ms_out[1] = t_best;
    }
    HMG_END
}

int hmg_vcycle(hmg_grid *g, int top_level, int steps, int steps_coarse, hmg_vec **states)
{
    HMG_TRY
    need(g && g->has_op && states, "null argument or operator not set");
    need(top_level >= 1 && top_level <= g->nlevels, "top_level out of range");
    for (int l = 1; l <= top_level; ++l)
        for (int q = 0; q < 5; ++q) check_vec(g, l, states[5 * (l - 1) + q], "states[]");
    ensure_smoother_diag(g, top_level, states);
    vcycle(g, top_level, steps, steps_coarse, states);
    HMG_END
}

static void check_two_levels(hmg_grid *g, int level, hmg_vec **states)
{
    need(g && g->has_op && states, "null argument or operator not set");
    need(level >= 2 && level <= g->nlevels, "level out of range (2..nlevels)");
    for (int l = level - 1; l <= level; ++l)
        for (int q = 0; q < 5; ++q) check_vec(g, l, states[5 * (l - 1) + q], "states[]");
}

int hmg_vcycle_down(hmg_grid *g, int level, int steps, hmg_vec **states)
{
    HMG_TRY
    check_two_levels(g, level, states);
    ensure_smoother_diag(g, level, states[5 * (level - 1) + 4]->d);
    g->ctx->last_pre_form = vcycle_down(g, level, steps, states);
    HMG_END
}

int hmg_vcycle_up(hmg_grid *g, int level, int steps, hmg_vec **states)
{
    HMG_TRY
    check_two_levels(g, level, states);
    ensure_smoother_diag(g, level, states[5 * (level - 1) + 4]->d);
    (void)vcycle_up(g, level, steps, states, Role::PostTop);
    HMG_END
}

}
```

homogenization.jl_amd/csrc/hmg_stencil.hpp:

```cpp
#pragma once
#include "hmg_device.hpp"

#include <cstdio>
#include <stdexcept>
#include <string>

namespace hmg {

#define HMG_HIP_CHECK(expr)                                                                     \
    do {                                                                                        \
        hipError_t _e = (expr);                                                                 \
        if (_e != hipSuccess)                                                                   \
            throw std::runtime_error(std::string("HIP error: ") + hipGetErrorString(_e) + " at " + \
                                     __FILE__ + ":" + std::to_string(__LINE__));                \
    } while (0)

static inline void check_launch() { HMG_HIP_CHECK(hipGetLastError()); }

constexpr int WSZ = 232;
constexpr int WSZ_RB = 64;

#define HMG_KP(T, p) ((const T __attribute__((address_space(4))) *)(uintptr_t)(p))

__device__ __forceinline__ double axpy1(double a, double x, double y) { return __builtin_fma(a, x, y); }

__device__ __forceinline__ void st_global(double *p, double v)
{
    asm volatile("global_store_dwordx2 %0, %1, off\n\ts_nop 1" : : "v"(p), "v"(v));
}

typedef double hmg_f64x2 __attribute__((ext_vector_type(2)));
__device__ __forceinline__ void st_global2(double *p, double lo, double hi)
{
    hmg_f64x2 v;
    v.x = lo;
    v.y = hi;
    asm volatile("global_store_dwordx4 %0, %1, off\n\ts_nop 1" : : "v"(p), "v"(v));
}

__device__ __forceinline__ double pair_swap_f64(double v)
{
    const int lo = __builtin_amdgcn_update_dpp(0, __double2loint(v), 0xB1, 0xf, 0xf, false);
    const int hi = __builtin_amdgcn_update_dpp(0, __double2hiint(v), 0xB1, 0xf, 0xf, false);
    return __hiloint2double(hi, lo);
}

__device__ __forceinline__ double wave_sum(double v)
{
#pragma unroll
    for (int o = 32; o > 0; o >>= 1) v += __shfl_down(v, o, 64);
    return v;
}

template <int CTRL, int ROW_MASK>
__device__ __forceinline__ double dpp_add(double v)
{
    const int lo = __builtin_amdgcn_update_dpp(0, __double2loint(v), CTRL, ROW_MASK, 0xf, false);
    const int hi = __builtin_amdgcn_update_dpp(0, __double2hiint(v), CTRL, ROW_MASK, 0xf, false);
    return v + __hiloint2double(hi, lo);
}
__device__ __forceinline__ double wave_sum63(double v)
{
    v = dpp_add<0x111, 0xf>(v);
    v = dpp_add<0x112, 0xf>(v);
    v = dpp_add<0x114, 0xf>(v);
    v = dpp_add<0x118, 0xf>(v);
    v = dpp_add<0x142, 0xa>(v);
    v = dpp_add<0x143, 0xc>(v);
    return v;
}

__device__ __forceinline__ double block_sum(double v, double *red)
{
    v = wave_sum63(v);
    const int lane = threadIdx.x & 63, w = threadIdx.x >> 6;
    if (lane == 63) red[w] = v;
    __syncthreads();
    double s = 0.0;
    if (threadIdx.x == 0) {
        const int nw = (blockDim.x + 63) >> 6;
        for (int i = 0; i < nw; ++i) s += red[i];
    }
    __syncthreads();
    return s;
}

__device__ __forceinline__ double sum_partials_all(const double *__restrict__ part, int nb, double *red, double *bc)
{
    double a = 0.0;
    for (int i = threadIdx.x; i < nb; i += blockDim.x) a += part[i];
    const double s = block_sum(a, red);
    if (threadIdx.x == 0) *bc = s;
    __syncthreads();
    return *bc;
}


template <int DIM>
__device__ __forceinline__ void cell_scales(const double *__restrict__ cc, double alpha, double lambda, double *s,
                                            int flags = 0)
{
    constexpr int NTERM = DIM == 3 ? 7 : 4;
#pragma unroll
    for (int t = 0; t < NTERM - 1; ++t) s[t] = (flags & 2) ? 0.0 : alpha * cc[t];
    s[NTERM - 1] = alpha * lambda * ((flags & 16) ? 1.0 : cc[NTERM - 1]);
}

typedef __attribute__((address_space(3))) double lds_f64;
__device__ __forceinline__ double lds_ld(const double *p)
{
    return *(const volatile lds_f64 *)(const lds_f64 *)p;
}

template <int DIM>
__device__ __forceinline__ double stencil_eval_v(const double *w, const double *p, int len, int A, int B, double &ctr)
{
    ctr = lds_ld(p);
    double acc = w[0] * ctr;
    acc += w[1] * lds_ld(p + 1);
    acc += w[2] * lds_ld(p - 1);
    acc += w[3] * lds_ld(p + len - 1);
    acc += w[4] * lds_ld(p - len);
    acc += w[5] * lds_ld(p + len);
    acc += w[6] * lds_ld(p - len - 1);
    if (DIM == 3) {
        const double *pu = p + A;
        const double *pd = p - B;
        acc += w[7] * lds_ld(pu - len);
        acc += w[8] * lds_ld(pd + len + 1);
        acc += w[9] * lds_ld(pu - 1);
        acc += w[10] * lds_ld(pd + 1);
        acc += w[11] * lds_ld(pu);
        acc += w[12] * lds_ld(pd);
        acc += w[13] * lds_ld(pu + 1 - len);
        acc += w[14] * lds_ld(pd + len);
    }
    return acc;
}

template <int DIM>
__device__ __forceinline__ double stencil_eval_c(const double *wr, const double *base, int L, int len, int A, int B,
                                                 double &ctr)
{
    auto at = [&](int off) { return lds_ld(base + max(L + off, 0)); };
    ctr = lds_ld(base + L);
    double acc = lds_ld(wr + 0) * ctr;
    acc += lds_ld(wr + 1) * lds_ld(base + L + 1);
    acc += lds_ld(wr + 2) * at(-1);
    acc += lds_ld(wr + 3) * lds_ld(base + L + len - 1);
    acc += lds_ld(wr + 4) * at(-len);
    acc += lds_ld(wr + 5) * lds_ld(base + L + len);
    acc += lds_ld(wr + 6) * at(-len - 1);
    if (DIM == 3) {
        acc += lds_ld(wr + 7) * lds_ld(base + L + A - len);
        acc += lds_ld(wr + 8) * at(len + 1 - B);
        acc += lds_ld(wr + 9) * lds_ld(base + L + A - 1);
        acc += lds_ld(wr + 10) * at(1 - B);
        acc += lds_ld(wr + 11) * lds_ld(base + L + A);
        acc += lds_ld(wr + 12) * at(-B);
        acc += lds_ld(wr + 13) * lds_ld(base + L + A + 1 - len);
        acc += lds_ld(wr + 14) * at(len - B);
    }
    return acc;
}

__device__ __forceinline__ double to_sgpr(double v)
{
    const unsigned lo = __builtin_amdgcn_readfirstlane(__double2loint(v));
    const unsigned hi = __builtin_amdgcn_readfirstlane(__double2hiint(v));
    return __hiloint2double((int)hi, (int)lo);
}

template <int DIM>
__device__ __forceinline__ void decode32(uint32_t w, int m, int &L, int &len, int &A, int &B, int &cls)
{
    L = (int)(w & 0xffffu);
    cls = (int)(w >> 28);
    if (DIM == 3) {
        const int j = (int)((w >> 16) & 63u), k = (int)((w >> 22) & 63u);
        len = m + 1 - j - k;
        const int n = m - k;
        const int Tk = (int)(__umul24((uint32_t)n + 1u, (uint32_t)n + 2u) >> 1);
        A = Tk - j;
        B = Tk + n + 2 - j;
    } else {
        const int j = (int)((w >> 16) & 255u);
        len = m + 1 - j;
        A = 0;
        B = 0;
    }
}

__device__ __forceinline__ void decode32w(uint32_t w, int m, int &L, int &len, int &A, int &B, int &cls, int &k)
{
    const int i = (int)(w & 127u), j = (int)((w >> 7) & 127u);
    k = (int)((w >> 14) & 127u);
    cls = (int)(w >> 21);
    len = m + 1 - j - k;
    const int n = m - k;
    const int Tk = ((n + 1) * (n + 2)) >> 1;
    A = Tk - j;
    B = Tk + n + 2 - j;
    const int full = (m + 1) * (m + 2) * (m + 3), rest = (n + 1) * (n + 2) * (n + 3);
    L = (full - rest) / 6 + j * (n + 1) - ((j * (j - 1)) >> 1) + i;
}

__device__ __forceinline__ void decode_lattice(uint32_t w, int m, int &L, int &len, int &A, int &B)
{
    L = (int)(w & 0xffffu);
    const int j = (int)((w >> 16) & 127u), k = (int)((w >> 23) & 127u);
    len = m + 1 - j - k;
    const int n = m - k;
    const int Tk = ((n + 1) * (n + 2)) >> 1;
    A = Tk - j;
    B = Tk + n + 2 - j;
}

__host__ __device__ constexpr uint32_t face_tap_mask(int f)
{
    return 0x7fffu & ~(f == 0   ? (1u << 8 | 1u << 10 | 1u << 12 | 1u << 14)
                       : f == 1 ? (1u << 4 | 1u << 6 | 1u << 7 | 1u << 13)
                       : f == 2 ? (1u << 2 | 1u << 3 | 1u << 9 | 1u << 14)
                                : (1u << 1 | 1u << 5 | 1u << 11 | 1u << 13));
}

__device__ __forceinline__ double readlane_f64(double v, int lane)
{
    const unsigned lo = __builtin_amdgcn_readlane(__double2loint(v), lane);
    const unsigned hi = __builtin_amdgcn_readlane(__double2hiint(v), lane);
    return __hiloint2double((int)hi, (int)lo);
}

template <uint32_t M, int NITEM, bool FUSED, bool PAP = FUSED>
__device__ __forceinline__ void class_items(double wv, int wlane0, const double *xs, int m, int nfi, int slot_base, int t0,
                                            const uint32_t (&fw)[NITEM], bool dirichlet, double mult, const double *sc,
                                            double *oc, double &pap, int lane, const double (&pre)[NITEM], bool use_pre,
                                            bool wdot = false, double *keep = nullptr, double wself = 1.0)
{
    double w[15];
#pragma unroll
    for (int d = 0; d < 15; ++d) w[d] = (M >> d) & 1u ? readlane_f64(wv, wlane0 + d) : 0.0;
#pragma unroll
    for (int q = 0; q < NITEM; ++q) {
        const int ti = t0 + q * 64 + lane;
        if (ti < nfi) {
            const int t = slot_base + ti;
            double o = 0.0;
            if (!dirichlet) {
                const double sv = use_pre ? pre[q] : sc ? sc[t] : 0.0;
                int L, len, A, B, cls;
                decode32<3>(fw[q], m, L, len, A, B, cls);
                const double *p = xs + L;
                const double ctr = lds_ld(p);
                double acc = w[0] * ctr;
                if ((M >> 1) & 1u) acc += w[1] * lds_ld(p + 1);
                if ((M >> 2) & 1u) acc += w[2] * lds_ld(p - 1);
                if ((M >> 3) & 1u) acc += w[3] * lds_ld(p + len - 1);
                if ((M >> 4) & 1u) acc += w[4] * lds_ld(p - len);
                if ((M >> 5) & 1u) acc += w[5] * lds_ld(p + len);
                if ((M >> 6) & 1u) acc += w[6] * lds_ld(p - len - 1);
                const double *pu = p + A, *pd = p - B;
                if ((M >> 7) & 1u) acc += w[7] * lds_ld(pu - len);
                if ((M >> 8) & 1u) acc += w[8] * lds_ld(pd + len + 1);
                if ((M >> 9) & 1u) acc += w[9] * lds_ld(pu - 1);
                if ((M >> 10) & 1u) acc += w[10] * lds_ld(pd + 1);
                if ((M >> 11) & 1u) acc += w[11] * lds_ld(pu);
                if ((M >> 12) & 1u) acc += w[12] * lds_ld(pd);
                if ((M >> 13) & 1u) acc += w[13] * lds_ld(pu + 1 - len);
                if ((M >> 14) & 1u) acc += w[14] * lds_ld(pd + len);
                o = wdot ? acc : sv + acc;
                if (PAP) pap += mult * ((wdot ? fma(wself, ctr, sv) : ctr) * o);
            }
            if (!FUSED || oc) oc[t] = o;
            if (keep) keep[q] = o;
        }
    }
}

template <int F, int NITEM, bool FUSED, bool PAP = FUSED>
__device__ __forceinline__ void face_items(double wv, int wlane0, const double *xs, int m, int nfi, int slot_base, int t0,
                                           const uint32_t (&fw)[NITEM], bool dirichlet, double mult, const double *sc,
                                           double *oc, double &pap, int lane, const double (&pre)[NITEM], bool use_pre,
                                           bool wdot = false, double *keep = nullptr, double wself = 1.0)
{
    class_items<face_tap_mask(F), NITEM, FUSED, PAP>(wv, wlane0, xs, m, nfi, slot_base, t0, fw, dirichlet, mult, sc, oc, pap, lane,
                                                     pre, use_pre, wdot, keep, wself);
}

__host__ __device__ constexpr uint32_t edge_tap_mask(int e)
{
    return face_tap_mask(e == 0 || e == 1 || e == 3 ? 0 : e == 2 || e == 4 ? 1 : 2) &
           face_tap_mask(e == 0 ? 1 : e == 1 || e == 2 ? 2 : 3);
}

template <int R>
__device__ __forceinline__ void block_slots(int m, uint32_t word, int slot0, int (&slot)[R])
{
    const int j = (int)((word >> 16) & 63u), n0 = m - (int)((word >> 22) & 63u);
    int sl = slot0, ds = (int)(__umul24((uint32_t)(n0 - 2), (uint32_t)(n0 - 1)) >> 1) - j + 1;
#pragma unroll
    for (int r = 0; r < R; ++r) {
        slot[r] = sl;
        sl += ds;
        ds -= n0 - 2 - r;
    }
}

template <int R, bool FUSED, bool WDOT = false, bool KEEP = false>
__device__ __forceinline__ void interior_block_core(const double (&w)[15], const double *xs, int m, int safe, uint32_t word,
                                                    int slot0, double *oc, double &pap, double (&acc)[R],
                                                    const double *wsv = nullptr, double wself = 1.0)
{
    const int L = (int)(word & 0xffffu), j = (int)((word >> 16) & 63u), k0 = (int)((word >> 22) & 63u);
    const int nv = (int)(word >> 28);
    const int n0 = m - k0;
    const int ds0 = (int)(__umul24((uint32_t)(n0 - 2), (uint32_t)(n0 - 1)) >> 1) - j + 1;
    double ctr[R];
    int len = n0 + 2 - j;
    int delta = (int)(__umul24((uint32_t)(n0 + 2), (uint32_t)(n0 + 3)) >> 1) - j;
    int q = L - delta;
    int slot = slot0, ds = ds0;
#pragma unroll
    for (int s = 0; s < R + 2; ++s) {
        const int qs = s <= nv + 1 ? q : safe;
        const double *a1 = xs + (qs - len - 1), *a2 = xs + (qs - 1), *a3 = xs + (qs + len - 1);
        double v0 = 0.0, v1 = 0.0, v2 = 0.0, v3, v4 = 0.0, v5 = 0.0, v6 = 0.0;
        if (s >= 1) {
            v0 = lds_ld(a1);
            v1 = lds_ld(a1 + 1);
            v2 = lds_ld(a2);
        }
        v3 = lds_ld(a2 + 1);
        if (s <= R) {
            v4 = lds_ld(a2 + 2);
            v5 = lds_ld(a3);
            v6 = lds_ld(a3 + 1);
        }
        if (s >= 2) {
            double t = acc[s - 2];
            t += w[7] * v0;
            t += w[13] * v1;
            t += w[9] * v2;
            t += w[11] * v3;
            if (KEEP) acc[s - 2] = t;
            if (s - 2 < nv) {
                if (!FUSED || oc) oc[slot] = t;
                if (FUSED && !KEEP) pap += (WDOT ? fma(wself, ctr[s - 2], wsv[s - 2]) : ctr[s - 2]) * t;
            }
            slot += ds;
            ds -= n0 - s;
        }
        if (s >= 1 && s <= R) {
            double t = acc[s - 1];
            if (!KEEP) ctr[s - 1] = v3;
            t += w[0] * v3;
            t += w[1] * v4;
            t += w[2] * v2;
            t += w[3] * v5;
            t += w[4] * v1;
            t += w[5] * v6;
            t += w[6] * v0;
            acc[s - 1] = t;
        }
        if (s < R) {
            double t = acc[s];
            t += w[12] * v3;
            t += w[10] * v4;
            t += w[14] * v5;
            t += w[8] * v6;
            acc[s] = t;
        }
        q += delta;
        delta -= n0 + 2 - s;
        len -= 1;
        __builtin_amdgcn_sched_barrier(0);
    }
}

template <int R>
__device__ __forceinline__ void block_positions(int m, uint32_t word, int (&pos)[R])
{
    const int L = (int)(word & 0xffffu), j = (int)((word >> 16) & 63u), n0 = m - (int)((word >> 22) & 63u);
    int delta = (int)(__umul24((uint32_t)(n0 + 2), (uint32_t)(n0 + 3)) >> 1) - j;
    int q = L - delta;
#pragma unroll
    for (int s = 0; s < R + 1; ++s) {
        if (s >= 1) pos[s - 1] = q;
        q += delta;
        delta -= n0 + 2 - s;
    }
}

template <int R, bool FUSED>
__device__ __forceinline__ void interior_block_keep(const double (&w)[15], const double *xs, int m, int safe, uint32_t word,
                                                    int slot0, const double *sc, double *oc, double (&res)[R])
{
    if (sc) {
        int slot[R];
        block_slots<R>(m, word, slot0, slot);
        const int nv = (int)(word >> 28);
#pragma unroll
        for (int r = 0; r < R; ++r) res[r] = r < nv ? sc[slot[r]] : 0.0;
    } else {
#pragma unroll
        for (int r = 0; r < R; ++r) res[r] = 0.0;
    }
    double pap = 0.0;
    interior_block_core<R, FUSED, false, true>(w, xs, m, safe, word, slot0, oc, pap, res);
}

template <int R, bool FUSED, bool SRC>
__device__ __forceinline__ void interior_block(const double (&w)[15], const double *xs, int m, int safe, uint32_t word,
                                               int slot0, const double *sc, double *oc, double &pap, bool wdot = false,
                                               double wself = 1.0)
{
    double acc[R];
    if (SRC) {
        int slot[R];
        block_slots<R>(m, word, slot0, slot);
        const int nv = (int)(word >> 28);
#pragma unroll
        for (int r = 0; r < R; ++r) acc[r] = r < nv ? sc[slot[r]] : 0.0;
        if (FUSED && wdot) {
            double wsv[R];
#pragma unroll
            for (int r = 0; r < R; ++r) {
                wsv[r] = acc[r];
                acc[r] = 0.0;
            }
            interior_block_core<R, FUSED, true>(w, xs, m, safe, word, slot0, oc, pap, acc, wsv, wself);
            return;
        }
    } else {
#pragma unroll
        for (int r = 0; r < R; ++r) acc[r] = 0.0;
    }
    interior_block_core<R, FUSED>(w, xs, m, safe, word, slot0, oc, pap, acc);
}


}
```

Before: 11.12 billion fine-DOF updates/s.

## Fold last post-smoothing CG r-update into a two-pass recomputed apply

For the top-level post-smoother's last CG step, the first apply now writes only surface (face/edge/corner) Ap values plus the pAp sum. A second apply pass recomputes the interior stencil from p and directly updates r = r - alpha*Ap, also applying the pending x-update. Surface entries get face-partner summation inline. This avoids writing and re-reading the full Ap vector and drops a separate r-update kernel, at the cost of recomputing the interior stencil and adding two new kernel instantiations.

```diff
diff --git a/homogenization.jl_amd/csrc/hmg_context.cpp b/homogenization.jl_amd/csrc/hmg_context.cpp
--- a/homogenization.jl_amd/csrc/hmg_context.cpp
+++ b/homogenization.jl_amd/csrc/hmg_context.cpp
@@ -254,6 +254,7 @@
     if (n == "smoother_diag_builds") return ctx->smoother_diag_builds;
     if (n == "lazy_top_form") return ctx->last_top_form;
     if (n == "lazy_pre_form") return ctx->last_pre_form;
+    if (n == "last_ap_form") return ctx->last_ap_form;
     if (n == "coarse_x_folds") return ctx->coarse_x_folds;
     if (n == "cell_moments_kernel_ns") return ctx->moments_kernel_ns;
     if (n == "cell_moments_download_ns") return ctx->moments_download_ns;
@@ -277,7 +278,7 @@
     static const std::pair<const char *, bool hmg_ctx::*> flags[] = {
         {"coarse_probe", &hmg_ctx::coarse_probe}, {"fuse_cg", &hmg_ctx::fuse_cg_default}, {"fold_x", &hmg_ctx::fold_x},
         {"swap_rp", &hmg_ctx::swap_rp}, {"fold_prolong", &hmg_ctx::fold_prolong}, {"zero_entry", &hmg_ctx::zero_entry},
-        {"fold_restrict", &hmg_ctx::fold_restrict}, {"lazy_dead", &hmg_ctx::lazy_dead}, {"lazy_pre", &hmg_ctx::lazy_pre}, {"fold_coarse_x", &hmg_ctx::fold_coarse_x}, {"fold_faces", &hmg_ctx::fold_faces},
+        {"fold_restrict", &hmg_ctx::fold_restrict}, {"lazy_dead", &hmg_ctx::lazy_dead}, {"lazy_pre", &hmg_ctx::lazy_pre}, {"fold_coarse_x", &hmg_ctx::fold_coarse_x}, {"fold_last_ap", &hmg_ctx::fold_last_ap}, {"fold_faces", &hmg_ctx::fold_faces},
         {"lean_post", &hmg_ctx::lean_post}, {"lazy_post", &hmg_ctx::lazy_post}, {"prolong_in_image", &hmg_ctx::prolong_in_image},
         {"comm_rehearsal", &hmg_ctx::comm_rehearsal}};
     for (const auto &f : flags)
diff --git a/homogenization.jl_amd/csrc/hmg_device.hpp b/homogenization.jl_amd/csrc/hmg_device.hpp
--- a/homogenization.jl_amd/csrc/hmg_device.hpp
+++ b/homogenization.jl_amd/csrc/hmg_device.hpp
@@ -137,6 +137,8 @@
     int64_t ncell_list;
     int64_t nwork;
     const int32_t *cell_class;
+    const double *rq;
+    const int32_t *fpart;
 };
 
 struct CoarseDev {
@@ -183,6 +185,7 @@
 bool apply_restricts(const Launch &L, const LevelDev &lv);
 bool apply_folds_coarse_x(const Launch &L, const LevelDev &lv);
 bool apply_defers3(const Launch &L, const LevelDev &lv);
+bool apply_folds_last_ap(const Launch &L, const LevelDev &lv);
 void launch_apply_fused_kernel(const Launch &L, const LevelDev &lv, const MeshDev &mesh, ApplyArgs a);
 void launch_apply_fused_reduce(const Launch &L, const MeshDev &mesh, int slot_pap, int slot_rr);
 void launch_apply_args(const Launch &L, const LevelDev &lv, const MeshDev &mesh, ApplyArgs a);
diff --git a/homogenization.jl_amd/csrc/hmg_kernels.hip b/homogenization.jl_amd/csrc/hmg_kernels.hip
--- a/homogenization.jl_amd/csrc/hmg_kernels.hip
+++ b/homogenization.jl_amd/csrc/hmg_kernels.hip
@@ -52,6 +52,8 @@
     constexpr int NDIR = DIM == 3 ? 15 : 7;
     constexpr int NTERM = DIM == 3 ? 7 : 4;
     constexpr int WS = RB ? WSZ_RB : WSZ;
+    constexpr bool SURF = FUSED && RB != 0 && DIM == 3 && LF == 6;
+    constexpr bool RUPD = FUSED && RB != 0 && DIM == 3 && LF == 7;
     extern __shared__ double smem[];
     double *W = smem;
     double *xs = smem + WS + lv.lds_g0;
@@ -163,7 +165,8 @@
         }
     };
     auto issue_words = [&]() {
-        if (RB) {
+        if (RB && RUPD) {
+        } else if (RB) {
 #pragma unroll
             for (int q = 0; q < FI; ++q) {
                 const int ti = ft0 + q * 64 + lane;
@@ -212,7 +215,7 @@
             for (int q = 0; q < 4; ++q) mq[q] = a.mult ? __builtin_amdgcn_readfirstlane(mqr[q]) : 0x01010101u;
         }
     };
-    constexpr bool rows_late = WC && (LF == 2 || LF == 5);
+    constexpr bool rows_late = WC && (LF == 2 || LF == 5 || LF == 6);
     constexpr bool WEARLY = false;
     if (EARLY && !rows_late) issue_rows();
     if (WEARLY) issue_words();
@@ -226,7 +229,7 @@
         const double beta = x2c ? a.scal[a.s_num] / a.scal[a.s_den] : 0.0;
         const double ax = xac || x3c ? a.scal[a.a_num] / a.scal[a.a_den] : 0.0;
         const double c2 = x3c ? a.scal[a.c_num] / a.scal[a.c_den] : 0.0;
-        constexpr bool X4 = FUSED && RS && LF == 4;
+        constexpr bool X4 = FUSED && ((RS && LF == 4) || RUPD);
         const double *x4c = X4 && a.x4 ? a.x4 + cell * lv.ld : nullptr;
         const double dx4 = x4c ? a.scal[a.d_num] / a.scal[a.d_den] : 0.0;
         const double *ccol = FUSED && !RS && a.xcoarse ? a.xcoarse + cell * a.ldc : nullptr;
@@ -337,7 +340,7 @@
                 }
             }
         }
-        const bool light2 = LF == 2 || (LF == 0 && !RS && FUSED && NT >= 512 && x2c && !xoc && !xac && !x3c && !ccol);
+        const bool light2 = LF == 2 || LF == 6 || (LF == 0 && !RS && FUSED && NT >= 512 && x2c && !xoc && !xac && !x3c && !ccol);
         if (FUSED && light2) {
             double xv[SPT], x2v[SPT];
             int lp[SPT];
@@ -401,10 +404,14 @@
                             const double t1 = axpy1(ax, x2v[q], v);
                             const double p2 = axpy1(beta, x2v[q], xav[q]);
                             v = axpy1(c2, p2, t1);
+                            if (RUPD) {
+                                if (xoc) xoc[t] = v;
+                                v = p2;
+                            }
                         } else if (x2c)
                             v = axpy1(beta, x2v[q], v);
-                        if (xoc) xoc[t] = v;
-                        if (!RS) rr += v * v;
+                        if (xoc && !RUPD) xoc[t] = v;
+                        if (!RS && !RUPD) rr += v * v;
                     }
                     xs[lp[q]] = v;
                 }
@@ -445,8 +452,56 @@
     const bool wdot = WD && FUSED && (a.flags & 8);
     const double wself = (wdot && (a.flags & 256)) ? 0.0 : 1.0;
     HMG_STAMP(2);
+    double us[FI], ur[FI], ues[NE], uer[NE], ucs = 0.0, ucr = 0.0;
+    const double nalpha = RUPD ? -(a.scal[a.c_num] / a.scal[a.c_den]) : 0.0;
+    if constexpr (RUPD) {
+        const double *qc = a.rq + cell * lv.ld;
+        if (face < 4) {
+            const int fb = lv.off_face + face * lv.nfi;
+            const int32_t fp = a.fpart[4 * cell + face];
+            const int64_t pc = fp >> 2;
+            const double *qp = fp >= 0 ? a.rq + pc * lv.ld + lv.off_face + (fp & 3) * lv.nfi : nullptr;
+#pragma unroll
+            for (int q = 0; q < FI; ++q) {
+                const int ti = ft0 + q * 64 + lane;
+                if (ti < lv.nfi) {
+                    const double own = qc[fb + ti];
+                    ur[q] = sc[fb + ti];
+                    if (qp) {
+                        const double other = qp[ti];
+                        us[q] = cell < pc ? own + other : other + own;
+                    } else
+                        us[q] = own;
+                }
+            }
+        }
+#pragma unroll
+        for (int q = 0; q < NE; ++q)
+            if (edge[q] >= 0 && lane < lv.nei) {
+                ues[q] = qc[ebase[q] + lane];
+                uer[q] = sc[ebase[q] + lane];
+            }
+        if (wave == NW - 1 && lane < lv.ncorner) {
+            ucs = qc[lane];
+            ucr = sc[lane];
+        }
+    }
     __syncthreads();
     HMG_STAMP(3);
+    if constexpr (RUPD) {
+        if (face < 4) {
+            const int fb = lv.off_face + face * lv.nfi;
+#pragma unroll
+            for (int q = 0; q < FI; ++q) {
+                const int ti = ft0 + q * 64 + lane;
+                if (ti < lv.nfi) oc[fb + ti] = axpy1(nalpha, us[q], ur[q]);
+            }
+        }
+#pragma unroll
+        for (int q = 0; q < NE; ++q)
+            if (edge[q] >= 0 && lane < lv.nei) oc[ebase[q] + lane] = axpy1(nalpha, ues[q], uer[q]);
+        if (wave == NW - 1 && lane < lv.ncorner) oc[lane] = axpy1(nalpha, ucs, ucr);
+    }
 
     const int wbase = RB ? (1 + lv.nface + lv.nedge) * NDIR : 0;
     auto surface_node = [&](int t, uint32_t pw) -> double {
@@ -474,7 +529,7 @@
         if (tid < nsw) interior_block_keep<RB ? RB : 1, FUSED>(w0e, xs, m, nf >> 1, q0, s0, sc, oc, ki[0]);
         if (NPASS > 1 && tid + NT < nsw) interior_block_keep<RB ? RB : 1, FUSED>(w0e, xs, m, nf >> 1, q1, s1, sc, oc, ki[NPASS - 1]);
     }
-    if (RB) {
+    if (RB && !RUPD) {
         if (DIM == 3) {
             const bool fdir = (dm >> face) & 1u;
             const double fmult = (double)((mq[0] >> (8 * (face & 3))) & 0xffu);
@@ -511,7 +566,7 @@
             }
             if (wave == NW - 1 && lane < lv.ncorner) kc = surface_node(lane, cw);
         }
-    } else {
+    } else if (!RB) {
         const int nit_surf = (nsurf + NT - 1) / NT;
         for (int it = 0; it < nit_surf; ++it) {
             const int t = tid + it * NT;
@@ -526,7 +581,13 @@
 #pragma unroll
     for (int d = 0; d < NDIR; ++d) w0[d] = RB ? readlane_f64(wv, d) : to_sgpr(W[d]);
     if (RB) {
-        if constexpr (!RS) {
+        if constexpr (RUPD) {
+            if (tid < nsw) interior_block_rupdate<RB ? RB : 1>(w0, xs, m, nf >> 1, q0, s0, sc, oc, nalpha);
+            if (NPASS > 1 && tid + NT < nsw) interior_block_rupdate<RB ? RB : 1>(w0, xs, m, nf >> 1, q1, s1, sc, oc, nalpha);
+        } else if constexpr (SURF) {
+            if (tid < nsw) interior_block<RB ? RB : 1, FUSED, false>(w0, xs, m, nf >> 1, q0, s0, nullptr, nullptr, pap);
+            if (NPASS > 1 && tid + NT < nsw) interior_block<RB ? RB : 1, FUSED, false>(w0, xs, m, nf >> 1, q1, s1, nullptr, nullptr, pap);
+        } else if constexpr (!RS) {
         if (DIM == 3 && tid < nsw) {
             if (sc)
                 interior_block<RB ? RB : 1, FUSED, true>(w0, xs, m, nf >> 1, q0, s0, sc, oc, pap, wdot, wself);
@@ -644,7 +705,7 @@
             rc[c] = 0.0 + acc;
         }
     }
-    if (FUSED && !RS) {
+    if (FUSED && !RS && !RUPD) {
         __syncthreads();
         const double s_pap = block_sum(pap, smem);
         const double s_rr = block_sum(rr, smem);
@@ -917,6 +978,11 @@
     return apply_restricts(L, lv) && lv.nf > 2048 && lv.nf <= 13 * 512;
 }
 
+bool apply_folds_last_ap(const Launch &L, const LevelDev &lv)
+{
+    return apply_defers3(L, lv) && lv.nface == 4 && lv.off_int == lv.off_face + 4 * lv.nfi && lv.off_int < lv.nf;
+}
+
 bool apply_folds_coarse_x(const Launch &L, const LevelDev &lv)
 {
     return lv.dim == 3 && apply_lds_bytes(lv) <= 160 * 1024 && L.apply_threads == 0 && L.apply_wg512 && lv.blk_R == 6 && lv.nblk <= 960 &&
@@ -955,7 +1021,11 @@
     auto kern = k_apply<DIM, NT, SPT, FUSED, RB, WD, CG, RS, WC, LF>;
     if (a.rcoarse && !RS) throw std::runtime_error("operator apply: this instantiation cannot restrict in its epilogue");
     if (a.xc_p && !(CG && LF == 5)) throw std::runtime_error("operator apply: this instantiation cannot finish the coarse x");
-    if (a.x4 && LF != 4) throw std::runtime_error("operator apply: this instantiation cannot carry a third pending x-update");
+    if (a.x4 && LF != 4 && LF != 7) throw std::runtime_error("operator apply: this instantiation cannot carry a third pending x-update");
+    if (((a.flags & 512) != 0) != (LF == 6)) throw std::runtime_error("operator apply: surface-only output (flags bit 9) and its instantiation do not match");
+    if ((a.rq != nullptr) != (LF == 7)) throw std::runtime_error("operator apply: the r-update form (rq) and its instantiation do not match");
+    if (LF == 7 && !(a.x2 && a.x3 && a.xout && a.src && a.out && mesh.face_partner))
+        throw std::runtime_error("operator apply: the r-update form needs x2, x3, xout, src, out and the face partner table");
     if ((a.flags & 128) && !(FUSED && (RS || RB == 0)))
         throw std::runtime_error("operator apply: this instantiation cannot take a zero input that is not in memory");
     if (FUSED && a.xcoarse && !CG) lds += sizeof(double) * (size_t)lv.nf_coarse;
@@ -967,6 +1037,7 @@
     ApplyArgs b = a;
     b.nwork = nblocks;
     b.cell_class = WC ? mesh.cell_class : nullptr;
+    b.fpart = LF == 7 ? mesh.face_partner : nullptr;
     if (WC && !weight_cache_ok(L, lv, mesh, a)) throw std::runtime_error("operator apply: class-weight cache not usable for this launch");
     if (L.cell_order && RB && !a.cell_list && !a.ncells_prefix && mesh.cell_perm) {
         b.cell_list = mesh.cell_perm;
@@ -982,7 +1053,13 @@
 static void launch_apply_dim(const Launch &L, const LevelDev &lv, const MeshDev &mesh, const ApplyArgs &a)
 {
     const size_t lds = apply_lds_bytes(lv);
-    if (a.x4 && !(FUSED && DIM == 3 && !WD && a.x3 && a.x2 && a.xout && a.rcoarse && !a.xcoarse && !a.xacc && !(a.flags & 128) &&
+    if (((a.flags & 512) || a.rq) &&
+        !(FUSED && DIM == 3 && !WD && a.out && !a.xcoarse && !a.rcoarse && !a.xacc && !a.xc_p && !a.xc_r && !(a.flags & (2 | 4 | 8 | 16 | 64 | 128 | 256)) &&
+          a.alpha == 1.0 && apply_folds_last_ap(L, lv) && !L.slab2_force &&
+          (a.rq ? !(a.flags & 512) && a.x2 && a.x3 && a.xout && a.src && !a.cell_list && !a.ncells_prefix
+                : a.x2 && !a.x3 && !a.x4 && !a.xout && !a.src)))
+        throw std::runtime_error("operator apply: the two-pass last step (flags bit 9 / rq) where no kernel carries it");
+    if (a.x4 && !a.rq && !(FUSED && DIM == 3 && !WD && a.x3 && a.x2 && a.xout && a.rcoarse && !a.xcoarse && !a.xacc && !(a.flags & 128) &&
                   apply_defers3(L, lv)))
         throw std::runtime_error("operator apply: a third pending x-update (x4) where no kernel carries it");
     if ((a.xc_p || a.xc_r) && !(FUSED && DIM == 3 && !WD && a.xc_p && a.xc_r && a.xcoarse && (a.flags & 64) && !a.x2 && !a.xacc && !a.x3 &&
@@ -1093,6 +1170,10 @@
                         launch_apply_generic<DIM, 512, 13, FUSED, R6, false, false, F3, DIM == 3, F3 ? 4 : 0>(L, lv, mesh, a, apply_lds_bytes_rb(lv));
                     else if (rs)
                         launch_apply_generic<DIM, 512, 13, FUSED, R6, false, false, F3, DIM == 3>(L, lv, mesh, a, apply_lds_bytes_rb(lv));
+                    else if (FUSED && a.rq)
+                        launch_apply_generic<DIM, 512, 13, FUSED, R6, false, false, false, DIM == 3, F3 ? 7 : 0>(L, lv, mesh, a, apply_lds_bytes_rb(lv));
+                    else if (FUSED && (a.flags & 512))
+                        launch_apply_generic<DIM, 512, 13, FUSED, R6, false, false, false, DIM == 3, F3 ? 6 : 0>(L, lv, mesh, a, apply_lds_bytes_rb(lv));
                     else if (FUSED && !a.x2 && !a.xacc && !a.x3 && !a.xcoarse && !a.rcoarse)
                         launch_apply_generic<DIM, 512, 13, FUSED, R6, false, false, false, DIM == 3, F3 ? 1 : 0>(L, lv, mesh, a, apply_lds_bytes_rb(lv));
                     else if (FUSED && a.x2 && (!a.xout || a.xout != a.x2) && !a.xacc && !a.x3 && !a.xcoarse && !a.rcoarse)
@@ -1109,6 +1190,10 @@
                     launch_apply_generic<DIM, 512, 13, FUSED, R6, false, false, F3, false, F3 ? 4 : 0>(L, lv, mesh, a, apply_lds_bytes_rb(lv));
                 else if (rs)
                     launch_apply_generic<DIM, 512, 13, FUSED, R6, false, false, F3>(L, lv, mesh, a, apply_lds_bytes_rb(lv));
+                else if (FUSED && a.rq)
+                    launch_apply_generic<DIM, 512, 13, FUSED, R6, false, false, false, false, F3 ? 7 : 0>(L, lv, mesh, a, apply_lds_bytes_rb(lv));
+                else if (FUSED && (a.flags & 512))
+                    launch_apply_generic<DIM, 512, 13, FUSED, R6, false, false, false, false, F3 ? 6 : 0>(L, lv, mesh, a, apply_lds_bytes_rb(lv));
                 else
                     launch_apply_generic<DIM, 512, 13, FUSED, R6>(L, lv, mesh, a, apply_lds_bytes_rb(lv));
                 return;
diff --git a/homogenization.jl_amd/csrc/hmg_objects.hpp b/homogenization.jl_amd/csrc/hmg_objects.hpp
--- a/homogenization.jl_amd/csrc/hmg_objects.hpp
+++ b/homogenization.jl_amd/csrc/hmg_objects.hpp
@@ -163,6 +163,7 @@
     bool lazy_post = true;
     bool fold_coarse_x = true;
     int lazy_top = 2;
+    bool fold_last_ap = true;
     bool zero_entry = true;
     bool fold_restrict = true;
     bool prolong_in_image = true;
@@ -197,6 +198,7 @@
     int64_t moments_kernel_ns = 0, moments_download_ns = 0;
     int64_t coarse_x_folds = 0;
     int last_pre_form = 0;
+    int last_ap_form = 0;
     int last_top_form = 0;
     bool vec_pool_on = true;
     std::vector<std::pair<size_t, void *>> vec_pool;
diff --git a/homogenization.jl_amd/csrc/hmg_smooth.cpp b/homogenization.jl_amd/csrc/hmg_smooth.cpp
--- a/homogenization.jl_amd/csrc/hmg_smooth.cpp
+++ b/homogenization.jl_amd/csrc/hmg_smooth.cpp
@@ -132,7 +132,9 @@
     const Launch &L = c->L;
     set_slab(g, lv);
     ensure_weight_cache(g);
-    const double streams = ((a.flags & 128) ? 0.0 : 1.0) + (a.out ? 1.0 : 0.0) + (a.src ? 1.0 : 0.0) + (a.x2 ? 1.0 : 0.0) + (a.xout ? 1.0 : 0.0) +
+    const double surf = (double)lv.off_int / (double)lv.nf;
+    const double streams = ((a.flags & 128) ? 0.0 : 1.0) + (a.out ? ((a.flags & 512) ? surf : 1.0) : 0.0) + (a.src && !a.rq ? 1.0 : 0.0) +
+                           (a.rq ? surf + 4.0 * (double)lv.nfi / (double)lv.nf : 0.0) + (a.x2 ? 1.0 : 0.0) + (a.xout ? 1.0 : 0.0) +
                            (a.xacc ? 2.0 : 0.0) + (a.x3 ? 1.0 : 0.0) + (a.x4 ? 1.0 : 0.0) + (a.xcoarse ? (double)lv.nf_coarse / (double)lv.nf : 0.0) +
                            (a.rcoarse ? (double)lv.nf_coarse / (double)lv.nf : 0.0) + (a.xc_p ? 2.0 * (double)lv.nf_coarse / (double)lv.nf : 0.0);
     TimedRegion tr(g, lv, 8.0 * (double)lv.nf * (double)g->md.ncells * streams);
@@ -161,6 +163,12 @@
             scalar_sum(g, slot_pap, 1);
         }
     };
+    if (a.rq) {
+        need(fused && !sum_out, "the r-update form of the apply is a full-grid launch without sums");
+        launch(nullptr, 0);
+        tr.stop();
+        return;
+    }
     if (!a.out && a.rcoarse) {
         need(fused && !sum_out, "epilogue restriction belongs to the cell-local residual");
         launch(nullptr, 0);
@@ -223,6 +231,7 @@
     bool swap_rp = false;
     bool ride = false;
     Tail tail = Tail::Full;
+    bool fold_ap = false;
     bool hand_up = false;
     bool x_zero = false;
 };
@@ -263,6 +272,7 @@
         f.tail = steps >= 3 && c->lazy_top > 1 && g->top_spare.n >= (size_t)lv.ld * (size_t)g->md.ncells ? Tail::Top3 : Tail::Top2;
     else if (lean)
         f.tail = Tail::ScratchP;
+    f.fold_ap = (f.tail == Tail::Top2 || f.tail == Tail::Top3) && role == Role::PostTop && c->fold_last_ap && apply_folds_last_ap(c->L, lv);
     return f;
 }
 
@@ -526,8 +536,35 @@
         }
         step(i, f.ride);
     }
-    if (f.tail == Tail::Top2 || f.tail == Tail::Top3) g->ctx->last_top_form = f.tail == Tail::Top3 ? 2 : 1;
+    if (f.tail == Tail::Top2 || f.tail == Tail::Top3) {
+        g->ctx->last_top_form = f.tail == Tail::Top3 ? 2 : 1;
+        g->ctx->last_ap_form = f.fold_ap ? 1 : 0;
+    }
     ApplyArgs a = args(last);
+    auto last_rupdate = [&](const double *p1, int a_num, int a_den, int b_num, int b_den, int al_num, int al_den, const double *p0,
+                            int z_num, int z_den) {
+        ApplyArgs u{};
+        u.alpha = 1.0;
+        u.lambda = g->lambda;
+        u.x = x->d;
+        u.xout = x->d;
+        u.x2 = p1;
+        u.x3 = r->d;
+        u.x4 = p0;
+        u.a_num = a_num;
+        u.a_den = a_den;
+        u.s_num = b_num;
+        u.s_den = b_den;
+        u.c_num = al_num;
+        u.c_den = al_den;
+        u.d_num = z_num;
+        u.d_den = z_den;
+        u.src = r->d;
+        u.out = r->d;
+        u.rq = Ap->d;
+        u.flags = 32;
+        apply_then_sum(g, lv, u, true, -1, -1, false);
+    };
     switch (f.tail) {
     case Tail::Full:
     case Tail::ScratchP:
@@ -572,6 +609,12 @@
         }
     case Tail::Top2:
         a.xout = a.xacc = nullptr;
+        if (f.fold_ap) {
+            a.flags |= 512;
+            apply_then_sum(g, lv, a, true, S_PAP2, -1, true, false);
+            last_rupdate(p->d, other, S_PAP, cur, other, cur, S_PAP2, nullptr, 0, 0);
+            return {};
+        }
         apply_then_sum(g, lv, a, true, S_PAP2, -1, true, false);
         launch_cg_rupdate_faces_x(L, lv, g->md, r->d, r->d, Ap->d, n, cur, S_PAP2, other, x->d, p->d, other, S_PAP, cur, other,
                                   nullptr, 0, 0);
@@ -582,6 +625,12 @@
         a.xout = a.xacc = nullptr;
         a.s_num = S_RS3;
         a.s_den = cur;
+        if (f.fold_ap) {
+            a.flags |= 512;
+            apply_then_sum(g, lv, a, true, S_PAP3, -1, true, false);
+            last_rupdate(g->top_spare.p, cur, S_PAP2, S_RS3, cur, S_RS3, S_PAP3, p->d, other, S_PAP);
+            return {};
+        }
         apply_then_sum(g, lv, a, true, S_PAP3, -1, true, false);
         launch_cg_rupdate_faces_x(L, lv, g->md, r->d, r->d, Ap->d, n, S_RS3, S_PAP3, other, x->d, g->top_spare.p, cur, S_PAP2,
                                   S_RS3, cur, p->d, other, S_PAP);
@@ -695,7 +744,7 @@
     const int deferred = vcycle_down(g, k, steps, st, true, x_zero, steps_coarse);
     if (top) g->ctx->last_pre_form = deferred;
     const DeferredX cx = vcycle_level(g, k - 1, steps_coarse, steps_coarse, st, false, false, coarse_x_folds(g, k, steps_coarse));
-    if (top) g->ctx->last_top_form = 0;
+    if (top) g->ctx->last_top_form = g->ctx->last_ap_form = 0;
     return vcycle_up(g, k, steps, st, top ? Role::PostTop : Role::PostBelow, &cx, hand_up);
 }
 
@@ -940,6 +989,7 @@
     HMG_TRY
     check_two_levels(g, level, states);
     ensure_smoother_diag(g, level, states[5 * (level - 1) + 4]->d);
+    g->ctx->last_ap_form = 0;
     (void)vcycle_up(g, level, steps, states, Role::PostTop);
     HMG_END
 }
diff --git a/homogenization.jl_amd/csrc/hmg_stencil.hpp b/homogenization.jl_amd/csrc/hmg_stencil.hpp
--- a/homogenization.jl_amd/csrc/hmg_stencil.hpp
+++ b/homogenization.jl_amd/csrc/hmg_stencil.hpp
@@ -306,10 +306,10 @@
     }
 }
 
-template <int R, bool FUSED, bool WDOT = false, bool KEEP = false>
+template <int R, bool FUSED, bool WDOT = false, bool KEEP = false, bool RUPD = false>
 __device__ __forceinline__ void interior_block_core(const double (&w)[15], const double *xs, int m, int safe, uint32_t word,
                                                     int slot0, double *oc, double &pap, double (&acc)[R],
-                                                    const double *wsv = nullptr, double wself = 1.0)
+                                                    const double *wsv = nullptr, double wself = 1.0, double nalpha = 0.0)
 {
     const int L = (int)(word & 0xffffu), j = (int)((word >> 16) & 63u), k0 = (int)((word >> 22) & 63u);
     const int nv = (int)(word >> 28);
@@ -344,15 +344,18 @@
             t += w[11] * v3;
             if (KEEP) acc[s - 2] = t;
             if (s - 2 < nv) {
-                if (!FUSED || oc) oc[slot] = t;
-                if (FUSED && !KEEP) pap += (WDOT ? fma(wself, ctr[s - 2], wsv[s - 2]) : ctr[s - 2]) * t;
+                if (RUPD)
+                    oc[slot] = axpy1(nalpha, t, wsv[s - 2]);
+                else if (!FUSED || oc)
+                    oc[slot] = t;
+                if (FUSED && !KEEP && !RUPD) pap += (WDOT ? fma(wself, ctr[s - 2], wsv[s - 2]) : ctr[s - 2]) * t;
             }
             slot += ds;
             ds -= n0 - s;
         }
         if (s >= 1 && s <= R) {
             double t = acc[s - 1];
-            if (!KEEP) ctr[s - 1] = v3;
+            if (!KEEP && !RUPD) ctr[s - 1] = v3;
             t += w[0] * v3;
             t += w[1] * v4;
             t += w[2] * v2;
@@ -409,6 +412,23 @@
     interior_block_core<R, FUSED, false, true>(w, xs, m, safe, word, slot0, oc, pap, res);
 }
 
+template <int R>
+__device__ __forceinline__ void interior_block_rupdate(const double (&w)[15], const double *xs, int m, int safe, uint32_t word,
+                                                       int slot0, const double *rin, double *rout, double nalpha)
+{
+    int slot[R];
+    block_slots<R>(m, word, slot0, slot);
+    const int nv = (int)(word >> 28);
+    double rv[R], acc[R];
+#pragma unroll
+    for (int r = 0; r < R; ++r) {
+        rv[r] = r < nv ? rin[slot[r]] : 0.0;
+        acc[r] = 0.0;
+    }
+    double pap = 0.0;
+    interior_block_core<R, true, false, false, true>(w, xs, m, safe, word, slot0, rout, pap, acc, rv, 1.0, nalpha);
+}
+
 template <int R, bool FUSED, bool SRC>
 __device__ __forceinline__ void interior_block(const double (&w)[15], const double *xs, int m, int safe, uint32_t word,
                                                int slot0, const double *sc, double *oc, double &pap, bool wdot = false,
```

New measurement: 11.22 billion fine-DOF updates/s (median of 6 runs). Within noise of the previous version (+0.9%).
